# junliu111/CV-MonoSLAM

Hardware: AMD Instinct MI355X
Metric: srukf_updates_per_sec (higher is better)
Workload: dtype f64; 1 GPU; BASELINE configs[2]: 200 inverse-depth landmarks (n=1204, Na=1209, L=2419), M=N matched, fp64, one batched refactor per frame, synthetic 640x480 figure-8 sequence; landmarks=200, state_dim=1204, sequences_per_gpu=1, update_mode=batched

## Files before the change

### cv-monoslam_amd/csrc/srukf_api.hip

```cpp

#include "srukf_ctx.h"
using namespace srukf_impl;


namespace srukf_impl {

void srukf_pool_init()
{
    static std::mutex mu;
    static unsigned long long done_mask = 0;
    int dev = 0; hipMemPool_t pool = nullptr;
    if (hipGetDevice(&dev) != hipSuccess || dev < 0 || dev >= 64) return;
    const unsigned long long bit = 1ull << dev;
    std::lock_guard<std::mutex> lk(mu);
    if (done_mask & bit) return;
    if (hipDeviceGetDefaultMemPool(&pool, dev) == hipSuccess && pool) {
        unsigned long long keep = ~0ull;
        hipMemPoolSetAttribute(pool, hipMemPoolAttrReleaseThreshold, &keep);
    }
    done_mask |= bit;
}

hipError_t srukf_dmalloc_raw(void** p, size_t bytes)
{
    srukf_pool_init();
    hipError_t e = hipMallocAsync(p, bytes ? bytes : 8, nullptr);
    if (e == hipSuccess) e = hipStreamSynchronize(nullptr);
    return e;
}

hipError_t srukf_dfree(void* p) { return p ? hipFreeAsync(p, nullptr) : hipSuccess; }
hipError_t srukf_dfree_on(void* p, hipStream_t st) { return p ? hipFreeAsync(p, st) : hipSuccess; }

thread_local std::string g_create_error;

}

static thread_local double* g_spare_stage = nullptr;

static thread_local size_t g_spare_stage_bytes = 0;

namespace srukf_impl {

const char* const kclass_name[KC_COUNT] = { "k_motion", "k_project", "k_meas_stats", "k_pxy", "k_gain", "k_syrk",
                                             "k_gmw_step64", "k_gmw_persist", "k_gmw_check", "k_gmw_col", "k_rank_expand", "k_project_motion", "k_project_table", "k_pxy2",
                                             "misc", "k_det_response", "k_det_cand", "k_det_rank", "k_det_select", "k_capture_patch", "k_lm_ellipsoid", "k_bgr2gray", "k_overlay",
                                             "k_archive_predict", "k_archive_warp", "k_archive_search", "k_associate_checked" };

void gmw_plan_destroy(GmwPlan& g, hipStream_t st)
{
    if (g.pans) srukf_dfree_on(g.pans, st);
    if (g.sync) srukf_dfree_on(g.sync, st);
    if (g.tiles) srukf_dfree_on(g.tiles, st);
    g = GmwPlan();
}

}

static void gmw_tiles_xcd_order(std::vector<short>& tk, int ntiles_all, int workers, int T, int Tp)
{
    const int ntiles = ntiles_all - ((Tp > 0 && Tp < T) ? T - Tp : 0);
    if (ntiles > workers || ntiles < 16) return;
    struct Tl { short v[4]; };
    std::vector<Tl> comp, rest;
    const int h0 = srukf_gmw_head_rows() / 64, hx = h0 + srukf_gmw_head_extra_diag();
    for (int q = 0; q < ntiles; q++) {
        Tl t; for (int e = 0; e < 4; e++) t.v[e] = tk[4 * q + e];
        const int I = t.v[0], J = t.v[1];
        const bool computes = I >= h0 && !(I < hx && J < hx) && !(Tp < T && I == Tp);
        (computes ? comp : rest).push_back(t);
    }
    if (comp.size() < 16) return;
    std::sort(comp.begin(), comp.end(), [](const Tl& a, const Tl& b) { return a.v[0] != b.v[0] ? a.v[0] < b.v[0] : a.v[1] < b.v[1]; });
    size_t cut = comp.size() / 2;
    while (cut < comp.size() && cut > 0 && comp[cut].v[0] == comp[cut - 1].v[0]) cut++;
    std::vector<std::vector<Tl>> grp(8);
    for (int band = 0; band < 2; band++) {
        std::vector<Tl> b(comp.begin() + (band ? cut : 0), band ? comp.end() : comp.begin() + cut);
        std::sort(b.begin(), b.end(), [](const Tl& x, const Tl& y) { return x.v[1] != y.v[1] ? x.v[1] < y.v[1] : x.v[0] < y.v[0]; });
        for (size_t q = 0; q < b.size(); q++) grp[4 * band + std::min<size_t>(3, q * 4 / b.size())].push_back(b[q]);
    }
    int cap[8] = { 0 };
    for (int w = 0; w < ntiles; w++) cap[(w + 1) % 8]++;
    std::vector<Tl> spill(rest);
    for (int x = 0; x < 8; x++) while ((int)grp[x].size() > cap[x]) { spill.push_back(grp[x].back()); grp[x].pop_back(); }
    for (int x = 0; x < 8; x++) while ((int)grp[x].size() < cap[x] && !spill.empty()) { grp[x].push_back(spill.back()); spill.pop_back(); }
    size_t pos[8] = { 0 };
    for (int w = 0; w < ntiles; w++) {
        const int x = (w + 1) % 8;
        const Tl t = grp[x][pos[x]++];
        for (int e = 0; e < 4; e++) tk[4 * w + e] = t.v[e];
    }
}

namespace srukf_impl {

int gmw_plan_create(GmwPlan& g, int np, hipStream_t st, int Tp, int tenants)
{
    g.T = np / 64;
    g.Tp = (Tp > 0 && Tp < g.T) ? Tp : g.T;
    g.tenants = tenants > 1 ? tenants : 1;
    int cus = 0, dev = 0;
    if (hipGetDevice(&dev) != hipSuccess || hipDeviceGetAttribute(&cus, hipDeviceAttributeMultiprocessorCount, dev) != hipSuccess || cus < 2) cus = 2;
    g.cus = cus;
    const int cap = cus / (tenants > 1 ? tenants : 1) - 1;
    g.workers = cap >= 1 ? srukf_gmw_persist_workers(g.T, g.Tp, cap) : -1;
    g.ntiles = srukf_gmw_build_tiles(g.T, g.Tp, nullptr);
    g.nreal = g.ntiles - (g.Tp < g.T ? g.T - g.Tp : 0);
    std::vector<short> tk((size_t)4 * (g.ntiles > 0 ? g.ntiles : 1), 0);
    srukf_gmw_build_tiles(g.T, g.Tp, tk.data());
    gmw_tiles_xcd_order(tk, g.ntiles, g.workers, g.T, g.Tp);
    const size_t sync_bytes = (size_t)srukf_gmw_sync_bytes(g.T);
    if (srukf_dmalloc_on(&g.pans, (size_t)srukf_gmw_panel_bytes() * g.T, st) != hipSuccess ||
        srukf_dmalloc_on(&g.sync, sync_bytes, st) != hipSuccess ||
        srukf_dmalloc_on(&g.tiles, sizeof(short) * tk.size(), st) != hipSuccess) { gmw_plan_destroy(g, st); return SRUKF_ERR_NOMEM; }
    const unsigned long long epoch1 = 1;
    if (hipMemsetAsync(g.pans, 0, (size_t)srukf_gmw_panel_bytes() * g.T, st) != hipSuccess ||
        hipMemsetAsync(g.sync, 0, sync_bytes, st) != hipSuccess ||
        hipMemcpyAsync((char*)g.sync + offsetof(GmwSync, epoch), &epoch1, sizeof epoch1, hipMemcpyHostToDevice, st) != hipSuccess ||
        hipMemcpyAsync(g.tiles, tk.data(), sizeof(short) * tk.size(), hipMemcpyHostToDevice, st) != hipSuccess ||
        hipStreamSynchronize(st) != hipSuccess) { gmw_plan_destroy(g, st); return SRUKF_ERR_HIP; }
    return SRUKF_OK;
}

void host_weights(int Na, const srukf_params& p, KWeights& w)
{
    const double alpha = p.ut_alpha, beta = p.ut_beta;
    const double Lammda = alpha * alpha * Na - Na;
    switch (p.weight_type) {
    case 0:
        w.wm0 = 1.0 - Na / 3.0; w.wc0 = 1.0 - Na / 3.0; w.wi = (1.0 - w.wc0) / (2 * Na); w.wi_sr = sqrt(w.wi);
        w.gamma = sqrt(Na / (1.0 - w.wm0));
        break;
    case 1:
        w.gamma = sqrt(Na + Lammda); w.wm0 = Lammda / (Na + Lammda); w.wc0 = w.wm0 + (1 - alpha * alpha + beta);
        w.wi = 1.0 / (2 * (Na + Lammda)); w.wi_sr = sqrt(fabs(w.wi));
        break;
    default:
        w.gamma = sqrt(3.0 * Na / 2.0); w.wm0 = 1.0 / 3.0; w.wc0 = 1.0 / 3.0; w.wi = 1.0 / (3.0 * Na); w.wi_sr = sqrt(w.wi);
        break;
    }
}

void prof_collect(srukf_ctx* c)
{
    for (auto& e : c->pev) {
        float ms = 0.f;
        hipEventSynchronize(e.b);
        hipEventElapsedTime(&ms, e.a, e.b);
        c->prof_ms[e.kc] += ms; c->prof_n[e.kc] += 1;
        hipEventDestroy(e.a); hipEventDestroy(e.b);
    }
    c->pev.clear();
}

}


namespace srukf_impl {

std::vector<int> build_tile_table(int n_own, int n_other, bool upper, bool own_is_row, int k_index )
{
    std::vector<std::vector<int>> lst(8);
    for (int x = 0; x < 8; x++)
        for (int o = 0; o < n_other; o++)
            for (int w = x; w < n_own; w += 8) {
                const int r = own_is_row ? w : o, c = own_is_row ? o : w;
                if (upper && c < r) continue;
                lst[x].push_back(r); lst[x].push_back(c);
            }
    {
        for (auto& l : lst) {
            std::vector<std::pair<int, int>> t;
            for (size_t q = 0; q < l.size() / 2; q++) t.push_back({ l[2 * q], l[2 * q + 1] });
            std::stable_sort(t.begin(), t.end(), [k_index](const std::pair<int, int>& a, const std::pair<int, int>& b) {
                return k_index ? a.second > b.second : a.first > b.first; });
            for (size_t q = 0; q < t.size(); q++) { l[2 * q] = t[q].first; l[2 * q + 1] = t[q].second; }
        }
    }
    size_t mx = 0;
    for (auto& l : lst) mx = l.size() / 2 > mx ? l.size() / 2 : mx;
    std::vector<int> tab(mx * 8 * 2, -1);
    for (int x = 0; x < 8; x++)
        for (size_t q = 0; q < lst[x].size() / 2; q++) { tab[(q * 8 + x) * 2] = lst[x][2 * q]; tab[(q * 8 + x) * 2 + 1] = lst[x][2 * q + 1]; }
    return tab;
}

}

static int alloc_zero(srukf_ctx* c, void** p, size_t bytes)
{
    HIPCHK(c, srukf_dmalloc_on(p, bytes, c->stream));
    HIPCHK(c, hipMemsetAsync(*p, 0, bytes, c->stream));
    return SRUKF_OK;
}

#define ALLOC(ptr, count) do { int rc_ = alloc_zero(c, (void**)&(ptr), sizeof(*(ptr)) * (size_t)(count)); if (rc_) { g_create_error = c->err; srukf_destroy(c); return rc_; } } while (0)

static int block_cov(srukf_ctx* c, int off, int bs, double* out)
{
    srukf_launch_block_cov(c->stream, c->d, c->S, off, bs, c->small, nullptr);
    HIPCHK(c, hipMemcpyAsync(c->hstage, c->small, sizeof(double) * bs * bs, hipMemcpyDeviceToHost, c->stream));
    HIPCHK(c, hipStreamSynchronize(c->stream));
    memcpy(out, c->hstage, sizeof(double) * bs * bs);
    return SRUKF_OK;
}

extern "C" {

int srukf_abi_version(void) { return SRUKF_ABI_VERSION; }

int srukf_default_params(srukf_params* p)
{
    if (!p) return SRUKF_ERR_BAD_ARG;
    memset(p, 0, sizeof *p);
    p->cam_dx = 0.0028; p->cam_dy = 0.0028; p->cam_cx = 310.1129; p->cam_cy = 236.7526;
    p->cam_k1 = 0.0001; p->cam_k2 = 0.0; p->cam_f = 2.1735; p->image_w = 640; p->image_h = 480;
    p->a1 = p->a2 = p->a3 = p->a4 = 8.0; p->sigma_measure = 3.0; p->rho0 = 1.0 / 3.0; p->sigma_rho = p->rho0 / 2.0;
    p->sigma_x = 0.02; p->sigma_y = 0.02; p->sigma_z = 0.005; p->sigma_theta = 0.02;
    p->epsilon = 1e-13; p->ut_alpha = 1e-3; p->ut_beta = 2.0;
    p->weight_type = 0; p->noise_type = 0; p->newton_iters = 100;
    return SRUKF_OK;
}

const char* srukf_last_error(const srukf_ctx* ctx) { return ctx ? ctx->err.c_str() : g_create_error.c_str(); }

int srukf_create(srukf_ctx** out, int N, const srukf_params* p, int device, void* stream)
{
    if (!out || !p || N < 0) { g_create_error = "bad argument"; return SRUKF_ERR_BAD_ARG; }
    if (N > 32 * SRUKF_STAT_GROUPS) { g_create_error = "more than 2048 landmarks: the per-group statistics counters (FrameScalars::stat_cnt) serve 64 groups of 32"; return SRUKF_ERR_UNSUPPORTED; }
    if (p->noise_type != 0) { g_create_error = "noise_type != 0 draws random numbers (SLAM.cpp:1505-1516) and is not built"; return SRUKF_ERR_UNSUPPORTED; }
    int ndev = 0;
    if (hipGetDeviceCount(&ndev) != hipSuccess || ndev <= 0 || device < 0 || device >= ndev) {
        g_create_error = "no HIP device (this library has no CPU fallback)";
        return SRUKF_ERR_NO_DEVICE;
    }
    if (hipSetDevice(device) != hipSuccess) { g_create_error = "hipSetDevice failed"; return SRUKF_ERR_NO_DEVICE; }
    hipDeviceProp_t prop;
    if (hipGetDeviceProperties(&prop, device) != hipSuccess) { g_create_error = "hipGetDeviceProperties failed"; return SRUKF_ERR_NO_DEVICE; }
    if (strncmp(prop.gcnArchName, "gfx950", 6) != 0) {
        g_create_error = std::string("device is ") + prop.gcnArchName + ", kernels are built for gfx950 only";
        return SRUKF_ERR_NO_DEVICE;
    }
    srukf_ctx* c = new srukf_ctx();
    c->device = device; c->p = *p;
    if (!g_dbg_graphs) c->use_graph = false;
    if (stream) { c->stream = (hipStream_t)stream; c->own_stream = false; }
    else {
        if (hipStreamCreateWithFlags(&c->stream, hipStreamNonBlocking) != hipSuccess) { g_create_error = "hipStreamCreate failed"; delete c; return SRUKF_ERR_HIP; }
        c->own_stream = true;
    }
    KDims& d = c->d;
    d.N = N; d.n = 6 * N + 4; d.Na = d.n + 5; d.L = 2 * d.Na + 1;
    d.np = round_up(d.n, SRUKF_PAD); d.mp = round_up(2 * N > 0 ? 2 * N : 1, SRUKF_PAD);
    host_weights(d.Na, c->p, c->w);
    const size_t np = d.np, mp = d.mp;
    ALLOC(c->X, np); ALLOC(c->S, np * np); ALLOC(c->G, np * np); ALLOC(c->Gbak, np * np); ALLOC(c->Wf, np * np);
    ALLOC(c->sigR, (size_t)d.L * 8 + 8); ALLOC(c->mpart, srukf_meas_part_doubles(d.mp)); ALLOC(c->dxp, srukf_gain_part_doubles(d.np)); ALLOC(c->Cmat, (np + 64) * 4); ALLOC(c->Z, (size_t)d.L * mp); ALLOC(c->DZ, np * mp);
    ALLOC(c->Ut, mp * np); ALLOC(c->PxyR, 5 * mp);
    { const size_t Nn = (size_t)(N > 0 ? N : 1); ALLOC(c->h, mp + 4 * Nn + (Nn + 1) / 2); c->Si = c->h + mp; c->vis = (int*)(c->h + mp + 4 * Nn);
      ALLOC(c->zcur, mp + (Nn + 1) / 2); c->mcur = (int*)(c->zcur + mp); }
    ALLOC(c->D, np); ALLOC(c->odocur, 8); ALLOC(c->small, 64);
    ALLOC(c->theta, np); ALLOC(c->fs, 1);
    { char* pb0 = nullptr; char* pb1 = nullptr; ALLOC(pb0, srukf_gmw_panel_bytes()); ALLOC(pb1, srukf_gmw_panel_bytes()); c->pan[0] = pb0; c->pan[1] = pb1; }
// ... 530 lines not shown
```

### cv-monoslam_amd/csrc/srukf_ctx.h

```cpp
#pragma once
#include <hip/hip_runtime.h>
#include <math.h>
#include <stdio.h>
#include <stdlib.h>
#include <string.h>
#include <string>
#include <cstddef>
#include <vector>
#include <algorithm>
#include <utility>
#include <atomic>
#include <mutex>
#include <map>
#include "srukf_device.h"
#include "srukf_rank.h"

extern "C" {
void srukf_launch_motion(hipStream_t, KDims, KWeights, srukf_params, double*, double*, double*, double*, FrameScalars*, const double*, const double*, RankArgs);
void srukf_launch_project(hipStream_t, KDims, KWeights, srukf_params, const double*, const double*, const double*, double*, double*, const FrameScalars*);
void srukf_launch_meas_stats(hipStream_t, KDims, KWeights, const double*, const double*, const double*, double*, double*, double*, int*, double*);
int srukf_meas_part_doubles(int);
void srukf_launch_gain(hipStream_t, KDims, KWeights, double*, const double*, const double*, const int*, const double*, const double*,
                       const double*, const int*, const int*, FrameScalars*, double*, double*, const double*, RankArgs, const double*, double*,
                       const double*, int, const double*, double, const double*, int, const double*, double*);
void srukf_launch_project_motion(hipStream_t, KDims, KWeights, srukf_params, double*, double*, double*, double*, double*, double*, FrameScalars*, RankArgs);
int srukf_gain_part_doubles(int);
void srukf_launch_traj(hipStream_t, KDims, const double*, const double*, FrameScalars*, double*, int);
void srukf_launch_block_cov(hipStream_t, KDims, const double*, int, int, double*, const double*);
void srukf_launch_project_points(hipStream_t, srukf_params, int, const double*, const double*, const double*, const double*, double*);
void srukf_launch_pxy(hipStream_t, KDims, const double*, const double*, double*, const void*, int, KWeights, MeasArgs);
void srukf_launch_pxy2(hipStream_t, KDims, const double*, const double*, double*, double*, const void*, int, int, KWeights, MeasArgs, GainFold);
int srukf_pxy2_build_tiles(int mp, int np, int kr, int* out);
int srukf_pxy2_split_groups(void);
void srukf_launch_syrk(hipStream_t, KDims, const double*, const double*, int, int, double*, FrameScalars*, const void*, int, const double*, double*, RankArgs, const double*);
void srukf_launch_gmw_step64(hipStream_t, int, int, int, double, double*, const void*, void*, double*, double*, const FrameScalars*);
int srukf_gmw_panel_bytes(void);
int srukf_gmw_sync_bytes(int T);
int srukf_gmw_build_tiles(int T, int Tp, short* out);
int srukf_gmw_persist_workers(int T, int Tp, int max_workers);
void srukf_launch_gmw_persist(hipStream_t, int, int, double, double*, void*, double*, double*, void*, const void*, int, int, void*, const double*, const double*, int, int, int, int, int);
void srukf_launch_gmw_persist_head(hipStream_t, int, int, double, double*, void*, double*, double*, void*, const void*, int, int, void*, const double*, const double*, int, int, int, int, int, const HeadArgs*);
void srukf_launch_gmw_split(hipStream_t, hipStream_t, int, int, double, double*, void*, double*, double*, void*, const void*, int, void*, int, int, double*, double*, int);
void srukf_launch_gmw_split_fold(hipStream_t, hipStream_t, int, int, double, double*, void*, double*, double*, void*, const void*, int, void*, int, int, double*, double*, const double*, const double*, int);
int srukf_gmw_build_fold_list(int T, int Tp, short* out);
int srukf_gmw_fold_head_tile(int tr, int tc, int head_rows);
int srukf_gmw_fold_head_rows(int Tp);
void srukf_gmw_fold_head_override(int v);
void srukf_launch_gmw_split_alone(hipStream_t, int, int, int, double, double*, void*, double*, double*, void*, const void*, int, void*, int, int, double*, double*);
void srukf_launch_row_energy(hipStream_t, int, int, const double*, double*);
void srukf_launch_rank_diag(hipStream_t, int, int, const double*, const int*, double*);
void srukf_launch_rank_expand(hipStream_t, int, int, int, double, const double*, const double*, const int*, const int*, const double*, void*, const double*, int, double*, double*, double*, double, int, KDims, KWeights, srukf_params, double*, double*, int, const StepExport*, double, unsigned int*, int);
void srukf_launch_project_table(hipStream_t, KDims, KWeights, srukf_params, double*, double*, double*, double*, double*, double*, FrameScalars*, RankArgs, NullSkip);
void srukf_launch_sigr_rows(hipStream_t, KDims, KWeights, const double*, const double*, double*, const FrameScalars*, const int*, int);
void srukf_launch_rank_shadow(hipStream_t, int, int, int, const double*, const int*, double*);
void srukf_launch_rank_canon(hipStream_t, int, int, int, double, const int*, double*);
void srukf_launch_rank_round(hipStream_t, int, int, double*);
void srukf_launch_syrk_own(hipStream_t, int, int, const double*, const double*, int, int, int, double*, void*, const void*, int, int);
int srukf_gmw_register_form(int, int, int, int);
int srukf_pxy2_b_per(int, int);
void srukf_launch_pxy2_b(hipStream_t, KDims, const void*, int, const void*, int, int, KWeights, int);
void srukf_launch_gain_b(hipStream_t, KDims, KWeights, const void*, int, int, double);
void srukf_launch_syrk_b(hipStream_t, KDims, const void*, int, const void*, int, int, int, int);
void srukf_launch_syrk_own_b(hipStream_t, int, int, const void*, int, int, int, int, const void*, int, int);
void srukf_launch_gmw_step64_b(hipStream_t, int, int, int, double, const void*, int, int, int);
void srukf_launch_gmw_pivslab_b(hipStream_t, int, int, int, double, const void*, int, int, int);
void srukf_launch_gmw_trail_b(hipStream_t, int, int, const void*, int, int, int, int);
void srukf_launch_rank_expand_b(hipStream_t, int, int, int, double, const void*, int, double, KDims, KWeights, srukf_params);
int srukf_gmw_head_rows(void);
int srukf_gmw_head_extra_diag(void);
void srukf_launch_gmw_check(hipStream_t, int, int, const double*, const double*, FrameScalars*, const double*, int, double*);
void srukf_launch_gmw_col(hipStream_t, int, int, int, double, const double*, double*, double*, unsigned long long*, FrameScalars*, double*);
void srukf_set_exact_right_looking(int on);
void srukf_warm_exact_path(hipStream_t st, FrameScalars* fs);
int srukf_get_exact_right_looking(void);
void srukf_launch_gmw_stats(hipStream_t, int, int, const double*, FrameScalars*);
void srukf_launch_landmarks_cartesian(hipStream_t, KDims, const double*, const double*, double*, double*);
void srukf_launch_aug_map(hipStream_t, srukf_params, int, int, int, int, double, const double*, const double*, const double*, double*);
void srukf_launch_aug_x(hipStream_t, int, int, int, double, double, const double*, const double*, const int*, double*, double*, int, int);
void srukf_launch_aug_build(hipStream_t, int, int, int, int, double, double, const double*, const double*, const double*, double*, int, int, int);
void srukf_launch_gram(hipStream_t, int, int, const double*, double*);
void srukf_launch_warp_patch(hipStream_t, KDims, srukf_params, const double*, const double*, const double*, const double*, const double*, const double*,
                             const unsigned char*, const int*, unsigned char*);
void srukf_launch_associate(hipStream_t, KDims, srukf_params, const unsigned char*, const double*, const double*, const int*, const int*,
                            const unsigned char*, double*, int*, double*);
int srukf_mixed_build_tasks(int np, int ue, short* out_tasks, int* out_tiles, int* ntiles);
int srukf_mixed_build_tasks_red(int np, int ue, int krows, int rows_lim, short* out_tasks, int* out_tiles, int* ntiles);
int srukf_mixed_krows(int r);
void srukf_launch_split_bf3(hipStream_t, int, int, int, int, const double*, void*, size_t);
void srukf_launch_syrk_bf3(hipStream_t, int, int, int, int, int, const void*, size_t, const void*, int, const void*, int, double*, double*, void*);
size_t srukf_mixed_part_bytes(int ntasks);
void srukf_launch_cvt_f32(hipStream_t, size_t, const double*, float*);
void srukf_launch_cvt_robot_cols(hipStream_t, int, int, const double*, float*);
void srukf_launch_gain_dx(hipStream_t, int, int, const double*, double*, const double*);
void srukf_launch_syrk32(hipStream_t, int, int, int, const float*, const float*, const void*, int, const void*, int, double*, double*, void*, int);
int srukf_app_patch_stride(void);
int srukf_app_tmpl_stride(void);
void srukf_launch_associate_checked(hipStream_t, KDims, srukf_params, double, double, int, int, const unsigned char*, const double*, const double*, const int*, const int*,
                                    const unsigned char*, double*, int*, double*, double*, double*);
int srukf_match_score_stride(void);
int srukf_match_tmpl_stride(void);
}

#define SRUKF_GRAPH_FRAMES 8
#define SRUKF_MAX_TENANTS 4
#define SRUKF_NULL_ENERGY 1e-12
#ifndef SRUKF_BATCH_GROUPS_MAX
#define SRUKF_BATCH_GROUPS_MAX 4
#endif

enum KClass { KC_MOTION = 0, KC_PROJECT, KC_STATS, KC_PXY, KC_GAIN, KC_SYRK, KC_GMW_TRAIL, KC_GMW_PERSIST, KC_GMW_CHECK,
              KC_GMW_COL, KC_RANK_EXPAND, KC_PROJECT_MOTION, KC_PROJECT_TABLE, KC_PXY2, KC_MISC,
              KC_DET_RESPONSE, KC_DET_CAND, KC_DET_RANK, KC_DET_SELECT, KC_CAPTURE, KC_LM_ELLIPSOID, KC_BGR2GRAY, KC_OVERLAY,
              KC_ARCHIVE_PREDICT, KC_ARCHIVE_WARP, KC_ARCHIVE_SEARCH, KC_ASSOC_CHECKED, KC_COUNT };
struct ProfEvent { hipEvent_t a, b; int kc; };

struct GmwPlan { void* pans = nullptr; void* sync = nullptr; void* tiles = nullptr; int ntiles = 0, nreal = 0, T = 0, Tp = 0, workers = -1, tenants = 1, cus = 0; };

struct DetScratch {
    double *resp = nullptr, *cand_r = nullptr; int *cand_pix = nullptr, *sorted = nullptr, *rank = nullptr, *gxy = nullptr, *blk = nullptr; void* hdr = nullptr;
    void *in = nullptr, *out = nullptr; size_t in_bytes = 0, out_bytes = 0;
};

struct RansacScratch {
    double *Ut = nullptr, *D = nullptr, *zin = nullptr, *res = nullptr, *X = nullptr, *S = nullptr, *odo = nullptr;
    double *sigR = nullptr, *Cm = nullptr, *Z = nullptr, *DZ = nullptr, *h = nullptr, *PxyR = nullptr, *mpart = nullptr;
    unsigned char* F = nullptr; int* votes = nullptr; FrameScalars* fs = nullptr;
};

struct ArchiveState {
    int L = 0;
    double *X6 = nullptr, *S66 = nullptr, *R = nullptr, *t = nullptr, *px = nullptr, *rob = nullptr, *out = nullptr, *hst = nullptr;
    unsigned char *patch = nullptr, *tmpl = nullptr;
};


struct srukf_switches {
    int rank_aware = 1;
    int debug_allow_mixed = 0;
    int debug_starve = 0;
    bool split_off = false;
    bool use_graph = true;
    struct DbgSwitches {
        int fused_motion = 2;
        int f32_fuse = 1;
        int table_perm = 1;
        int tail_fuse = 1;
        int head_fold = 1;
        int nullskip = 1;
        int pxy2 = 1;
        int step_fuse_export = 1;
        int view_auto = 1;
        int step_early = 2;
        int step_spin = 1;
        int step_fast = 1;
        int split_record = 0;
        int null_canon = 1;
        int split_fold = 1;
        int gain_fold = 0;
        int mixed_rank = 1;
        int mixed_null_ppm = 1;
        int mixed_bf16 = 0;
        int mixed_f64_robot = 1;
    } dbg;
};

struct srukf_handle_scope : srukf_switches {
    int device = 0;
    hipStream_t stream = nullptr;
    bool own_stream = false;
    srukf_params p;
    std::vector<srukf_ctx*> retired;
    double* spare_stage = nullptr; size_t spare_stage_bytes = 0;
    bool profiling = false;
    std::vector<ProfEvent> pev;
    double prof_ms[KC_COUNT] = {}; long long prof_n[KC_COUNT] = {}; double prof_flops[KC_COUNT] = {}; double prof_bytes[KC_COUNT] = {};
    unsigned char *d_image = nullptr, *d_bgr = nullptr, *d_ovl = nullptr; bool frame_valid = false, bgr_valid = false;
    DetScratch det;
    ArchiveState archive;
    std::string err;
    template <class F> void each_device_buffer(F f) const { void* b[] = { d_image, d_bgr, d_ovl }; for (void* q : b) f(q); }
};

struct srukf_life {
    int storage = SRUKF_STORAGE_F64;
    bool dx_pending = false;
    bool dx_lm = false;
    bool xr1_pending = false;
    int K_new = 0;
    bool null_canonical = false;
    bool tail_ok = false;
    int clamp_frame_host = -1, clamp_row_host = -1;
    int seqF = 0;
    int phase = 0;
    bool frame_updated = false;
    bool next_odo_valid = false;
    bool async_pending = false;
    bool step_fast = false;
    bool step_uncommitted = false;
    bool step_chain = false;
    bool proj_valid = false;
    bool fs_seq_step = false;
    bool last_update_sequential = false;
    bool ck_valid = false;
    bool ck3_inflight = false;
    bool ck_pending = false;
    bool pre_issued = false;
    bool next_pose_pending = false;
    bool setstep_done = false;
    unsigned long long meas_seq = 0;
    bool step_export_attached = false;
    StepExport step_export = {};
    bool mirror_next = false;
    bool view_auto = false; int view_unused = 0;
    int view_hits = 0;
    bool view_cached = false;
    bool robot_cached = false;
    bool f32_stale = false;
    int step_fast_frames = 0, step_slow_frames = 0;
    int exact_frames = 0;
};

struct srukf_map_scope : srukf_life {
    KDims d;
    KWeights w;
    double *X = nullptr, *S = nullptr, *G = nullptr, *Gbak = nullptr, *Wf = nullptr;
    double *sigR = nullptr, *Cmat = nullptr, *Z = nullptr, *DZ = nullptr, *Ut = nullptr;
    double *h = nullptr, *Si = nullptr, *PxyR = nullptr, *D = nullptr;
    double *zcur = nullptr, *odocur = nullptr, *small = nullptr, *mpart = nullptr, *dxp = nullptr;
    int *vis = nullptr, *mcur = nullptr;
    unsigned long long* theta = nullptr;
    unsigned int* fold_sync = nullptr; double* dxk = nullptr; int fold_robot_tiles = 0;
    unsigned char *app_patch = nullptr, *app_tmpl = nullptr;
    double *appR = nullptr, *appT = nullptr, *appPx = nullptr, *corr = nullptr;
    int* has_app = nullptr;
    double* ov_in = nullptr; void* ov_rec = nullptr;
    double *match_res = nullptr, *match_scores = nullptr; bool match_valid = false;
    RansacScratch ransac;
    double* disp = nullptr;
    float *S32 = nullptr, *X32 = nullptr;
    float *U32 = nullptr; double* mx_part = nullptr; void *mx_tasks = nullptr, *mx_tiles = nullptr; int mx_ntasks = 0, mx_ntiles = 0;
    float* A32 = nullptr; double* mxr_part = nullptr; void *mxr_tasks = nullptr, *mxr_tiles = nullptr; int mxr_ntasks = 0, mxr_ntiles = 0, mxr_krows = 0, mxr_for_r = 0;
    int* mxr_f64_tiles = nullptr; int mxr_n_f64_tiles = 0;
    unsigned short* mxr_xt = nullptr; size_t mxr_xt_stride = 0; int mxr_ktot = 0;
    int *perm = nullptr, *iperm = nullptr;
    double* Sdis = nullptr;
    void* pan[2] = { nullptr, nullptr };
    GmwPlan gplan;
    int red_r = 0, red_Tp = 0;
    int *red_perm = nullptr, *red_iperm = nullptr;
    double* gdiag = nullptr;
    double *shadowA = nullptr, *Utp = nullptr;
    double *slabW = nullptr, *slabL = nullptr;
    double *gsW = nullptr, *gsL = nullptr; int gs_panels = 0;
    hipStream_t side = nullptr; hipEvent_t ev_fork = nullptr, ev_join = nullptr;
    double* P1 = nullptr; int* pxy2_tiles = nullptr; int n_pxy2_tiles = 0, pxy2_split_b0 = 0;
    int* nskip = nullptr; int ns_full = 0, ns_null = 0, ns_rows = 0;
    int* red_head0_tiles = nullptr; int n_red_head0_tiles = 0;
    void* split_fold_list = nullptr; int n_split_fold = 0;
    double red_head0_flop = 0.0;
    int* red_syrk_tiles = nullptr; int n_red_syrk_tiles = 0;
    double red_fac_flop = 0, red_own_flop = 0;
    GmwPlan gplan_red;
    int shared_tenants = 2;
    int gmw_shared = 0;
    double *ckS = nullptr, *ckX = nullptr;
    int *syrk_tiles = nullptr, *pxy_tiles = nullptr;
    int *syrk_head_tiles = nullptr;
    int n_syrk_tiles = 0, n_pxy_tiles = 0, n_syrk_head_tiles = 0, n_syrk_head_crit = 0;
    int* syrk_head_tiles_b = nullptr; int n_syrk_head_tiles_b = 0;
// ... 184 lines not shown
```

### cv-monoslam_amd/csrc/srukf_debug.hip

```cpp

#include "srukf_ctx.h"
using namespace srukf_impl;


namespace srukf_impl {
std::atomic<int> g_dbg_gmw_persist{1}, g_dbg_gmw_fused{1}, g_dbg_rank_fused{1}, g_dbg_rank_fold{1}, g_dbg_rank_aware{1}, g_dbg_graphs{1};
std::atomic<int> g_dbg_mem_split{1};
std::atomic<int> g_dbg_shared_tenants{2};
std::atomic<int> g_dbg_batch_wide{1}, g_dbg_batch_groups{0}, g_dbg_batch_split{1};
std::atomic<int> g_dbg_timing{0}, g_dbg_fold_head{0}, g_dbg_fold_force{0}, g_dbg_ctx_keep{24}, g_dbg_batch_xcd{1}, g_dbg_batch_k128{1};
std::atomic<int> g_dbg_head_fold_free{0};
}

static bool debug_buffer(srukf_ctx* c, const char* key, double** ptr, long long* cap)
{
    const KDims& d = c->d;
    const GmwPlan& gp = c->red_r > 0 ? c->gplan_red : c->gplan;
    double* src = nullptr; long long n = 0;
    if (!strcmp(key, "Z")) { src = c->Z; n = (long long)d.L * d.mp; }
    else if (!strcmp(key, "DZ")) { src = c->DZ; n = (long long)d.np * d.mp; }
    else if (!strcmp(key, "sigR")) { src = c->sigR; n = (long long)(d.L + 1) * 8; }
    else if (!strcmp(key, "Cmat")) { src = c->Cmat; n = (long long)d.n * 4; }
    else if (!strcmp(key, "Xr1")) { src = (double*)((char*)c->fs + offsetof(FrameScalars, Xr1)); n = 4; }
    else if (!strcmp(key, "Utp")) { src = c->Utp; n = c->Utp ? (long long)d.mp * d.np : 0; }
    else if (!strcmp(key, "P1")) { src = c->P1; n = c->P1 ? (long long)d.mp * d.np : 0; }
    else if (!strcmp(key, "h")) { src = c->h; n = 2LL * d.N; }
    else if (!strcmp(key, "Si")) { src = c->Si; n = 4LL * d.N; }
    else if (!strcmp(key, "det_resp")) { src = c->det.resp; n = c->det.resp ? (long long)c->p.image_w * (long long)c->p.image_h : 0; }
    else if (!strcmp(key, "Wf")) { src = c->Wf; n = (long long)d.np * d.np; }
    else if (!strcmp(key, "Gbak")) { src = c->Gbak; n = (long long)d.np * d.np; }
    else if (!strcmp(key, "G")) { src = c->G; n = (long long)d.np * d.np; }
    else if (!strcmp(key, "D")) { src = c->D; n = d.np; }
    else if (!strcmp(key, "fold_dbg")) { src = c->fold_sync ? (double*)(c->fold_sync + ((srukf_fold_words(d.mp / 64, d.np / 64) + 1) & ~1)) : nullptr; n = c->fold_sync ? FOLD_DBG_STAMPS : 0; }
    else if (!strcmp(key, "gsW")) { src = c->gsW; n = c->gsW ? (long long)c->gs_panels * 64 * d.np : 0; }
    else if (!strcmp(key, "gsL")) { src = c->gsL; n = c->gsL ? (long long)c->gs_panels * 64 * d.np : 0; }
    else if (!strcmp(key, "pans")) { src = (double*)gp.pans; n = gp.pans ? (long long)srukf_gmw_panel_bytes() * gp.T / 8 : 0; }
    else if (!strcmp(key, "sync")) { src = (double*)gp.sync; n = gp.sync ? (long long)srukf_gmw_sync_bytes(gp.T) / 8 : 0; }
    else return false;
    *ptr = src; *cap = n;
    return true;
}

extern "C" {

int srukf_debug_allow_mixed(srukf_ctx* c, int on)
{
    if (!c) return SRUKF_ERR_BAD_ARG;
    c->debug_allow_mixed = on ? 1 : 0;
    return SRUKF_OK;
}

int srukf_debug_poke_state(srukf_ctx* c, int row, int col, double value)
{
    if (!c || row < 0 || col < row || col >= c->d.n) return SRUKF_ERR_BAD_ARG;
    HIPCHK(c, hipSetDevice(c->device));
    step_commit_motion(c); step_invalidate(c);
    HIPCHK(c, hipStreamSynchronize(c->stream));
    HIPCHK(c, hipMemcpy(c->S + (size_t)row * c->d.np + col, &value, sizeof(double), hipMemcpyHostToDevice));
    return SRUKF_OK;
}

int srukf_debug_set(srukf_ctx* c, const char* key, int value)
{
    if (!key) return SRUKF_ERR_BAD_ARG;
    struct { const char* k; std::atomic<int>* v; } globals[] = { { "gmw_persist", &g_dbg_gmw_persist }, { "gmw_fused", &g_dbg_gmw_fused }, { "rank_fused", &g_dbg_rank_fused },
                                                    { "rank_fold", &g_dbg_rank_fold }, { "rank_aware", &g_dbg_rank_aware }, { "graphs", &g_dbg_graphs }, { "mem_split", &g_dbg_mem_split }
                                                  };
    if (!strcmp(key, "batch_split")) { g_dbg_batch_split = value ? 1 : 0; batch_drop_all_graphs(); return SRUKF_OK; }
    if (!strcmp(key, "head_fold_free")) { if (value < 1) return SRUKF_ERR_BAD_ARG; g_dbg_head_fold_free = value; if (c) { hipSetDevice(c->device); step_commit_motion(c); step_invalidate(c); hipStreamSynchronize(c->stream); drop_graphs(c); } return SRUKF_OK; }
    if (!strcmp(key, "batch_groups")) { if (value < 0 || value > SRUKF_BATCH_GROUPS_MAX) return SRUKF_ERR_BAD_ARG; g_dbg_batch_groups = value; return SRUKF_OK; }
    if (!strcmp(key, "batch_wide")) { g_dbg_batch_wide = value ? 1 : 0; return SRUKF_OK; }
    if (!strcmp(key, "timing")) { g_dbg_timing = value ? 1 : 0; return SRUKF_OK; }
    if (!strcmp(key, "fold_head")) { g_dbg_fold_head = value < 0 ? 0 : value; srukf_gmw_fold_head_override(g_dbg_fold_head); return SRUKF_OK; }
    if (!strcmp(key, "batch_k128")) { g_dbg_batch_k128 = value ? 1 : 0; batch_drop_all_graphs(); return SRUKF_OK; }
    if (!strcmp(key, "batch_xcd")) { g_dbg_batch_xcd = value ? 1 : 0; batch_drop_all_graphs(); return SRUKF_OK; }
    if (!strcmp(key, "ctx_keep")) { g_dbg_ctx_keep = value < 0 ? 0 : value; return SRUKF_OK; }
    if (!strcmp(key, "fold_force")) { g_dbg_fold_force = value ? 1 : 0; return SRUKF_OK; }
    if (!strcmp(key, "exact_rl")) { srukf_set_exact_right_looking(value); return SRUKF_OK; }
    if (!strcmp(key, "shared_tenants")) {
        if (value < 2 || value > 8) return SRUKF_ERR_BAD_ARG;
        g_dbg_shared_tenants = value;
        return SRUKF_OK;
    }
    for (auto& g : globals)
        if (!strcmp(key, g.k)) {
            g.v->store(!strcmp(key, "mem_split") ? value : (value ? 1 : 0));
            if (c) { hipSetDevice(c->device); step_commit_motion(c); step_invalidate(c); hipStreamSynchronize(c->stream); drop_graphs(c); if (!strcmp(key, "rank_aware")) return update_null_set(c); }
            return SRUKF_OK;
        }
    if (!c) return SRUKF_ERR_BAD_ARG;
    HIPCHK(c, hipSetDevice(c->device));
    step_commit_motion(c); step_invalidate(c);
    HIPCHK(c, hipStreamSynchronize(c->stream));
    if (!strcmp(key, "use_graph")) c->use_graph = value != 0;
    else if (!strcmp(key, "pxy2")) c->dbg.pxy2 = value ? 1 : 0;
    else if (!strcmp(key, "nullskip")) c->dbg.nullskip = value ? 1 : 0;
    else if (!strcmp(key, "head_fold")) c->dbg.head_fold = value ? 1 : 0;
    else if (!strcmp(key, "tail_fuse")) c->dbg.tail_fuse = value ? 1 : 0;
    else if (!strcmp(key, "table_perm")) c->dbg.table_perm = value ? 1 : 0;
    else if (!strcmp(key, "f32_fuse")) c->dbg.f32_fuse = value ? 1 : 0;
    else if (!strcmp(key, "split_record")) c->dbg.split_record = value ? 1 : 0;
    else if (!strcmp(key, "gain_fold")) c->dbg.gain_fold = value ? 1 : 0;
    else if (!strcmp(key, "null_canon")) c->dbg.null_canon = value ? 1 : 0;
    else if (!strcmp(key, "split_fold")) c->dbg.split_fold = value < 0 ? 0 : value > 2 ? 2 : value;
    else if (!strcmp(key, "mixed_rank")) c->dbg.mixed_rank = value ? 1 : 0;
    else if (!strcmp(key, "mixed_f64_robot")) c->dbg.mixed_f64_robot = value ? 1 : 0;
    else if (!strcmp(key, "mixed_bf16")) c->dbg.mixed_bf16 = value ? 1 : 0;
    else if (!strcmp(key, "mixed_null_ppm")) c->dbg.mixed_null_ppm = value < 0 ? 0 : value;
    else if (!strcmp(key, "step_fast")) c->dbg.step_fast = value ? 1 : 0;
    else if (!strcmp(key, "step_spin")) c->dbg.step_spin = value ? 1 : 0;
    else if (!strcmp(key, "step_early")) c->dbg.step_early = value < 0 ? 0 : value > 2 ? 2 : value;
    else if (!strcmp(key, "view_auto")) { c->dbg.view_auto = value ? 1 : 0; if (!value) { c->view_auto = false; c->view_cached = false; } }
    else if (!strcmp(key, "step_fuse_export")) c->dbg.step_fuse_export = value ? 1 : 0;
    else if (!strcmp(key, "fused_motion")) c->dbg.fused_motion = value < 0 ? 0 : value > 2 ? 2 : value;
    else { c->err = std::string("srukf_debug_set: unknown key ") + key; return SRUKF_ERR_BAD_ARG; }
    drop_graphs(c);
    return SRUKF_OK;
}

int srukf_debug_gmw_stamps(srukf_ctx* c, unsigned long long* buf)
{
    if (!c) return SRUKF_ERR_BAD_ARG;
    static unsigned long long* dbuf = nullptr;
    HIPCHK(c, hipSetDevice(c->device));
    HIPCHK(c, hipStreamSynchronize(c->stream));
    GmwPlan& g = c->red_r > 0 ? c->gplan_red : c->gplan;
    if (!g.sync) return SRUKF_ERR_SEQUENCE;
    if (!dbuf) { HIPCHK(c, hipMalloc((void**)&dbuf, 8 * 4096)); HIPCHK(c, hipMemset(dbuf, 0, 8 * 4096)); }
    if (buf) HIPCHK(c, hipMemcpy(buf, dbuf, 8 * 4096, hipMemcpyDeviceToHost));
    HIPCHK(c, hipMemcpy((char*)g.sync + offsetof(GmwSync, dbg), &dbuf, 8, hipMemcpyHostToDevice));
    return SRUKF_OK;
}

int srukf_debug_get(srukf_ctx* c, const char* key, long long* value)
{
    if (!c || !key || !value) return SRUKF_ERR_BAD_ARG;
    HIPCHK(c, hipSetDevice(c->device));
    HIPCHK(c, hipMemcpyAsync(c->hfs, c->fs, sizeof(FrameScalars), hipMemcpyDeviceToHost, c->stream));
    HIPCHK(c, hipStreamSynchronize(c->stream));
    if (!strcmp(key, "gmw_aborts")) *value = c->hfs->gmw_aborts;
    else if (!strcmp(key, "clamp_rows")) *value = c->hfs->clamp_rows;
    else if (!strcmp(key, "frame")) *value = c->hfs->frame;
    else if (!strcmp(key, "frozen")) *value = c->hfs->frozen;
    else if (!strcmp(key, "gate_timeouts")) *value = c->hfs->gate_timeouts;
    else if (!strcmp(key, "gmw_shared")) *value = c->gmw_shared;
    else if (!strcmp(key, "split_off")) *value = c->split_off ? 1 : 0;
    else if (!strcmp(key, "use_graph")) *value = c->use_graph ? 1 : 0;
    else if (!strncmp(key, "pad", 3) && key[3] >= '1' && key[3] <= '7' && !key[4]) {
        const GmwPlan& gp = c->red_r > 0 ? c->gplan_red : c->gplan;
        unsigned long long v = 0, zero = 0;
        const size_t off = offsetof(GmwSync, pad) + 8 * (size_t)(key[3] - '0');
        if (gp.sync) { HIPCHK(c, hipMemcpy(&v, (char*)gp.sync + off, sizeof v, hipMemcpyDeviceToHost)); HIPCHK(c, hipMemcpy((char*)gp.sync + off, &zero, sizeof zero, hipMemcpyHostToDevice)); }
        *value = (long long)v;
    }
    else if (!strcmp(key, "abort_code")) {
        const GmwPlan& gp = c->red_r > 0 ? c->gplan_red : c->gplan;
        unsigned long long code = 0, zero = 0;
        if (gp.sync) {
            HIPCHK(c, hipMemcpy(&code, (char*)gp.sync + offsetof(GmwSync, pad), sizeof code, hipMemcpyDeviceToHost));
            HIPCHK(c, hipMemcpy((char*)gp.sync + offsetof(GmwSync, pad), &zero, sizeof zero, hipMemcpyHostToDevice));
        }
        *value = (long long)code;
    }
    else if (!strcmp(key, "step_fast")) *value = c->step_fast_frames;
    else if (!strcmp(key, "step_slow")) *value = c->step_slow_frames;
    else if (!strcmp(key, "exact_frames")) *value = c->exact_frames;
    else if (!strcmp(key, "fold_seqs")) *value = c->fold_seqs;
    else if (!strcmp(key, "split_fold_seqs")) *value = c->split_fold_seqs;
    else if (!strncmp(key, "pxy2_stamp", 10) && key[10] >= '1' && key[10] <= '7') { const unsigned long long* t = (const unsigned long long*)(c->hmeas + c->d.mp + 5 * (size_t)c->d.N); *value = (long long)(t[key[10] - '0'] - t[0]); }
    else if (!strcmp(key, "meas_flag_ticks")) { const unsigned long long* t = (const unsigned long long*)(c->hmeas + c->d.mp + 5 * (size_t)c->d.N); *value = (long long)(t[1] - t[0]); }
    else if (!strcmp(key, "view_hits")) *value = c->view_hits;
    else if (!strcmp(key, "view_auto")) *value = c->view_auto ? 1 : 0;
    else if (!strcmp(key, "split_form")) *value = split_form(c, c->red_r > 0 ? c->gplan_red : c->gplan) ? 1 : 0;
    else if (!strncmp(key, "plan_", 5)) {
        const GmwPlan& gp = c->red_r > 0 ? c->gplan_red : c->gplan;
        const RefactorPlan rp = refactor_form(c, refactor_frame_tail(c));
        const bool persist = plan_persists(c, gp);
        const char* k = key + 5;
        if (!strcmp(k, "T")) *value = gp.T;
        else if (!strcmp(k, "Tp")) *value = gp.Tp;
        else if (!strcmp(k, "tiles")) *value = gp.nreal;
        else if (!strcmp(k, "workers")) *value = gp.workers;
        else if (!strcmp(k, "persist")) *value = persist ? 1 : 0;
        else if (!strcmp(k, "register_form")) *value = (persist && !split_form(c, gp) && srukf_gmw_register_form(gp.T, gp.Tp, gp.ntiles, gp.workers)) ? 1 : 0;
        else if (!strcmp(k, "tiles_per_worker")) *value = gp.workers > 0 ? (gp.nreal + gp.workers - 1) / gp.workers : -1;
        else if (!strcmp(k, "fold")) *value = rp.form == RF_OWNERS_FOLD ? 1 : 0;
        else if (!strcmp(k, "head_fold")) *value = rp.head_fold ? 1 : 0;
        else if (!strcmp(k, "red_perm")) *value = replay_red_perm(c) ? 1 : 0;
        else if (!strcmp(k, "motion")) *value = replay_motion_mode(c);
        else if (!strcmp(k, "fuse")) *value = frame_form(c).fused_tail() ? 1 : 0;
        else if (!strcmp(k, "kept")) *value = c->red_r;
        else if (!strcmp(k, "sync_doubles")) *value = gp.sync ? srukf_gmw_sync_bytes(gp.T) / 8 : 0;
        else if (!strcmp(k, "pans_doubles")) *value = gp.pans ? (long long)srukf_gmw_panel_bytes() * gp.T / 8 : 0;
        else if (!strcmp(k, "slab_panels")) *value = c->gs_panels;
        else return SRUKF_ERR_BAD_ARG;
    }
    else return SRUKF_ERR_BAD_ARG;
    return SRUKF_OK;
}

int srukf_debug_copy(srukf_ctx* c, const char* key, double* out, long long count)
{
    if (!c || !key || !out || count < 0) return SRUKF_ERR_BAD_ARG;
    HIPCHK(c, hipSetDevice(c->device));
    HIPCHK(c, hipStreamSynchronize(c->stream));
    double* src = nullptr; long long cap = 0;
    if (!debug_buffer(c, key, &src, &cap)) return SRUKF_ERR_BAD_ARG;
    if (!src || count > cap) return SRUKF_ERR_DIM_MISMATCH;
    HIPCHK(c, hipMemcpy(out, src, sizeof(double) * (size_t)count, hipMemcpyDeviceToHost));
    return SRUKF_OK;
}

int srukf_debug_upload(srukf_ctx* c, const char* key, const double* in, long long count)
{
    if (!c || !key || !in || count < 0) return SRUKF_ERR_BAD_ARG;
    HIPCHK(c, hipSetDevice(c->device));
    HIPCHK(c, hipStreamSynchronize(c->stream));
    double* dst = nullptr; long long cap = 0;
    if (!debug_buffer(c, key, &dst, &cap)) return SRUKF_ERR_BAD_ARG;
    if (!dst || count > cap) return SRUKF_ERR_DIM_MISMATCH;
    HIPCHK(c, hipMemcpy(dst, in, sizeof(double) * (size_t)count, hipMemcpyHostToDevice));
    return SRUKF_OK;
}

int srukf_debug_starve_workers(srukf_ctx* c, int on)
{
    if (!c) return SRUKF_ERR_BAD_ARG;
    c->debug_starve = on == 2 ? 2 : on ? 1 : 0;
    step_invalidate(c);
    drop_graphs(c);
    return SRUKF_OK;
}

int srukf_gmw_host(int device, int n, const double* G, double* S_out, double* D_out, double epsilon, int force_slow, int* clamp_hit)
{
    if (n < 1 || !G || !S_out) return SRUKF_ERR_BAD_ARG;
    int ndev = 0;
    if (hipGetDeviceCount(&ndev) != hipSuccess || device < 0 || device >= ndev) return SRUKF_ERR_NO_DEVICE;
    if (hipSetDevice(device) != hipSuccess) return SRUKF_ERR_NO_DEVICE;
    const int np = round_up(n, SRUKF_PAD);
    const size_t bytes = sizeof(double) * (size_t)np * np;
    std::vector<double> hG((size_t)np * np, 0.0), hS((size_t)np * np, 0.0), hD(np, 0.0);
    for (int r = 0; r < n; r++) for (int c = r; c < n; c++) hG[(size_t)r * np + c] = G[(size_t)r * n + c];
    struct Res {
        double *dG = nullptr, *dS = nullptr, *dD = nullptr, *dWf = nullptr; unsigned long long* dTh = nullptr; FrameScalars* dFs = nullptr;
        void* pan[2] = { nullptr, nullptr }; GmwPlan gp;
        ~Res() { for (void* b : { (void*)dG, (void*)dS, (void*)dD, (void*)dWf, (void*)dTh, (void*)dFs, pan[0], pan[1] }) if (b) srukf_dfree(b); gmw_plan_destroy(gp); }
    } r;
#define GH(call) do { if ((call) != hipSuccess) return SRUKF_ERR_HIP; } while (0)
    GH(srukf_dmalloc((void**)&r.dG, bytes)); GH(srukf_dmalloc((void**)&r.dS, bytes)); GH(srukf_dmalloc((void**)&r.dWf, bytes));
    GH(srukf_dmalloc((void**)&r.dD, sizeof(double) * np)); GH(srukf_dmalloc((void**)&r.dTh, sizeof(unsigned long long) * np)); GH(srukf_dmalloc((void**)&r.dFs, sizeof(FrameScalars)));
    GH(hipMemcpy(r.dG, hG.data(), bytes, hipMemcpyHostToDevice));
    GH(hipMemset(r.dS, 0, bytes)); GH(hipMemset(r.dWf, 0, bytes)); GH(hipMemset(r.dTh, 0, sizeof(unsigned long long) * np));
    GH(hipMemset(r.dFs, 0, sizeof(FrameScalars))); GH(hipMemset(r.dD, 0, sizeof(double) * np));
    hipStream_t st = nullptr;
    srukf_launch_gmw_stats(st, n, np, r.dG, r.dFs);
    FrameScalars fs;
    if (!force_slow) {
        if (gmw_persist_mode()) { const int rc = gmw_plan_create(r.gp, np, st); if (rc) return rc; }
        if (gmw_persist_mode() && r.gp.workers >= 0) {
            srukf_launch_gmw_persist(st, n, np, epsilon, r.dG, r.gp.pans, r.dD, r.dS, r.gp.sync, r.gp.tiles, r.gp.ntiles, r.gp.workers, r.dFs, nullptr, nullptr, 0, 0, 0, 0, 0);
        } else {
            GH(srukf_dmalloc(&r.pan[0], srukf_gmw_panel_bytes())); GH(srukf_dmalloc(&r.pan[1], srukf_gmw_panel_bytes()));
            GH(hipMemset(r.pan[0], 0, srukf_gmw_panel_bytes())); GH(hipMemset(r.pan[1], 0, srukf_gmw_panel_bytes()));
            int pb = 0;
            for (int j0 = -64; j0 + 64 < np; j0 += 64, pb ^= 1)
                srukf_launch_gmw_step64(st, n, np, j0, epsilon, r.dG, r.pan[pb ^ 1], r.pan[pb], r.dD, r.dS, nullptr);
        }
        GH(hipDeviceSynchronize());
        srukf_launch_gmw_check(st, n, np, r.dD, r.dS, r.dFs, nullptr, 0, nullptr);
        GH(hipMemcpy(&fs, r.dFs, sizeof fs, hipMemcpyDeviceToHost));
        if (clamp_hit) *clamp_hit = fs.clamp_rows;
        if (fs.clamp_rows > 0) force_slow = 2;
    }
    if (force_slow) {
        GH(hipMemcpy(r.dG, hG.data(), bytes, hipMemcpyHostToDevice));
        GH(hipMemset(r.dTh, 0, sizeof(unsigned long long) * np));
        GH(hipMemset(r.dS, 0, bytes));
        for (int j = 0; j < n; j++) srukf_launch_gmw_col(st, n, np, j, epsilon, r.dG, r.dWf, r.dD, r.dTh, r.dFs, r.dS);
        GH(hipMemcpy(&fs, r.dFs, sizeof fs, hipMemcpyDeviceToHost));
        if (clamp_hit && force_slow == 1) *clamp_hit = fs.clamp_rows;
    }
    GH(hipDeviceSynchronize());
    GH(hipMemcpy(hS.data(), r.dS, bytes, hipMemcpyDeviceToHost));
    GH(hipMemcpy(hD.data(), r.dD, sizeof(double) * np, hipMemcpyDeviceToHost));
#undef GH
    for (int rr = 0; rr < n; rr++) memcpy(S_out + (size_t)rr * n, hS.data() + (size_t)rr * np, sizeof(double) * n);
    if (D_out) memcpy(D_out, hD.data(), sizeof(double) * n);
    return SRUKF_OK;
}

int srukf_project_host(int device, const srukf_params* p, int count, const double* feat6, const double* pos3, const double* psi,
                       const double* err2, double* uv_out)
{
    if (!p || count < 1 || !feat6 || !pos3 || !psi || !err2 || !uv_out) return SRUKF_ERR_BAD_ARG;
    int ndev = 0;
    if (hipGetDeviceCount(&ndev) != hipSuccess || device < 0 || device >= ndev) return SRUKF_ERR_NO_DEVICE;
    if (hipSetDevice(device) != hipSuccess) return SRUKF_ERR_NO_DEVICE;
    double *df, *dp, *ds, *de, *dout;
    srukf_dmalloc((void**)&df, sizeof(double) * 6 * count); srukf_dmalloc((void**)&dp, sizeof(double) * 3 * count);
    srukf_dmalloc((void**)&ds, sizeof(double) * count); srukf_dmalloc((void**)&de, sizeof(double) * 2 * count); srukf_dmalloc((void**)&dout, sizeof(double) * 2 * count);
    hipMemcpy(df, feat6, sizeof(double) * 6 * count, hipMemcpyHostToDevice); hipMemcpy(dp, pos3, sizeof(double) * 3 * count, hipMemcpyHostToDevice);
    hipMemcpy(ds, psi, sizeof(double) * count, hipMemcpyHostToDevice); hipMemcpy(de, err2, sizeof(double) * 2 * count, hipMemcpyHostToDevice);
    srukf_launch_project_points(nullptr, *p, count, df, dp, ds, de, dout);
    hipError_t e = hipDeviceSynchronize();
    hipMemcpy(uv_out, dout, sizeof(double) * 2 * count, hipMemcpyDeviceToHost);
    srukf_dfree(df); srukf_dfree(dp); srukf_dfree(ds); srukf_dfree(de); srukf_dfree(dout);
    return e == hipSuccess ? SRUKF_OK : SRUKF_ERR_HIP;
}

}
```

### cv-monoslam_amd/csrc/srukf_gmw_persist.hip

```cpp
#include <hip/hip_runtime.h>
#include <algorithm>
#include <cmath>
#include <cstdio>
#include <cstdlib>
#include <utility>
#include <vector>
#include "srukf_device.h"
#include "srukf_tiles.h"
#include "srukf_gmw_cols.h"
#include "srukf_gmw_panel.h"
#include "srukf_rank.h"

#ifndef GMW_XWG_LIMIT
#define GMW_XWG_LIMIT (1 << 16)
#endif
__device__ __forceinline__ unsigned long long gmw_uniform64(unsigned long long v)
{
    return ((unsigned long long)(unsigned)__builtin_amdgcn_readfirstlane((int)(v >> 32)) << 32) | (unsigned)__builtin_amdgcn_readfirstlane((int)v);
}
__device__ __forceinline__ bool gmw_wait_ge(const unsigned long long* f, unsigned long long want, const int* abort_flag)
{
    for (int spins = 0; spins < GMW_XWG_LIMIT; spins++) {
        if (gmw_uniform64(__hip_atomic_load(f, __ATOMIC_RELAXED, __HIP_MEMORY_SCOPE_AGENT)) >= want) return true;
        if ((spins & 31) == 31 && __builtin_amdgcn_readfirstlane(__hip_atomic_load(abort_flag, __ATOMIC_RELAXED, __HIP_MEMORY_SCOPE_AGENT))) return false;
// ... 123 lines not shown
                    Wc[32 + jj][cc] = W2[a][t];  Lr[32 + jj][cc] = W2[a][t] * dr[2 + a][t];
                }
        }
        if (wv0) GMW_TS(sy, p, 1);
        __syncthreads();
        if (!first) {
#pragma unroll
            for (int k = 0; k < 64; k += 4)
                g = __builtin_amdgcn_mfma_f64_16x16x4f64(-Lr[k + lk][16 * qa + lr], Wc[k + lk][16 * qb + lr], g, 0, 0, 0);
        }
#pragma unroll
        for (int t = 0; t < 4; t++) ws.Xm[16 * qa + lk + 4 * t][16 * qb + lr] = g[t];
        __syncthreads();
        if (wv0) GMW_TS(sy, p, 2);
        if (wv0) { gmw_cols_pivot_wave(ws, eps, lane); GMW_TS(sy, p + 64, 4); }
        else if (wvu == 2) { gmw_cols_t_wave<0>(ws, lane, nullptr, kp.T1); GMW_TS(sy, p + 64, 5); }
        else {
            if (!first) {
#pragma unroll
                for (int k = 0; k < 64; k += 4) {
                    const double a0 = -Lr[k + lk][ro + lr], a1 = -Lr[k + lk][ro + 16 + lr];
                    const double b0 = Wc[k + lk][32 + lr], b1 = Wc[k + lk][48 + lr];
                    acc[0][0] = __builtin_amdgcn_mfma_f64_16x16x4f64(a0, b0, acc[0][0], 0, 0, 0);
                    acc[0][1] = __builtin_amdgcn_mfma_f64_16x16x4f64(a0, b1, acc[0][1], 0, 0, 0);
                    acc[1][0] = __builtin_amdgcn_mfma_f64_16x16x4f64(a1, b0, acc[1][0], 0, 0, 0);
                    acc[1][1] = __builtin_amdgcn_mfma_f64_16x16x4f64(a1, b1, acc[1][1], 0, 0, 0);
                }
            }
            double (*X)[32] = (wv == 1) ? X01 : X11;
#pragma unroll
            for (int a = 0; a < 2; a++)
#pragma unroll
                for (int b = 0; b < 2; b++)
#pragma unroll
                    for (int t = 0; t < 4; t++) X[16 * a + lk + 4 * t][16 * b + lr] = acc[a][b][t];
            if (!first) {
                const int c4 = lr * 4;
#pragma unroll 4
                for (int i = 0; i < 8; i++) {
                    const int row = ro + 4 * i + lk;
                    const double sq = kp.sq[row];
                    d4 w = *(const d4*)&Wc[row][c4];
                    w[0] *= sq; w[1] *= sq; w[2] *= sq; w[3] *= sq;
                    *(d4*)&Sout[(size_t)(j0 + row) * ld + base + c4] = w;
                }
            }
            if (wv1) GMW_TS(sy, p + 64, 6); else GMW_TS(sy, p + 64, 7);
        }
        __syncthreads();
        if (wv0) GMW_TS(sy, p, 3);
        {
            d4 wq = (d4){0, 0, 0, 0};
#pragma unroll
            for (int u = 0; u < 8; u++)
                wq = __builtin_amdgcn_mfma_f64_16x16x4f64(kp.T1[(4 * u + lk) * 33 + 16 * qa + lr], X01[4 * u + lk][16 * qb + lr], wq, 0, 0, 0);
#pragma unroll
            for (int t = 0; t < 4; t++) {
                const int k = 16 * qa + lk + 4 * t, cc = 16 * qb + lr;
                const double e = wq[t] * gmw_pivot_rcp(ws.Dv[k]);
                Wc[k][cc] = wq[t];
                Lr[k][cc] = e;
                kp.Ep[k * 32 + (cc ^ (16 * (k & 1)))] = e;
            }
        }
        __syncthreads();
        if (!half_only) {
            d4 x;
#pragma unroll
            for (int t = 0; t < 4; t++) x[t] = X11[16 * qa + lk + 4 * t][16 * qb + lr];
#pragma unroll
            for (int k = 0; k < 32; k += 4)
                x = __builtin_amdgcn_mfma_f64_16x16x4f64(-Lr[k + lk][16 * qa + lr], Wc[k + lk][16 * qb + lr], x, 0, 0, 0);
#pragma unroll
            for (int t = 0; t < 4; t++) ws2.Xm[16 * qa + lk + 4 * t][16 * qb + lr] = x[t];
        }
        __syncthreads();
        if (wv0) GMW_TS(sy, p, 4);
        unsigned long long early = 0;
        if (wv0) { if (!half_only) gmw_cols_pivot_wave(ws2, eps, lane); GMW_TS(sy, p + 64, 0); }
        else if (wvu == 2) {
            if (!half_only) {
            unsigned long long fa = 0, fb = 0;
            if (p >= 1 && p + 1 < Tp) {
                fa = __hip_atomic_load(&ver[GMW_VIDX(p, p + 1, T)], __ATOMIC_RELAXED, __HIP_MEMORY_SCOPE_AGENT);
                fb = __hip_atomic_load(&ver[GMW_VIDX((p + 1), p + 1, T)], __ATOMIC_RELAXED, __HIP_MEMORY_SCOPE_AGENT);
            }
            gmw_cols_t_wave<2>(ws2, lane, nxt->Tt2, kp.T2, [&] {
                if (p == 0 || gmw_uniform64(fa) >= ebase + p) stageok[0] = 1;
                if (p == 0 || gmw_uniform64(fb) >= ebase + p) stageok[1] = 1;
            });
            GMW_TS(sy, p + 192, 0);
            }
        } else {
            const int c4 = (lane & 7) * 4;
            if (wv1) {
#pragma unroll
                for (int i = 0; i < 4; i++) {
                    const int row = 8 * i + (lane >> 3);
                    st_d4<true>(&nxt->E[row * 32 + c4], *(const d4*)&Lr[row][c4]);
                }
                if (lane < 32) {
                    const double D = ws.Dv[lane], rc = gmw_pivot_rcp(D), sq = sqrt(D) * rc;
                    st_dev(&nxt->D[lane], D); st_dev(&nxt->sq[lane], sq); st_dev(&nxt->rD[lane], rc);
                }
            } else gmw_copy_t<true>(kp.T1, nxt->Tt1, lane);
            asm volatile("s_waitcnt vmcnt(0)" ::: "memory");
            {
                int prev = 0;
                if (lane == 0) prev = __hip_atomic_fetch_add(halfcnt, 1, __ATOMIC_RELAXED, __HIP_MEMORY_SCOPE_WORKGROUP);
                if (__builtin_amdgcn_readfirstlane(prev) == 1) gmw_set_panel_flag(sy->half_ready, ebase + p + 1, lane);
            }
            if (!wv1) {
#pragma unroll
                for (int i = 0; i < 4; i++) {
                    const int row = 8 * i + (lane >> 3);
                    const double Dr = ws.Dv[row];
                    const double sq = (base + row < n) ? sqrt(Dr) * gmw_pivot_rcp(Dr) : 0.0;
                    d4 w = *(const d4*)&Wc[row][c4];
                    w[0] *= sq; w[1] *= sq; w[2] *= sq; w[3] *= sq;
                    *(d4*)&Sout[(size_t)(base + row) * ld + base + 32 + c4] = w;
                }
            }
            gmw_cols_out_wave<true>(ws, wv1 ? 0 : 1, lane, n, ld, base, nxt->D, nxt->sq, nxt->rD, Dall, Sout, kp.sq, kp.rD);
            if (!half_only) gmw_cols_out_wave<true>(ws2, wv1 ? 0 : 1, lane, n, ld, base + 32, nxt->D + 32, nxt->sq + 32, nxt->rD + 32, Dall, Sout, kp.sq + 32, kp.rD + 32,
                                                    [&] { if (p >= 1 && p + 1 < Tp) early = __hip_atomic_load(&ver[GMW_VIDX((wv1 ? p : p + 1), p + 1, T)], __ATOMIC_RELAXED, __HIP_MEMORY_SCOPE_AGENT); });
            if (wv1) GMW_TS(sy, p + 64, 1); else GMW_TS(sy, p + 64, 2);
        }
        if (p + 1 < Tp) {
            const bool tileA = wvu < 2;
            const int tr = tileA ? p : p + 1, r0 = (wvu & 1) ? 0 : 32;
            if (wv1) GMW_TS(sy, p, 5);
            const bool ready = p == 0 || gmw_uniform64(early) >= ebase + p || __builtin_amdgcn_readfirstlane(stageok[tileA ? 0 : 1]) != 0 ||
                               gmw_wait_ge(&ver[GMW_VIDX(tr, p + 1, T)], ebase + p, &sy->abort);
            if (wv1) GMW_TS(sy, p, 6);
            if (!ready) *okp = 0;
            else {
                double (*dst)[G64_LS] = tileA ? Lr : Wc;
                const double* src = G + (size_t)(64 * tr + r0) * ld + 64 * (p + 1) + lane;
                double v[32];
#pragma unroll
                for (int r = 0; r < 32; r++) v[r] = ld_dev(src + (size_t)r * ld);
#pragma unroll
                for (int r = 0; r < 32; r++) dst[r0 + r][lane] = v[r];
            }
        }
        else asm volatile("s_waitcnt vmcnt(0)" ::: "memory");
        __syncthreads();
        if (wv3 && p + 1 < T) { gmw_set_panel_flag(sy->panel_ready, ebase + p + 1, lane); GMW_TS(sy, p + 64, 3); }
        if (wv0) GMW_TS(sy, p, 7);
        if (!*okp) { if (wv0) gmw_abandon(sy, 1); return; }
    }
}

#ifndef GMW_MEM_EARLY2
#define GMW_MEM_EARLY2 0
#endif
struct GmwOwned { int I, J, nsteps; bool computed; int kfirst; bool passon; };
struct KDimsLite { int n, ld; };
__device__ __forceinline__ bool gmw_owner_step(int n, int ld, int T, int k, const GmwOwned& tl, d4 (&acc)[2][2], double* __restrict__ G,
                                               GmwPanel64* pans, double* __restrict__ Sout, GmwSync* sy, unsigned long long ebase,
                                               double (*Lr)[G64_LS], double (*Wc)[G64_LS], int* okp, bool wv0, int tid, bool memtile = false, bool rows32 = false)
{
    unsigned long long* ver = gmw_sync_ver(sy);
    if (wv0) {
        const unsigned long long want = ebase + k;
        unsigned long long a = want, b = want, pr = 0;
        for (int spins = 0; spins < GMW_XWG_LIMIT; spins++) {
            if (k > 0) {
                a = __hip_atomic_load(&ver[GMW_VIDX(k, tl.I, T)], __ATOMIC_RELAXED, __HIP_MEMORY_SCOPE_AGENT);
                b = __hip_atomic_load(&ver[GMW_VIDX(k, tl.J, T)], __ATOMIC_RELAXED, __HIP_MEMORY_SCOPE_AGENT);
            }
            pr = __hip_atomic_load(&sy->panel_ready[(blockIdx.x % GMW_FLAG_COPIES) * GMW_FLAG_STRIDE], __ATOMIC_RELAXED, __HIP_MEMORY_SCOPE_AGENT);
            a = gmw_uniform64(a); b = gmw_uniform64(b); pr = gmw_uniform64(pr);
            if (a >= want && b >= want) break;
            if ((spins & 31) == 31 && __builtin_amdgcn_readfirstlane(__hip_atomic_load(&sy->abort, __ATOMIC_RELAXED, __HIP_MEMORY_SCOPE_AGENT))) break;
            __builtin_amdgcn_s_sleep(1);
        }
        *okp = (a >= want && b >= want) ? ((pr >= ebase + k + 1) ? 2 : 1) : 0;
    }
    __syncthreads();
    if (!*okp) return false;
    const bool behind = *okp == 2;
    const bool last = k == tl.nsteps - 1;
    __syncthreads();
    return gmw_tile_update<true>(n, ld, 64 * k, tl.I - k - 1, tl.J - k - 1, G, pans + k, Sout, Lr, Wc, tid, acc, !tl.passon && (memtile || (k == 0 && !tl.computed)),
                                 !tl.passon && (memtile || last),
        [&] {
            if (!behind) { if (wv0) *okp = gmw_wait_ge(&sy->half_ready[(blockIdx.x % GMW_FLAG_COPIES) * GMW_FLAG_STRIDE], ebase + k + 1, &sy->abort); }
            __syncthreads();
            return *okp != 0;
        },
        [&] {
            if (!behind) { if (wv0) *okp = gmw_wait_ge(&sy->panel_ready[(blockIdx.x % GMW_FLAG_COPIES) * GMW_FLAG_STRIDE], ebase + k + 1, &sy->abort); }
            __syncthreads();
            return *okp != 0;
        },
        [&] { if (last && !tl.passon) gmw_publish(&ver[GMW_VIDX(tl.I, tl.J, T)], ebase + tl.nsteps, wv0); },
        behind && (!memtile || GMW_MEM_EARLY2 > 0), rows32 && tl.passon, memtile && GMW_MEM_EARLY2 == 1);
}

#define GMW_OWNED_MAX 2
#define GMW_OWNED_MEM 6
struct GmwTile { short I, J, nsteps, pad; };
#define GMW_HEAD_ROWS 2
#define GMW_HEAD_EXTRA_DIAG 2
__device__ __forceinline__ bool gmw_owner_computes(int I, int J) { return I >= GMW_HEAD_ROWS && !(I < GMW_HEAD_ROWS + GMW_HEAD_EXTRA_DIAG && J < GMW_HEAD_ROWS + GMW_HEAD_EXTRA_DIAG); }
template <bool DEEP = true>
__device__ __forceinline__ void gmw_owner_syrk(const KDimsLite d, const double* __restrict__ S0, const double* __restrict__ Ut0, int u0, int u1,
                                               int I, int J, d4 (&acc)[2][2], FrameScalars* __restrict__ fs, int tid, int krows)
{
    const int lane = tid & 63, wv = tid >> 6, lr = lane & 15, lk = lane >> 4;
    const int m0 = 64 * I + 32 * (wv >> 1), c0 = 64 * J + 32 * (wv & 1);
    zero_acc(acc);
    if (m0 >= d.ld || c0 >= d.ld || c0 + 32 <= m0) return;
    if constexpr (DEEP) {
        tile32_tn_deep<false>(acc, S0, d.ld, S0, d.ld, m0, c0, 0, min(m0 + 32, krows), lane);
        tile32_tn_deep<true>(acc, Ut0, d.ld, Ut0, d.ld, m0, c0, u0, u1, lane);
    } else {
        tile32_tn<false>(acc, S0, d.ld, S0, d.ld, m0, c0, 0, min(m0 + 32, krows), lane);
        tile32_tn<true>(acc, Ut0, d.ld, Ut0, d.ld, m0, c0, u0, u1, lane);
    }
    double gmax = 0.0, xmax = 0.0;
#pragma unroll
    for (int a = 0; a < 2; a++)
#pragma unroll
        for (int b = 0; b < 2; b++)
#pragma unroll
            for (int t = 0; t < 4; t++) {
                const int r = m0 + 16 * a + lk + 4 * t, c = c0 + 16 * b + lr;
                if (r < d.n && c < d.n && c >= r) { if (r == c) gmax = fmax(gmax, acc[a][b][t]); else xmax = fmax(xmax, acc[a][b][t]); }
            }
    gmax = wave_max(gmax); xmax = wave_max(xmax);
    if (lane == 0) {
        if (gmax > 0.0) atomicMax(&fs->gmax_bits, (unsigned long long)__double_as_longlong(gmax));
        if (xmax > 0.0) atomicMax(&fs->ximax_bits, (unsigned long long)__double_as_longlong(xmax));
    }
}

template <bool DEEP>
__device__ __forceinline__ void syrk_own_body(int n, int ld, const double* __restrict__ S0, const double* __restrict__ Ut0, int u0, int u1, int krows,
                                              double* __restrict__ G, FrameScalars* __restrict__ fs, const GmwTile* __restrict__ tiles, int nreal, const int bid)
{
    const GmwTile t = tiles[nreal - 1 - bid];
    if (!gmw_owner_computes(t.I, t.J)) return;
    const int tid = threadIdx.x, lane = tid & 63, wv = tid >> 6, lr = lane & 15, lk = lane >> 4;
    d4 acc[2][2];
    const KDimsLite dl = { n, ld };
    gmw_owner_syrk<DEEP>(dl, S0, Ut0, u0, u1, t.I, t.J, acc, fs, tid, krows);
    const int m0 = 64 * t.I + 32 * (wv >> 1), c0 = 64 * t.J + 32 * (wv & 1);
    if (m0 >= ld || c0 >= ld || c0 + 32 <= m0) return;
#pragma unroll
    for (int a = 0; a < 2; a++)
#pragma unroll
        for (int b = 0; b < 2; b++)
#pragma unroll
            for (int tt = 0; tt < 4; tt++) G[(size_t)(m0 + 16 * a + lk + 4 * tt) * ld + c0 + 16 * b + lr] = acc[a][b][tt];
}
__global__ __launch_bounds__(256) void k_syrk_own(int n, int ld, const double* __restrict__ S0, const double* __restrict__ Ut0, int u0, int u1, int krows,
                                                  double* __restrict__ G, FrameScalars* __restrict__ fs, const GmwTile* __restrict__ tiles, int nreal)
{
    syrk_own_body<true>(n, ld, S0, Ut0, u0, u1, krows, G, fs, tiles, nreal, (int)blockIdx.x);
}
__global__ __launch_bounds__(256) __attribute__((amdgpu_waves_per_eu(4, 8))) void k_syrk_own_b(int n, int ld, const SyrkOwnArgs* __restrict__ tab, int B, int u0, int u1, int krows, const GmwTile* __restrict__ tiles, int nreal)
{
    const int f = (int)blockIdx.x % B, bid = (int)blockIdx.x / B;
    const SyrkOwnArgs a = tab[f];
    syrk_own_body<false>(n, ld, a.S0, a.Ut0, u0, u1, krows, a.G, a.fs, tiles, nreal, bid);
}

__device__ int g_gmw_admitted = 0;
__global__ void k_gmw_gate(FrameScalars* __restrict__ fs, int limit)
{
    if (fs->frozen) return;
    if (threadIdx.x != 0) return;
    for (int spins = 0; spins < (1 << 22); spins++) {
        const int cur = __hip_atomic_load(&g_gmw_admitted, __ATOMIC_RELAXED, __HIP_MEMORY_SCOPE_AGENT);
        if (cur < limit && atomicCAS(&g_gmw_admitted, cur, cur + 1) == cur) return;
        __builtin_amdgcn_s_sleep(8);
    }
    atomicAdd(&g_gmw_admitted, 1);
    atomicAdd(&fs->gate_timeouts, 1);
}

__device__ __forceinline__ void gmw_head_tile_job(int n, int ld, int krows, const double* __restrict__ S0, const double* __restrict__ Ut0, int u0, int u1,
                                                  int2 tl, double* __restrict__ G, FrameScalars* __restrict__ fs, double* smem, int tid, GmwSync* sy = nullptr, bool stamp = false)
{
    if (tl.x < 0) return;
    double (*red)[64][17] = (double (*)[64][17])smem;
    const int lane = tid & 63, wv = tid >> 6, lr = lane & 15, lk = lane >> 4;
    const int m0 = tl.x * 32, n0 = tl.y * 32;
    d4 acc[2][2];
    zero_acc(acc);
    const int ke = min(m0 + 32, krows);
    const int ngs = ke >> 4, ngu = (u1 - u0) >> 4, ng = ngs + ngu;
    const int g0 = (ng * wv) >> 2, g1 = (ng * (wv + 1)) >> 2;
    if (g0 < ngs) tile32_tn_deep<false>(acc, S0, ld, S0, ld, m0, n0, g0 << 4, min(g1, ngs) << 4, lane);
    if (stamp && wv == 0) GMW_TS(sy, 132, 1);
    if (g1 > ngs) tile32_tn_deep<true>(acc, Ut0, ld, Ut0, ld, m0, n0, u0 + ((max(g0, ngs) - ngs) << 4), u0 + ((g1 - ngs) << 4), lane);
    if (stamp && wv == 0) GMW_TS(sy, 132, 2);
    if (stamp && wv == 3) GMW_TS(sy, 132, 6);
    splitk_reduce(acc, red, wv, lane);
    if (stamp && wv == 0) GMW_TS(sy, 132, 3);
    if (wv != 0) return;
    double gmax = 0.0, xmax = 0.0;
#pragma unroll
    for (int a = 0; a < 2; a++)
#pragma unroll
        for (int b = 0; b < 2; b++)
#pragma unroll
            for (int t = 0; t < 4; t++) {
                const int r = m0 + 16 * a + lk + 4 * t, c = n0 + 16 * b + lr;
                const double v = acc[a][b][t];
                st_dev(&G[(size_t)r * ld + c], v);
                if (r < n && c < n) { if (r == c) gmax = fmax(gmax, v); else xmax = fmax(xmax, v); }
            }
    gmax = wave_max(gmax); xmax = wave_max(xmax);
    if (lane == 0) {
        if (gmax > 0.0) atomicMax(&fs->gmax_bits, (unsigned long long)__double_as_longlong(gmax));
        if (xmax > 0.0) atomicMax(&fs->ximax_bits, (unsigned long long)__double_as_longlong(xmax));
    }
}
__device__ __forceinline__ bool gmw_wait_head(const unsigned int* cnt, unsigned int want, const int* abort_flag)
{
    for (int spins = 0; spins < GMW_XWG_LIMIT; spins++) {
        if ((unsigned)__builtin_amdgcn_readfirstlane((int)__hip_atomic_load(cnt, __ATOMIC_RELAXED, __HIP_MEMORY_SCOPE_AGENT)) >= want) return true;
        if ((spins & 31) == 31 && __builtin_amdgcn_readfirstlane(__hip_atomic_load(abort_flag, __ATOMIC_RELAXED, __HIP_MEMORY_SCOPE_AGENT))) return false;
        __builtin_amdgcn_s_sleep(1);
    }
    return false;
}

template <bool MEM>
__global__ __launch_bounds__(256) void k_gmw_persist(int n, int ld, int T, int Tp, double* __restrict__ G, GmwPanel64* __restrict__ pans,
                                                     double* __restrict__ Sout, double* __restrict__ Dall, double eps,
                                                     GmwSync* __restrict__ sy, const GmwTile* __restrict__ tiles, int ntiles,
                                                     FrameScalars* __restrict__ fs,
                                                     const double* __restrict__ S0, const double* __restrict__ Ut0, int u0, int u1, int krows, int gated,
                                                     const HeadArgs ha)
{
    __shared__ double Lr[64][G64_LS];
    __shared__ double Wc[64][G64_LS];
    __shared__ double facreg[2 * GMW_FAC_DOUBLES];
    __shared__ double xreg[1024 + 1024 + 32 * 33];
    __shared__ double keepreg[1024 + 64 + 64];
    __shared__ int ok, halfcnt, stageok[2];
    const int tid = threadIdx.x;
    const int nhelp = ha.nhelp;
    const int nmain = (int)gridDim.x - nhelp;
    const int role = (int)blockIdx.x < nmain ? (int)blockIdx.x : -1;
    int2 mytile = make_int2(-1, -1);
    unsigned long long t01 = 0, t23 = 0, t45 = 0;
    const int npass = (!MEM && Tp < T) ? T - Tp : 0, nreal = ntiles - npass;
    if (!MEM) {
        if (role < 0) { const int hb = (int)blockIdx.x - nmain; if (hb < ha.ntiles) mytile = ha.tiles[hb]; }
        else if (role > 0) {
            const unsigned long long* tq = (const unsigned long long*)tiles;
            if (role - 1 < nreal) t01 = tq[role - 1];
            if (role - 1 + nmain - 1 < nreal) t23 = tq[role - 1 + nmain - 1];
            if (role - 1 < npass) t45 = tq[nreal + role - 1];
        }
    }
    int frozen_now = fs->frozen;
    unsigned long long epoch_now = sy->epoch;
    if constexpr (MEM) asm volatile("" : "+s"(frozen_now), "+s"(epoch_now));
    else asm volatile("" : "+v"(mytile.x), "+v"(mytile.y), "+v"(t01), "+v"(t23), "+v"(t45), "+v"(frozen_now), "+v"(epoch_now));
    if (frozen_now) return;
    const unsigned long long ebase = epoch_now << GMW_EPOCH_SHIFT;
    if (role < 0) {
        if constexpr (!MEM) {
        const int nhead = ha.ntiles + ha.ndx + ha.ngd;
        const int wvu = __builtin_amdgcn_readfirstlane(tid >> 6), lane = tid & 63;
        const int job = (int)blockIdx.x - nmain;
#ifdef SRUKF_GMW_DBG
        if (tid == 0) atomicAdd(&sy->pad[1], 1ull);
#endif
        if ((int)blockIdx.x == nmain) GMW_TS(sy, 131, 0);
        if (job < ha.ntiles) {
            if (job == 0) GMW_TS(sy, 132, 0);
            gmw_head_tile_job(n, ld, krows, S0, Ut0, u0, u1, mytile, G, fs, &Lr[0][0], tid, sy, job == 0);
            if (job == 0) GMW_TS(sy, 132, 4);
            asm volatile("s_waitcnt vmcnt(0)" ::: "memory");
            __syncthreads();
            if (job == 0) GMW_TS(sy, 132, 5);
            if (job < ha.ncrit && job < 32) GMW_TS(sy, 140 + job, 0);
            if (wvu == 0) { if (lane == 0) __hip_atomic_fetch_add(job < ha.ncrit ? gmw_head_crit(sy) : gmw_head_done(sy), 1u, __ATOMIC_RELAXED, __HIP_MEMORY_SCOPE_AGENT); }
        } else if (job < ha.ntiles + ha.ndx) {
            const int dj = job - ha.ntiles;
            if (ha.ra.prep_next && dj == 0 && tid == 255) fs->ctl_next_valid = srukf_prepare_control(fs, fs->frame + 1) ? 1 : 0;
            srukf_gain_dx_job(n, ld, ha.dxp, ha.X, dj, ha.xr1, ha.ra.f32round, ha.ra.dxN);
        } else if (job < nhead) srukf_rank_gdiag_job(n, ld, u1, ha.ra, &fs->gmax_bits, job - ha.ntiles - ha.ndx);
        if ((int)blockIdx.x == nmain) GMW_TS(sy, 131, 1);
        if ((int)blockIdx.x == (int)gridDim.x - 1) GMW_TS(sy, 131, 2);
#ifdef SRUKF_GMW_DBG
        __syncthreads();
        if (tid == 0) atomicAdd(&sy->pad[2], 1ull);
#endif
        }
    } else if (role == 0) {
        bool head_ok = true;
        GMW_TS(sy, 128, 0);
        if (ha.ntiles > 0) {
            if (__builtin_amdgcn_readfirstlane(tid >> 6) == 0) ok = gmw_wait_head(gmw_head_crit(sy), (unsigned)ha.ncrit, &sy->abort) ? 1 : 0;
            __syncthreads();
            head_ok = ok != 0;
            __syncthreads();
        }
        GMW_TS(sy, 128, 1);
        if (head_ok) gmw_pivot_persist(n, ld, T, Tp, eps, G, pans, Dall, Sout, sy, ebase, Lr, Wc, facreg, xreg, keepreg, &ok, &halfcnt, stageok, tid, krows);
        else if (__builtin_amdgcn_readfirstlane(tid >> 6) == 0) gmw_abandon(sy, 2);
        GMW_TS(sy, 128, 2);
    } else {
        const bool wv0 = __builtin_amdgcn_readfirstlane(tid >> 6) == 0;
        const int workers = nmain - 1, w = role - 1;
        bool good = true;
        const bool half_last = (Tp < T) && (krows <= 64 * (Tp - 1) + 32);
        if constexpr (MEM) {
            int kmax = 0;
            for (int m = 0; m < GMW_OWNED_MEM; m++) if (w + m * workers < ntiles) kmax = max(kmax, (int)tiles[w + m * workers].nsteps);
            for (int k = 0; k < kmax && good; k++)
                for (int m = 0; m < GMW_OWNED_MEM && good; m++) {
                    const int ti = w + m * workers;
                    if (ti >= ntiles) break;
                    const GmwTile t = tiles[ti];
                    if (k >= t.nsteps) continue;
                    if (k < t.pad) continue;
                    const GmwOwned tm = { t.I, t.J, t.nsteps, false, t.pad, Tp < T && t.I == Tp };
                    d4 accm[2][2];
                    zero_acc(accm);
                    good = gmw_owner_step(n, ld, T, k, tm, accm, G, pans, Sout, sy, ebase, Lr, Wc, &ok, wv0, tid, true, half_last && k == Tp - 1);
                }
        } else {
        GmwOwned ta = { 0, 0, 0, false, 0, false }, tb = { 0, 0, 0, false, 0, false }, tc = { 0, 0, 0, false, 0, false };
        auto entry = [](unsigned long long q) { GmwTile t; t.I = (short)(q & 0xffff); t.J = (short)((q >> 16) & 0xffff); t.nsteps = (short)((q >> 32) & 0xffff); t.pad = (short)((q >> 48) & 0xffff); return t; };
        if (w < nreal) { const GmwTile t = entry(t01); ta.I = t.I; ta.J = t.J; ta.nsteps = t.nsteps; ta.kfirst = t.pad; ta.passon = Tp < T && t.I == Tp; }
        if (w + workers < nreal) { const GmwTile t = entry(t23); tb.I = t.I; tb.J = t.J; tb.nsteps = t.nsteps; tb.kfirst = t.pad; tb.passon = Tp < T && t.I == Tp; }
        if (w < npass) { const GmwTile t = entry(t45); tc.I = t.I; tc.J = t.J; tc.nsteps = t.nsteps; tc.kfirst = t.pad; tc.passon = true; tc.computed = true; }
        d4 acca[2][2], accb[2][2];
        zero_acc(acca); zero_acc(accb);
        if (role == 1) GMW_TS(sy, 129, 0);
        if (role == nmain - 1) GMW_TS(sy, 130, 0);
        if (S0) {
            const KDimsLite dl = { n, ld };
            if (ta.nsteps > 0 && gmw_owner_computes(ta.I, ta.J)) { if (!ta.passon) gmw_owner_syrk(dl, S0, Ut0, u0, u1, ta.I, ta.J, acca, fs, tid, krows); ta.computed = true; }
            if (tb.nsteps > 0 && gmw_owner_computes(tb.I, tb.J)) { if (!tb.passon) gmw_owner_syrk(dl, S0, Ut0, u0, u1, tb.I, tb.J, accb, fs, tid, krows); tb.computed = true; }
        }
        if (role == 1) GMW_TS(sy, 129, 1);
        if (role == nmain - 1) GMW_TS(sy, 130, 1);
        if (ha.ntiles > 0) {
            if (wv0) ok = (gmw_wait_head(gmw_head_crit(sy), (unsigned)ha.ncrit, &sy->abort) && gmw_wait_head(gmw_head_done(sy), (unsigned)(ha.ntiles - ha.ncrit), &sy->abort)) ? 1 : 0;
            __syncthreads();
            good = ok != 0;
            if (!good && wv0) gmw_abandon(sy, 3);
            __syncthreads();
        }
        if (role == 1) GMW_TS(sy, 129, 2);
        if (role == nmain - 1) GMW_TS(sy, 130, 2);
        const int kmax = max(ta.nsteps, tb.nsteps);
        for (int k = 0; k < kmax && good; k++) {
            if (k < ta.nsteps && k >= ta.kfirst) good = gmw_owner_step(n, ld, T, k, ta, acca, G, pans, Sout, sy, ebase, Lr, Wc, &ok, wv0, tid, false, half_last && k == Tp - 1);
            if (good && k < tb.nsteps && k >= tb.kfirst) good = gmw_owner_step(n, ld, T, k, tb, accb, G, pans, Sout, sy, ebase, Lr, Wc, &ok, wv0, tid, false, half_last && k == Tp - 1);
        }
        if (good && tc.nsteps > 0) good = gmw_owner_step(n, ld, T, tc.kfirst, tc, acca, G, pans, Sout, sy, ebase, Lr, Wc, &ok, wv0, tid, false, half_last);
        }
        if (!good && wv0) gmw_abandon(sy, 4);
        if (role == 1) GMW_TS(sy, 129, 3);
        if (role == nmain - 1) GMW_TS(sy, 130, 3);
    }
    GMW_DBG(sy, 6, 7777);
    __syncthreads();
    if (tid == 0) {
        const unsigned int done = __hip_atomic_fetch_add(&sy->exited, 1u, __ATOMIC_RELAXED, __HIP_MEMORY_SCOPE_AGENT);
        if (done == gridDim.x - 1) {
            if (__hip_atomic_load(&sy->abort, __ATOMIC_RELAXED, __HIP_MEMORY_SCOPE_AGENT)) { atomicAdd(&fs->clamp_rows, 1); atomicMin(&fs->clamp_first, 0); atomicAdd(&fs->gmw_aborts, 1); }
#ifdef SRUKF_GMW_DBG
            sy->pad[3] = __hip_atomic_load(gmw_head_done(sy), __ATOMIC_RELAXED, __HIP_MEMORY_SCOPE_AGENT); sy->pad[4] = __hip_atomic_load(gmw_head_crit(sy), __ATOMIC_RELAXED, __HIP_MEMORY_SCOPE_AGENT);
            sy->pad[5] = gridDim.x; sy->pad[6] = (unsigned long long)nhelp;
#endif
            __hip_atomic_store(&sy->abort, 0, __ATOMIC_RELAXED, __HIP_MEMORY_SCOPE_AGENT);
            __hip_atomic_store(&sy->exited, 0u, __ATOMIC_RELAXED, __HIP_MEMORY_SCOPE_AGENT);
            __hip_atomic_store(gmw_head_done(sy), 0u, __ATOMIC_RELAXED, __HIP_MEMORY_SCOPE_AGENT);
            __hip_atomic_store(gmw_head_crit(sy), 0u, __ATOMIC_RELAXED, __HIP_MEMORY_SCOPE_AGENT);
            __hip_atomic_store(&sy->resident, 0u, __ATOMIC_RELAXED, __HIP_MEMORY_SCOPE_AGENT);
            __hip_atomic_store(&sy->epoch, (ebase >> GMW_EPOCH_SHIFT) + 1, __ATOMIC_RELAXED, __HIP_MEMORY_SCOPE_AGENT);
            if (gated) atomicSub(&g_gmw_admitted, 1);
        }
    }
}

__global__ __launch_bounds__(256) void k_gmw_pivslab_persist(int n, int ld, int T, int Tp, double* __restrict__ G, GmwPanel64* __restrict__ pans,
                                                             double* __restrict__ Sout, double* __restrict__ Dall, double eps, GmwSync* __restrict__ sy,
                                                             FrameScalars* __restrict__ fs, int krows, double* __restrict__ Wslab, double* __restrict__ Lslab,
                                                             unsigned int total_exits)
{
    __shared__ double Lr[64][G64_LS];
    __shared__ double Wc[64][G64_LS];
    __shared__ double facreg[2 * GMW_FAC_DOUBLES];
    __shared__ double xreg[1024 + 1024 + 32 * 33];
    __shared__ double keepreg[1024 + 64 + 64];
    __shared__ int ok, halfcnt, stageok[2];
    const int tid = threadIdx.x, lane = tid & 63;
    int frozen_now = fs->frozen;
    unsigned long long epoch_now = sy->epoch;
    asm volatile("" : "+s"(frozen_now), "+s"(epoch_now));
    if (frozen_now) return;
    const unsigned long long ebase = epoch_now << GMW_EPOCH_SHIFT;
    if (tid == 0) __hip_atomic_fetch_add(&sy->resident, 1u, __ATOMIC_RELAXED, __HIP_MEMORY_SCOPE_AGENT);
    const bool wv0 = __builtin_amdgcn_readfirstlane(tid >> 6) == 0;
    if (blockIdx.x == 0) {
        gmw_pivot_persist(n, ld, T, Tp, eps, G, pans, Dall, Sout, sy, ebase, Lr, Wc, facreg, xreg, keepreg, &ok, &halfcnt, stageok, tid, krows);
    } else {
        const int J = (int)blockIdx.x, wv = tid >> 6;
        unsigned long long* ver = gmw_sync_ver(sy);
        unsigned long long* slabver = gmw_sync_slabver(sy, T);
        const bool half_last = (Tp < T) && (krows <= 64 * (Tp - 1) + 32);
        const int kend = min(J, Tp);
        bool good = true;
        for (int k = 0; k < kend && good; k++) {
            if (wv0) {
                bool g2 = gmw_wait_ge(&sy->panel_ready[(blockIdx.x % GMW_FLAG_COPIES) * GMW_FLAG_STRIDE], ebase + k + 1, &sy->abort);
                if (g2 && k >= 1) g2 = gmw_wait_ge(&ver[GMW_VIDX(k, J, T)], ebase + k, &sy->abort);
                ok = g2 ? 1 : 0;
            }
            __syncthreads();
            good = ok != 0;
            if (good) {
                const bool r32 = half_last && k == Tp - 1;
                gmw_slab16_to_global<true>(n, ld, 64 * k, 64 * J + 16 * wv, G, pans + k, Sout, Wslab + (size_t)k * 64 * ld, Lslab + (size_t)k * 64 * ld, J >= k + 2 || (Tp < T && k == Tp - 1), r32, lane);
                gmw_publish(&slabver[GMW_VIDX(k, J, T)], ebase + 1, wv0);
            }
            __syncthreads();
        }
        if (!good && wv0) gmw_abandon(sy, 5);
    }
    __syncthreads();
    if (tid == 0) {
        const unsigned int done = __hip_atomic_fetch_add(&sy->exited, 1u, __ATOMIC_RELAXED, __HIP_MEMORY_SCOPE_AGENT);
        if (done == total_exits - 1) {
            if (__hip_atomic_load(&sy->abort, __ATOMIC_RELAXED, __HIP_MEMORY_SCOPE_AGENT)) { atomicAdd(&fs->clamp_rows, 1); atomicMin(&fs->clamp_first, 0); atomicAdd(&fs->gmw_aborts, 1); }
            __hip_atomic_store(&sy->abort, 0, __ATOMIC_RELAXED, __HIP_MEMORY_SCOPE_AGENT);
            __hip_atomic_store(&sy->exited, 0u, __ATOMIC_RELAXED, __HIP_MEMORY_SCOPE_AGENT);
            __hip_atomic_store(&sy->resident, 0u, __ATOMIC_RELAXED, __HIP_MEMORY_SCOPE_AGENT);
            __hip_atomic_store(&sy->epoch, (ebase >> GMW_EPOCH_SHIFT) + 1, __ATOMIC_RELAXED, __HIP_MEMORY_SCOPE_AGENT);
        }
    }
}
__global__ __launch_bounds__(256) __attribute__((amdgpu_waves_per_eu(4, 8)))
void k_gmw_tiles_persist(int ld, int T, double* __restrict__ G, GmwSync* __restrict__ sy, const GmwTile* __restrict__ tiles, FrameScalars* __restrict__ fs,
                         const double* __restrict__ Wslab, const double* __restrict__ Lslab, unsigned int total_exits)
{
    __shared__ int ok;
    const int tid = threadIdx.x, lane = tid & 63, wv = tid >> 6, lr = lane & 15, lk = lane >> 4;
    const unsigned long long tq = ((const unsigned long long*)tiles)[blockIdx.x];
    int frozen_now = fs->frozen;
    unsigned long long epoch_now = sy->epoch;
    if (frozen_now) return;
    const unsigned long long ebase = epoch_now << GMW_EPOCH_SHIFT;
    const int I = (int)(short)(tq & 0xffff), J = (int)(short)((tq >> 16) & 0xffff), ns = (int)(short)((tq >> 32) & 0xffff);
    const bool wv0 = __builtin_amdgcn_readfirstlane(wv) == 0;
    unsigned long long* ver = gmw_sync_ver(sy);
    const unsigned long long* slabver = gmw_sync_slabver(sy, T);
    const int m0 = 64 * I + 32 * (wv >> 1), c0 = 64 * J + 32 * (wv & 1);
    const bool live = (m0 < ld) && (c0 < ld) && (c0 + 32 > m0);
    d4 acc[2][2];
    zero_acc(acc);
    if (live) {
#pragma unroll
        for (int a = 0; a < 2; a++)
#pragma unroll
            for (int b = 0; b < 2; b++)
#pragma unroll
                for (int t = 0; t < 4; t++) acc[a][b][t] = G[(size_t)(m0 + 16 * a + lk + 4 * t) * ld + c0 + 16 * b + lr];
    }
    bool good = true;
    for (int k = 0; k < ns && good; k++) {
        if (wv0) {
            const unsigned long long want = ebase + 1;
            unsigned long long a = 0, b = 0;
            for (int spins = 0; spins < GMW_XWG_LIMIT; spins++) {
                a = gmw_uniform64(__hip_atomic_load(&slabver[GMW_VIDX(k, I, T)], __ATOMIC_RELAXED, __HIP_MEMORY_SCOPE_AGENT));
                b = gmw_uniform64(__hip_atomic_load(&slabver[GMW_VIDX(k, J, T)], __ATOMIC_RELAXED, __HIP_MEMORY_SCOPE_AGENT));
                if (a >= want && b >= want) break;
                if ((spins & 31) == 31 && __builtin_amdgcn_readfirstlane(__hip_atomic_load(&sy->abort, __ATOMIC_RELAXED, __HIP_MEMORY_SCOPE_AGENT))) break;
                if (I - k <= 2) __builtin_amdgcn_s_sleep(2); else __builtin_amdgcn_s_sleep(32);
            }
            ok = (a >= want && b >= want) ? 1 : 0;
        }
        __syncthreads();
        good = ok != 0;
        if (good && live) {
            const double* __restrict__ Lb = Lslab + (size_t)k * 64 * ld + m0 + lr;
            const double* __restrict__ Wb = Wslab + (size_t)k * 64 * ld + c0 + lr;
#pragma unroll
            for (int kk = 0; kk < 64; kk += 16) {
                double a0[4], a1[4], b0[4], b1[4];
#pragma unroll
                for (int u = 0; u < 4; u++) {
                    const size_t ro = (size_t)(kk + 4 * u + lk) * ld;
                    a0[u] = Lb[ro]; a1[u] = Lb[ro + 16]; b0[u] = Wb[ro]; b1[u] = Wb[ro + 16];
                }
#pragma unroll
                for (int u = 0; u < 4; u++) {
                    acc[0][0] = __builtin_amdgcn_mfma_f64_16x16x4f64(-a0[u], b0[u], acc[0][0], 0, 0, 0);
                    acc[0][1] = __builtin_amdgcn_mfma_f64_16x16x4f64(-a0[u], b1[u], acc[0][1], 0, 0, 0);
                    acc[1][0] = __builtin_amdgcn_mfma_f64_16x16x4f64(-a1[u], b0[u], acc[1][0], 0, 0, 0);
                    acc[1][1] = __builtin_amdgcn_mfma_f64_16x16x4f64(-a1[u], b1[u], acc[1][1], 0, 0, 0);
                }
            }
        }
        __syncthreads();
    }
    if (good) {
        if (live) {
#pragma unroll
            for (int a = 0; a < 2; a++)
#pragma unroll
                for (int b = 0; b < 2; b++)
#pragma unroll
                    for (int t = 0; t < 4; t++) st_dev(&G[(size_t)(m0 + 16 * a + lk + 4 * t) * ld + c0 + 16 * b + lr], acc[a][b][t]);
// ... 34 lines not shown
        for (int b = 0; b < 2; b++)
#pragma unroll
            for (int t = 0; t < 4; t++) {
                const int r = m0 + 16 * a + lk + 4 * t, c = n0 + 16 * b + lr;
                const double v = acc[a][b][t];
                st_dev(&G[(size_t)r * ld + c], v);
                if (r < n && c < n) { if (r == c) gmax = fmax(gmax, v); else xmax = fmax(xmax, v); }
            }
    gmax = wave_max(gmax); xmax = wave_max(xmax);
    if (lane == 0) {
        if (gmax > 0.0) atomicMax(&fs->gmax_bits, (unsigned long long)__double_as_longlong(gmax));
        if (xmax > 0.0) atomicMax(&fs->ximax_bits, (unsigned long long)__double_as_longlong(xmax));
    }
}
__device__ __forceinline__ void gmw_fold_tile_wg(int ld, int T, int I, int J, int ns, double* __restrict__ G, GmwSync* __restrict__ sy, unsigned long long ebase,
                                                 const double* __restrict__ Wslab, const double* __restrict__ Lslab, int* okp, int head_rows)
{
    const int tid = threadIdx.x, lane = tid & 63, wv = tid >> 6, lr = lane & 15, lk = lane >> 4;
    const bool wv0 = __builtin_amdgcn_readfirstlane(wv) == 0;
    unsigned long long* ver = gmw_sync_ver(sy);
    const unsigned long long* slabver = gmw_sync_slabver(sy, T);
    unsigned long long* formver = gmw_sync_formver(sy, T);
    int& ok = *okp;
    {
        __builtin_amdgcn_s_setprio(3);
        const int m0 = 64 * I + 32 * (wv >> 1), c0 = 64 * J + 32 * (wv & 1);
        const bool live = (m0 < ld) && (c0 < ld) && (c0 + 32 > m0);
        if (wv0) {
            const int nq = (I < head_rows || (I == 1 && J == 1)) ? 0 : (I == J ? 3 : 4);
            const unsigned long long want = ebase + nq;
            const unsigned long long* w = &formver[GMW_VIDX(I, J, T)];
            int got = nq == 0 ? 1 : 0;
            for (int spins = 0; spins < GMW_XWG_LIMIT && !got; spins++) {
                if (gmw_uniform64(__hip_atomic_load(w, __ATOMIC_RELAXED, __HIP_MEMORY_SCOPE_AGENT)) >= want) got = 1;
                else {
                    if ((spins & 31) == 31 && __builtin_amdgcn_readfirstlane(__hip_atomic_load(&sy->abort, __ATOMIC_RELAXED, __HIP_MEMORY_SCOPE_AGENT))) break;
                    if (I <= 2) __builtin_amdgcn_s_sleep(2); else __builtin_amdgcn_s_sleep(32);
                }
            }
            ok = got;
        }
        __syncthreads();
        bool good = ok != 0;
        __syncthreads();
        d4 acc[2][2];
        zero_acc(acc);
        if (good && live) {
#pragma unroll
            for (int a = 0; a < 2; a++)
#pragma unroll
                for (int b = 0; b < 2; b++)
#pragma unroll
                    for (int t = 0; t < 4; t++) acc[a][b][t] = ld_dev(&G[(size_t)(m0 + 16 * a + lk + 4 * t) * ld + c0 + 16 * b + lr]);
        }
        for (int k = 0; k < ns && good; k++) {
            if (wv0) {
                const unsigned long long want = ebase + 1;
                unsigned long long a = 0, b = 0;
                for (int spins = 0; spins < GMW_XWG_LIMIT; spins++) {
                    a = gmw_uniform64(__hip_atomic_load(&slabver[GMW_VIDX(k, I, T)], __ATOMIC_RELAXED, __HIP_MEMORY_SCOPE_AGENT));
                    b = gmw_uniform64(__hip_atomic_load(&slabver[GMW_VIDX(k, J, T)], __ATOMIC_RELAXED, __HIP_MEMORY_SCOPE_AGENT));
                    if (a >= want && b >= want) break;
                    if ((spins & 31) == 31 && __builtin_amdgcn_readfirstlane(__hip_atomic_load(&sy->abort, __ATOMIC_RELAXED, __HIP_MEMORY_SCOPE_AGENT))) break;
                    if (I - k <= 2) __builtin_amdgcn_s_sleep(2); else __builtin_amdgcn_s_sleep(32);
                }
                ok = (a >= want && b >= want) ? 1 : 0;
            }
            __syncthreads();
            good = ok != 0;
            if (good && live) {
                const double* __restrict__ Lb = Lslab + (size_t)k * 64 * ld + m0 + lr;
                const double* __restrict__ Wb = Wslab + (size_t)k * 64 * ld + c0 + lr;
                double a0[16], a1[16], b0[16], b1[16];
#pragma unroll
                for (int u = 0; u < 16; u++) {
                    const size_t ro = (size_t)(4 * u + lk) * ld;
                    a0[u] = Lb[ro]; a1[u] = Lb[ro + 16]; b0[u] = Wb[ro]; b1[u] = Wb[ro + 16];
                }
#pragma unroll
                for (int u = 0; u < 16; u++) {
                    acc[0][0] = __builtin_amdgcn_mfma_f64_16x16x4f64(-a0[u], b0[u], acc[0][0], 0, 0, 0);
                    acc[0][1] = __builtin_amdgcn_mfma_f64_16x16x4f64(-a0[u], b1[u], acc[0][1], 0, 0, 0);
                    acc[1][0] = __builtin_amdgcn_mfma_f64_16x16x4f64(-a1[u], b0[u], acc[1][0], 0, 0, 0);
                    acc[1][1] = __builtin_amdgcn_mfma_f64_16x16x4f64(-a1[u], b1[u], acc[1][1], 0, 0, 0);
                }
            }
            __syncthreads();
        }
        if (good) {
            if (live) {
#pragma unroll
                for (int a = 0; a < 2; a++)
#pragma unroll
                    for (int b = 0; b < 2; b++)
#pragma unroll
                        for (int t = 0; t < 4; t++) st_dev(&G[(size_t)(m0 + 16 * a + lk + 4 * t) * ld + c0 + 16 * b + lr], acc[a][b][t]);
            }
            gmw_publish(&ver[GMW_VIDX(I, J, T)], ebase + ns, wv0);
        } else if (wv0) gmw_abandon(sy, 6);
        }
}
__global__ __launch_bounds__(256) __attribute__((amdgpu_waves_per_eu(4, 8)))
void k_gmw_tiles_fold(int n, int ld, int T, double* __restrict__ G, GmwSync* __restrict__ sy, const GmwTile* __restrict__ list, FrameScalars* __restrict__ fs,
                      const double* __restrict__ Wslab, const double* __restrict__ Lslab, unsigned int total_exits,
                      const double* __restrict__ A, const double* __restrict__ Ut, int mp, int krows, int head_rows)
{
    __shared__ int ok;
    __shared__ double red[3][64][17];
    const int tid = threadIdx.x;
    const unsigned long long tq = ((const unsigned long long*)list)[blockIdx.x];
    int frozen_now = fs->frozen;
    unsigned long long epoch_now = sy->epoch;
    if (frozen_now) return;
    const unsigned long long ebase = epoch_now << GMW_EPOCH_SHIFT;
    const int I = (int)(short)(tq & 0xffff), J = (int)(short)((tq >> 16) & 0xffff), ns = (int)(short)((tq >> 32) & 0xffff);
    unsigned long long* formver = gmw_sync_formver(sy, T);
    if (ns == -1) {
        gmw_form_job(n, ld, krows, A, Ut, mp, I, J, G, fs, red, tid);
        asm volatile("s_waitcnt vmcnt(0)" ::: "memory");
        if (tid == 0) {
            unsigned long long* w = &formver[GMW_VIDX(I >> 1, J >> 1, T)];
            unsigned long long cur = __hip_atomic_load(w, __ATOMIC_RELAXED, __HIP_MEMORY_SCOPE_AGENT);
            for (;;) {
                const unsigned long long nxt = (cur >= ebase ? cur : ebase) + 1;
                if (__hip_atomic_compare_exchange_strong(w, &cur, nxt, __ATOMIC_RELAXED, __ATOMIC_RELAXED, __HIP_MEMORY_SCOPE_AGENT)) break;
            }
        }
    } else if (ns >= 0) {
        gmw_fold_tile_wg(ld, T, I, J, ns, G, sy, ebase, Wslab, Lslab, &ok, head_rows);
    }
    __syncthreads();
    if (tid == 0) {
        const unsigned int done = __hip_atomic_fetch_add(&sy->exited, 1u, __ATOMIC_RELAXED, __HIP_MEMORY_SCOPE_AGENT);
        if (done == total_exits - 1) {
            if (__hip_atomic_load(&sy->abort, __ATOMIC_RELAXED, __HIP_MEMORY_SCOPE_AGENT)) { atomicAdd(&fs->clamp_rows, 1); atomicMin(&fs->clamp_first, 0); atomicAdd(&fs->gmw_aborts, 1); }
            __hip_atomic_store(&sy->abort, 0, __ATOMIC_RELAXED, __HIP_MEMORY_SCOPE_AGENT);
            __hip_atomic_store(&sy->exited, 0u, __ATOMIC_RELAXED, __HIP_MEMORY_SCOPE_AGENT);
            __hip_atomic_store(&sy->resident, 0u, __ATOMIC_RELAXED, __HIP_MEMORY_SCOPE_AGENT);
            __hip_atomic_store(&sy->epoch, (ebase >> GMW_EPOCH_SHIFT) + 1, __ATOMIC_RELAXED, __HIP_MEMORY_SCOPE_AGENT);
        }
    }
}
__global__ void k_gmw_split_gate(GmwSync* __restrict__ sy, const FrameScalars* __restrict__ fs, unsigned int want)
{
    if (fs->frozen) return;
    for (int spins = 0; spins < GMW_XWG_LIMIT; spins++) {
        if ((unsigned)__builtin_amdgcn_readfirstlane((int)__hip_atomic_load(&sy->resident, __ATOMIC_RELAXED, __HIP_MEMORY_SCOPE_AGENT)) >= want) return;
        __builtin_amdgcn_s_sleep(4);
    }
    if (threadIdx.x == 0) gmw_abandon(sy, 7);
}

extern "C" {
int srukf_gmw_sync_bytes(int T) { return (int)(sizeof(GmwSync) + 3 * sizeof(unsigned long long) * (size_t)T * T * GMW_VER_STRIDE); }
int srukf_gmw_build_tiles(int T, int Tp, short* out)
{
    int cnt = 0;
    const int Imax = (Tp < T) ? Tp : T - 1;
    for (int I = 1; I <= Imax; I++)
        for (int J = I; J < T; J++) {
            const int ns = (I == J && I < Tp) ? I - 1 : I;
            if (ns < 1) continue;
            if (out) { out[4 * cnt] = (short)I; out[4 * cnt + 1] = (short)J; out[4 * cnt + 2] = (short)ns; out[4 * cnt + 3] = (short)((Tp < T && I == Tp) ? Tp - 1 : 0); }
            cnt++;
        }
    return cnt;
}
int srukf_gmw_persist_workers(int T, int Tp, int max_workers)
{
    const int nt = srukf_gmw_build_tiles(T, Tp, nullptr);
    if (nt == 0) return 0;
    const int npass = (Tp > 0 && Tp < T) ? T - Tp : 0, nreal = nt - npass;
    if (nreal >= 1 && nreal <= GMW_OWNED_MAX * max_workers) {
        const int w = nreal <= max_workers ? nreal : max_workers;
        if (npass <= w) return w;
    }
    if (nt <= GMW_OWNED_MEM * max_workers) return max_workers;
    return -1;
}
static bool gmw_register_form(int T, int Tp, int ntiles, int workers)
{
    const int npass = (Tp > 0 && Tp < T) ? T - Tp : 0, nreal = ntiles - npass;
    return workers > 0 && nreal <= GMW_OWNED_MAX * workers && npass <= workers;
}
void srukf_launch_gmw_persist_head(hipStream_t st, int n, int ld, double eps, double* G, void* pans, double* D, double* Sout,
                                   void* sync, const void* tiles, int ntiles, int workers, void* fs,
                                   const double* S0, const double* Ut0, int u0, int u1, int Tp, int krows, int gate_limit, const HeadArgs* hap)
{
    if (gate_limit > 0) hipLaunchKernelGGL(k_gmw_gate, dim3(1), dim3(64), 0, st, (FrameScalars*)fs, gate_limit);
    const int T = ld / 64;
    if (Tp <= 0 || Tp > T) Tp = T;
    if (krows <= 0 || krows > ld) krows = ld;
    HeadArgs ha = {};
    if (hap) ha = *hap;
    if (workers > 0 && !gmw_register_form(T, Tp, ntiles, workers))
        hipLaunchKernelGGL((k_gmw_persist<true>), dim3(1 + workers), dim3(256), 0, st, n, ld, T, Tp, G, (GmwPanel64*)pans, Sout, D, eps,
                           (GmwSync*)sync, (const GmwTile*)tiles, ntiles, (FrameScalars*)fs, S0, Ut0, u0, u1, krows, gate_limit > 0 ? 1 : 0, HeadArgs{});
    else
        hipLaunchKernelGGL((k_gmw_persist<false>), dim3(ha.nhelp + 1 + workers), dim3(256), 0, st, n, ld, T, Tp, G, (GmwPanel64*)pans, Sout, D, eps,
                           (GmwSync*)sync, (const GmwTile*)tiles, ntiles, (FrameScalars*)fs, S0, Ut0, u0, u1, krows, gate_limit > 0 ? 1 : 0, ha);
}
void srukf_launch_gmw_persist(hipStream_t st, int n, int ld, double eps, double* G, void* pans, double* D, double* Sout,
                              void* sync, const void* tiles, int ntiles, int workers, void* fs,
                              const double* S0, const double* Ut0, int u0, int u1, int Tp, int krows, int gate_limit)
{
    srukf_launch_gmw_persist_head(st, n, ld, eps, G, pans, D, Sout, sync, tiles, ntiles, workers, fs, S0, Ut0, u0, u1, Tp, krows, gate_limit, nullptr);
}
void srukf_launch_syrk_own(hipStream_t st, int n, int ld, const double* S0, const double* Ut0, int u0, int u1, int krows, double* G, void* fs, const void* tiles, int ntiles, int Tp)
{
    const int T = ld / 64;
    const int nreal = ntiles - ((Tp > 0 && Tp < T) ? T - Tp : 0);
    if (krows <= 0 || krows > ld) krows = ld;
    if (nreal > 0) hipLaunchKernelGGL(k_syrk_own, dim3(nreal), dim3(256), 0, st, n, ld, S0, Ut0, u0, u1, krows, G, (FrameScalars*)fs, (const GmwTile*)tiles, nreal);
}
void srukf_launch_syrk_own_b(hipStream_t st, int n, int ld, const void* tab, int B, int u0, int u1, int krows, const void* tiles, int ntiles, int Tp)
{
    const int T = ld / 64;
    const int nreal = ntiles - ((Tp > 0 && Tp < T) ? T - Tp : 0);
    if (krows <= 0 || krows > ld) krows = ld;
    if (nreal > 0) hipLaunchKernelGGL(k_syrk_own_b, dim3(nreal * B), dim3(256), 0, st, n, ld, (const SyrkOwnArgs*)tab, B, u0, u1, krows, (const GmwTile*)tiles, nreal);
}
int srukf_gmw_register_form(int T, int Tp, int ntiles, int workers) { return gmw_register_form(T, Tp, ntiles, workers) ? 1 : 0; }
void srukf_launch_gmw_split(hipStream_t stA, hipStream_t stB, int n, int ld, double eps, double* G, void* pans, double* D, double* Sout, void* sync,
                            const void* tiles, int ntiles, void* fs, int Tp, int krows, double* Wslab, double* Lslab, int starve)
{
    const int T = ld / 64;
    if (Tp <= 0 || Tp > T) Tp = T;
    if (krows <= 0 || krows > ld) krows = ld;
    const int nreal = ntiles - ((Tp < T) ? T - Tp : 0);
    const unsigned int total = (unsigned)(T + (starve ? 0 : nreal));
    hipLaunchKernelGGL(k_gmw_pivslab_persist, dim3(T), dim3(256), 0, stA, n, ld, T, Tp, G, (GmwPanel64*)pans, Sout, D, eps, (GmwSync*)sync, (FrameScalars*)fs, krows, Wslab, Lslab, total);
    hipLaunchKernelGGL(k_gmw_split_gate, dim3(1), dim3(64), 0, stB, (GmwSync*)sync, (const FrameScalars*)fs, (unsigned)T);
    if (nreal > 0 && !starve) hipLaunchKernelGGL(k_gmw_tiles_persist, dim3(nreal), dim3(256), 0, stB, ld, T, G, (GmwSync*)sync, (const GmwTile*)tiles, (FrameScalars*)fs, Wslab, Lslab, total);
}
void srukf_launch_gmw_split_alone(hipStream_t st, int which, int n, int ld, double eps, double* G, void* pans, double* D, double* Sout, void* sync,
                                  const void* tiles, int ntiles, void* fs, int Tp, int krows, double* Wslab, double* Lslab)
{
    const int T = ld / 64;
    if (Tp <= 0 || Tp > T) Tp = T;
    if (krows <= 0 || krows > ld) krows = ld;
    const int nreal = ntiles - ((Tp < T) ? T - Tp : 0);
    if (which == 0) hipLaunchKernelGGL(k_gmw_pivslab_persist, dim3(T), dim3(256), 0, st, n, ld, T, Tp, G, (GmwPanel64*)pans, Sout, D, eps, (GmwSync*)sync, (FrameScalars*)fs, krows, Wslab, Lslab, (unsigned)T);
    else if (nreal > 0) hipLaunchKernelGGL(k_gmw_tiles_persist, dim3(nreal), dim3(256), 0, st, ld, T, G, (GmwSync*)sync, (const GmwTile*)tiles, (FrameScalars*)fs, Wslab, Lslab, (unsigned)nreal);
}
static int g_fold_head_override = 0;
void srukf_gmw_fold_head_override(int v) { g_fold_head_override = v; }
int srukf_gmw_fold_head_rows(int Tp)
{
    int v = 2 * (Tp - 17);
    if (g_fold_head_override > 0) v = g_fold_head_override;
    return std::max(1, std::min(v, Tp - 4));
}
int srukf_gmw_fold_head_tile(int tr, int tc, int head_rows) { return (tr < 2 * head_rows || (tr < 4 && tc < 4)) ? 1 : 0; }
int srukf_gmw_build_fold_list(int T, int Tp, short* out)
{
    if (Tp <= 0 || Tp > T) Tp = T;
    const int nt = srukf_gmw_build_tiles(T, Tp, nullptr);
    std::vector<short> tk((size_t)4 * (nt > 0 ? nt : 1));
    srukf_gmw_build_tiles(T, Tp, tk.data());
    const int nreal = nt - ((Tp < T) ? T - Tp : 0);
    const int Ilast = (Tp < T) ? Tp - 1 : T - 1;
    const int head_rows = srukf_gmw_fold_head_rows(Tp);
    int cnt = 0;
    auto emit = [&](int a, int b, int c) { if (out) { out[4 * cnt] = (short)a; out[4 * cnt + 1] = (short)b; out[4 * cnt + 2] = (short)c; out[4 * cnt + 3] = 0; } cnt++; };
    auto pad8 = [&]() { while (cnt % 8) emit(0, 0, -2); };
    const double lead_a = 1.38, lead_b = 4.6;
    auto place = [&](int I) { const int f = (int)floor(lead_a * I - lead_b); return std::min(Ilast, std::max(I, f)); };
    const int rows = 2, single = 2;
    for (int F0 = 1; F0 <= Ilast;) {
        const int F1 = std::min(Ilast, F0 <= single ? F0 : F0 + rows - 1);
        std::vector<std::pair<short, short>> q[8];
        for (int Jc = F0; Jc < T; Jc++)
            for (int F = F0; F <= F1 && F <= Jc; F++)
                for (int tc = 2 * Jc; tc <= 2 * Jc + 1; tc++)
                    for (int tr = 2 * F; tr <= 2 * F + 1 && tr <= tc; tr++)
                        if (!srukf_gmw_fold_head_tile(tr, tc, head_rows)) q[Jc % 8].push_back({ (short)tr, (short)tc });
        size_t longest = 0;
        for (int x = 0; x < 8; x++) longest = std::max(longest, q[x].size());
        for (size_t r = 0; r < longest; r++)
            for (int x = 0; x < 8; x++) { if (r < q[x].size()) emit(q[x][r].first, q[x][r].second, -1); else emit(0, 0, -2); }
        for (int I = 1; I <= Ilast; I++) {
            const int pl = place(I);
            if (pl < F0 || pl > F1) continue;
            for (int t = 0; t < nreal; t++) if (tk[4 * t] == I) emit(tk[4 * t], tk[4 * t + 1], tk[4 * t + 2]);
        }
        pad8();
        F0 = F1 + 1;
    }
    return cnt;
}
void srukf_launch_gmw_split_fold(hipStream_t stA, hipStream_t stB, int n, int ld, double eps, double* G, void* pans, double* D, double* Sout, void* sync,
                                 const void* list, int nlist, void* fs, int Tp, int krows, double* Wslab, double* Lslab, const double* A, const double* Ut, int mp)
{
    const int T = ld / 64;
    if (Tp <= 0 || Tp > T) Tp = T;
    if (krows <= 0 || krows > ld) krows = ld;
    const unsigned int total = (unsigned)(T + nlist);
    hipLaunchKernelGGL(k_gmw_pivslab_persist, dim3(T), dim3(256), 0, stA, n, ld, T, Tp, G, (GmwPanel64*)pans, Sout, D, eps, (GmwSync*)sync, (FrameScalars*)fs, krows, Wslab, Lslab, total);
    hipLaunchKernelGGL(k_gmw_split_gate, dim3(1), dim3(64), 0, stB, (GmwSync*)sync, (const FrameScalars*)fs, (unsigned)T);
    if (nlist > 0) hipLaunchKernelGGL(k_gmw_tiles_fold, dim3(nlist), dim3(256), 0, stB, n, ld, T, G, (GmwSync*)sync, (const GmwTile*)list, (FrameScalars*)fs, Wslab, Lslab, total, A, Ut, mp, krows, srukf_gmw_fold_head_rows(Tp));
}
int srukf_gmw_head_rows(void) { return 64 * GMW_HEAD_ROWS; }
int srukf_gmw_head_extra_diag(void) { return GMW_HEAD_EXTRA_DIAG; }
}
```

### cv-monoslam_amd/csrc/srukf_replay.hip

```cpp

#include "srukf_ctx.h"
using namespace srukf_impl;

__global__ void k_refactor_reset(int np, unsigned long long* theta_bits, FrameScalars* fs, int reset_stats)
{
    const int i = blockIdx.x * blockDim.x + threadIdx.x;
    if (i < np) theta_bits[i] = 0ull;
    if (i == 0 && reset_stats) { fs->gmax_bits = 0ull; fs->ximax_bits = 0ull; }
}

__global__ void k_set_seq(FrameScalars* fs, const double* odo_seq, int seqF, double a1, double a2, double a3, double a4)
{
    fs->odo_seq = odo_seq; fs->seqF = seqF;
    fs->a[0] = a1; fs->a[1] = a2; fs->a[2] = a3; fs->a[3] = a4;
}

__global__ void k_set_frame(FrameScalars* fs, int frame, int clear_clamp)
{
    fs->frame = frame;
    srukf_prepare_control(fs);
    fs->stat_count = 0;
    fs->const_rows_ok = 0; fs->const_rows_pending = 0;
    for (int q = 0; q < SRUKF_STAT_GROUPS; q++) fs->stat_cnt[q] = 0;
    fs->traj_base = nullptr;
// ... 98 lines not shown
{
    StepPoses po; for (int e = 0; e < 9; e++) po.v[e] = poses[e];
    hipLaunchKernelGGL(k_set_step, dim3(1), dim3(1), 0, st, fs, odo, seqF, a1, a2, a3, a4, fresh, po);
}
void launch_export(hipStream_t st, const void* a, size_t bytes_a, const void* b, size_t bytes_b, void* host_pinned, unsigned long long* flag, unsigned long long seq)
{
    const int na = (int)((bytes_a + 7) / 8), nb = (int)((bytes_b + 7) / 8);
    const int blocks = flag ? 1 : ((na + nb + 255) / 256 > 8 ? 8 : (na + nb + 255) / 256);
    hipLaunchKernelGGL(k_export, dim3(blocks), dim3(256), 0, st, (const unsigned long long*)a, na, (const unsigned long long*)b, nb, (unsigned long long*)host_pinned, flag, seq);
}
void launch_set_frame_control(hipStream_t st, FrameScalars* fs) { hipLaunchKernelGGL(k_set_frame_control, dim3(1), dim3(1), 0, st, fs); }
void launch_commit_motion(hipStream_t st, int n, int ld, double* X, double* S, const double* Cm, const FrameScalars* fs, double* A, const int* iperm, int rk) { hipLaunchKernelGGL(k_commit_motion, dim3((n + 255) / 256), dim3(256), 0, st, n, ld, X, S, Cm, fs, A, iperm, rk); }
void launch_sym_permute(hipStream_t st, int n, int ld, const double* src, int lds, double* dst, const int* map) { hipLaunchKernelGGL(k_sym_permute, dim3(ld), dim3(256), 0, st, n, ld, src, lds, dst, map); }
void launch_gather(hipStream_t st, int n, int ld, const double* src, double* dst, const int* map) { hipLaunchKernelGGL(k_gather, dim3((ld + 255) / 256), dim3(256), 0, st, n, ld, src, dst, map); }

int gmw_persist_mode() { return g_dbg_gmw_persist; }

void quantize_state(srukf_ctx* c)
{
    if (c->storage != SRUKF_STORAGE_F64) hipLaunchKernelGGL(k_quantize, dim3(c->d.n + 1), dim3(256), 0, c->stream, c->d.n, c->d.np, c->S, c->X, c->S32, c->X32);
}

static const double* dx_src(const srukf_ctx* c) { return c->dx_pending ? (c->dx_lm ? c->dxk : c->dxp) : nullptr; }

RankArgs rank_args(const srukf_ctx* c)
{
    RankArgs ra = {};
    ra.dxN = (c->dx_pending && c->dx_lm) ? c->d.N : 0;
    if (c->red_r > 0 && c->shadowA) { ra.A = c->shadowA; ra.Utp = c->Utp; ra.gdiag = c->gdiag; ra.iperm = c->red_iperm; ra.perm = c->red_perm; ra.r = c->red_r; }
    return ra;
}

RankArgs tail_rank_args(const srukf_ctx* c, FrameForm ff) { RankArgs ra = rank_args(c); ra.prep_next = ff.robot_table ? 1 : 0; ra.f32round = (ff.fused_tail() && storage_f32_like(c)) ? 1 : 0; return ra; }

NullSkip null_skip(const srukf_ctx* c)
{
    NullSkip ns = {};
    if (c->dbg.nullskip && c->dbg.pxy2 && c->nskip && c->red_r > 0) {
        ns.dirs = c->nskip; ns.nulls = c->nskip + c->ns_full; ns.rows = c->nskip + c->ns_full + c->ns_null;
        ns.nfull = c->ns_full; ns.nnull = c->ns_null; ns.nrows = c->ns_rows; ns.iperm = c->red_iperm; ns.r = c->red_r;
    }
    return ns;
}

static const double* take_xr1(srukf_ctx* c)
{
    if (!c->xr1_pending) return nullptr;
    c->xr1_pending = false;
    return (const double*)((const char*)c->fs + offsetof(FrameScalars, Xr1));
}

void seq_predict_fused(srukf_ctx* c, FrameForm ff)
{
    const KDims& d = c->d;
    ProfScope ps(c, ff.robot_table ? KC_PROJECT_TABLE : KC_PROJECT_MOTION, 2.0 * 60.0 * d.Na * d.N + 60.0 * d.L, 8.0 * ((double)d.n * d.n / 2 + 2.0 * d.L * 2 * d.N + (double)d.n * 2 * d.N + 8.0 * d.L + 8.0 * d.n));
    RankArgs ra = rank_args(c);
    ra.dzperm = (ff.robot_table && ff.pxy2()) ? 1 : 0;
    if (ff.robot_table) srukf_launch_project_table(c->stream, d, c->w, c->p, c->X, c->S, c->sigR, c->Cmat, c->Z, c->DZ, c->fs, ra, null_skip(c));
    else srukf_launch_project_motion(c->stream, d, c->w, c->p, c->X, c->S, c->sigR, c->Cmat, c->Z, c->DZ, c->fs, ra);
    c->xr1_pending = true;
}

void seq_predict_motion(srukf_ctx* c, const double* odo_pair_dev)
{
    const KDims& d = c->d;
    ProfScope ps(c, KC_MOTION, 60.0 * d.L, 8.0 * (4.0 * d.n + 8.0 * d.L + 4.0 * d.n));
    srukf_launch_motion(c->stream, d, c->w, c->p, c->X, c->S, c->sigR, c->Cmat, c->fs, c->odo_seq, odo_pair_dev, rank_args(c));
}

void seq_predict_measurement(srukf_ctx* c, FrameForm ff)
{
    const KDims& d = c->d;
    {
        ProfScope ps(c, KC_PROJECT, 2.0 * 60.0 * d.Na * d.N, 8.0 * ((double)d.n * d.n / 2 + 2.0 * d.L * 2 * d.N + (double)d.n * 2 * d.N));
        srukf_launch_project(c->stream, d, c->w, c->p, c->X, c->S, c->sigR, c->Z, c->DZ, c->fs);
    }
    if (!ff.fused_stats()) {
        ProfScope ps(c, KC_STATS, 30.0 * d.L * d.N, 8.0 * 3.0 * d.L * 2 * d.N);
        srukf_launch_meas_stats(c->stream, d, c->w, c->X, c->sigR, c->Z, c->mpart, c->h, c->Si, c->vis, c->PxyR);
    }
}

int rank_fused_mode() { return g_dbg_rank_fused; }

void shadow_rebuild(srukf_ctx* c)
{
    if (c->red_r > 0 && c->shadowA) srukf_launch_rank_shadow(c->stream, c->d.n, c->d.np, c->red_r, c->S, c->red_perm, c->shadowA);
}

static bool gmw_plan_persists(const srukf_ctx* c, const GmwPlan& gp) { return gp.workers >= 0 || split_form(c, gp, true); }
static bool gmw_use_persist(const srukf_ctx* c) { return gmw_persist_mode() && c->gmw_shared != 2 && gmw_plan_persists(c, c->gplan); }
bool plan_persists(const srukf_ctx* c, const GmwPlan& gp) { return gmw_use_persist(c) && gmw_plan_persists(c, gp); }

static int plan_tenants(const srukf_ctx* c) { return c->gmw_shared == 1 ? c->shared_tenants : 1; }
int gate_limit(const srukf_ctx* c) { return c->gmw_shared == 1 ? c->shared_tenants : 0; }

static void rank_expand(srukf_ctx* c, const RefactorRequest& rq, FrameForm ff)
{
    const int n = c->d.n, np = c->d.np;
    const bool frame_tail = rq.kind == RefactorRequest::FRAME_TAIL, table = ff.robot_table, fuse = ff.fused_tail();
    const bool f32s = c->storage != SRUKF_STORAGE_F64;
    const bool f32fuse = storage_f32_like(c) && fuse && table && frame_tail;
    const bool f32 = f32s && !f32fuse;
    const bool tt = table && frame_tail && !f32;
    const bool exports = c->step_export.dst && tt && fuse;
    srukf_launch_rank_expand(c->stream, n, np, c->red_r, c->p.epsilon, c->G, c->D, c->red_perm, c->red_iperm, c->gdiag, c->fs, c->X, (frame_tail && !f32) ? 1 : 0, c->S, c->shadowA,
                             tt ? c->sigR : nullptr, c->w.gamma, (tt && fuse) ? 1 : 0, c->d, c->w, c->p, c->Z, c->DZ, f32fuse ? 1 : 0, exports ? &c->step_export : nullptr,
                             c->storage == SRUKF_STORAGE_F32_MIXED ? 1e-6 * c->dbg.mixed_null_ppm : 0.0,
                             (tt && fuse) ? c->fold_sync : nullptr, c->fold_sync ? 4 * (c->d.mp / 64) * (c->d.np / 64) : 0);
    c->step_export_attached = exports;
    if (f32) {
        quantize_state(c);
        srukf_launch_rank_round(c->stream, np, c->red_r, c->shadowA);
        if (frame_tail) srukf_launch_traj(c->stream, c->d, c->X, c->S, c->fs, nullptr, 1);
    }
}

static int fold_tiles_pct(const srukf_ctx* c) { return c->gmw_shared == 1 ? 200 : 106; }

static bool replay_red_fused(const srukf_ctx* c)
{
    return c->red_r > 0 && c->storage != SRUKF_STORAGE_F32_MIXED && c->shadowA && c->w.wc0 == c->w.wm0 && gmw_use_persist(c) &&
           c->gplan_red.workers >= 0 && c->gplan_red.nreal <= c->gplan_red.workers * fold_tiles_pct(c) / 100 && c->gplan_red.T >= 16 &&
           !c->debug_starve && g_dbg_gmw_fused && rank_fused_mode() && g_dbg_rank_fold;
}

bool replay_red_perm(const srukf_ctx* c) { return c->dbg.table_perm && refactor_form(c, refactor_frame_tail(c)).form == RF_PERMUTED_SYRK; }

int replay_motion_mode(const srukf_ctx* c)
{
    const bool st_ok = c->storage == SRUKF_STORAGE_F64 ||
                       (storage_f32_like(c) && c->dbg.f32_fuse && c->dbg.tail_fuse && c->dbg.pxy2 && c->dbg.nullskip && c->nskip && c->tail_ok &&
                        (size_t)c->d.np * sizeof(double) <= 48 * 1024);
    if (c->dbg.fused_motion == 2 && !((replay_red_fused(c) || replay_red_perm(c)) && st_ok && c->null_canonical)) return 1;
    return c->dbg.fused_motion;
}

FrameForm frame_form(const srukf_ctx* c)
{
    const int mode = replay_motion_mode(c);
    const bool fuse = mode == 2 && c->dbg.pxy2 && c->dbg.nullskip && c->nskip && c->tail_ok && c->dbg.tail_fuse &&
                      (size_t)c->d.np * sizeof(double) <= 48 * 1024;
    return FrameForm{ fuse ? MEAS_FUSED_TAIL : (mode == 2 && c->dbg.pxy2) ? MEAS_TABLE : mode ? MEAS_FUSED_MOTION : MEAS_PLAIN, mode == 2 };
}

#define SRUKF_HEAD_FOLD_MIN_FREE_CUS 32

struct HeadJobs { int tiles, dx, gd; int total() const { return tiles + dx + gd; } };
static HeadJobs head_fold_jobs(const srukf_ctx* c) { return HeadJobs{ c->n_syrk_head_tiles, (c->d.n + 255) / 256, (c->d.n - c->red_r + SRUKF_RANK_COLS - 1) / SRUKF_RANK_COLS }; }

static bool head_fold_ok(const srukf_ctx* c)
{
    const int need = g_dbg_head_fold_free.load() > 0 ? g_dbg_head_fold_free.load() : SRUKF_HEAD_FOLD_MIN_FREE_CUS;
    const int free_cus = c->gplan_red.cus - 1 - c->gplan_red.workers;
    const int nhelp = head_fold_jobs(c).total();
    const bool pays = g_dbg_head_fold_free.load() > 0 || 4 * nhelp <= 9 * free_cus;
    return c->dbg.head_fold && c->gmw_shared == 0 && free_cus >= need && pays;
}

static bool split_fold_ok(const srukf_ctx* c)
{
    const GmwPlan& gp = c->gplan_red;
    const bool fits = gp.nreal <= 4 * (gp.cus - gp.T) || g_dbg_fold_force.load() != 0;
    return c->dbg.split_fold && (fits || c->dbg.split_fold == 2) && c->red_r > 0 && c->storage != SRUKF_STORAGE_F32_MIXED && c->split_fold_list && c->n_split_fold > 0 && c->red_head0_tiles &&
           !c->debug_starve && !c->dbg.split_record && plan_persists(c, gp) && split_form(c, gp, true);
}

RefactorPlan refactor_form(const srukf_ctx* c, const RefactorRequest& rq)
{
    RefactorPlan p = {};
    const GmwPlan& gr = c->gplan_red;
    const bool tail = rq.kind == RefactorRequest::FRAME_TAIL;
    const bool reduced = c->red_r > 0 && (c->storage != SRUKF_STORAGE_F32_MIXED || (c->dbg.mixed_rank && c->A32));
    if (tail && replay_red_fused(c)) {
        p.form = RF_OWNERS_FOLD; p.persist = true; p.head_fold = head_fold_ok(c);
    } else if (reduced && tail && c->shadowA && c->w.wc0 == c->w.wm0 && rank_fused_mode()) {
        p.form = RF_PERMUTED_SYRK; p.persist = plan_persists(c, gr);
        p.own_order = c->gmw_shared == 1 && gmw_use_persist(c) && gr.workers > 0 && gr.T >= 16 && !c->debug_starve && g_dbg_gmw_fused && g_dbg_rank_fold &&
                      srukf_gmw_register_form(gr.T, gr.Tp, gr.ntiles, gr.workers);
        p.split_fold = !p.own_order && split_fold_ok(c);
    } else if (reduced) {
        p.form = RF_RANK_VIA_PERMUTATION; p.persist = plan_persists(c, gr);
    } else {
        p.form = RF_FULL_RANK; p.persist = gmw_use_persist(c);
        p.fused = tail && p.persist && c->storage == SRUKF_STORAGE_F64 && c->gplan.ntiles <= c->gplan.workers && c->gplan.T >= 16 && !c->debug_starve && g_dbg_gmw_fused;
    }
    return p;
}

static void syrk_permuted(srukf_ctx* c, FrameForm ff, const int* tiles, int ntiles)
{
    srukf_launch_syrk(c->stream, c->d, c->shadowA, c->Utp, 0, c->d.mp, c->Wf, c->fs, tiles, ntiles, dx_src(c), c->X, tail_rank_args(c, ff), take_xr1(c));
    c->dx_pending = false;
}

static void refactor_owners_fold(srukf_ctx* c, const RefactorRequest& rq, const RefactorPlan& plan, FrameForm ff)
{
    const KDims& d = c->d; const int np = d.np, n = d.n;
    const double rr = c->red_r, hr = srukf_gmw_head_rows();
    const double head_flop = 2.0 * hr * n * (hr / 2.0 + d.mp) + 2.0 * (n - rr) * (rr + d.mp), head_byte = 8.0 * ((hr + d.mp) * n + (n - rr) * (rr + d.mp));
    if (!plan.head_fold) {
        ProfScope ps(c, KC_SYRK, head_flop, head_byte);
        syrk_permuted(c, ff, c->syrk_head_tiles, c->n_syrk_head_tiles);
    }
    {
        ProfScope ps(c, KC_GMW_PERSIST, c->red_fac_flop + c->red_own_flop + (plan.head_fold ? head_flop : 0.0), 8.0 * (2.0 * rr * n + (double)d.mp * n));
        HeadArgs ha = {};
        if (plan.head_fold) {
            HeadJobs hj = head_fold_jobs(c);
            if (!c->dx_pending) hj.dx = 0;
            ha.tiles = (const int2*)c->syrk_head_tiles; ha.ntiles = hj.tiles; ha.ncrit = c->n_syrk_head_crit;
            ha.dxp = dx_src(c); ha.X = c->X; ha.xr1 = take_xr1(c); ha.ndx = hj.dx;
            ha.ra = tail_rank_args(c, ff); ha.ngd = hj.gd;
            ha.nhelp = hj.total();
            c->dx_pending = false;
        }
        srukf_launch_gmw_persist_head(c->stream, n, np, c->p.epsilon, c->Wf, c->gplan_red.pans, c->D, c->G, c->gplan_red.sync, c->gplan_red.tiles, c->gplan_red.ntiles,
                                      c->gplan_red.workers, c->fs, c->shadowA, c->Utp, 0, d.mp, c->red_Tp, kept_rows16(c), gate_limit(c), plan.head_fold ? &ha : nullptr);
    }
    ProfScope ps(c, KC_RANK_EXPAND, 0, 8.0 * 2.5 * (double)n * n);
    rank_expand(c, rq, ff);
}

static void refactor_permuted_syrk(srukf_ctx* c, const RefactorRequest& rq, const RefactorPlan& plan, FrameForm ff)
{
    const KDims& d = c->d; const int np = d.np, n = d.n;
    const double rr = c->red_r, rp = 64.0 * c->red_Tp;
    const bool sfold = plan.split_fold;
    const double syrk_flop_all = rr * rr * rr / 3.0 + rr * rr * (n - rr) + 2.0 * d.mp * (rr * n - rr * rr / 2.0) + 2.0 * (n - rr) * (rr + d.mp);
    {
        ProfScope ps(c, KC_SYRK, sfold ? c->red_head0_flop + 2.0 * (n - rr) * (rr + d.mp) : syrk_flop_all, 8.0 * (rr * n + (double)d.mp * n + rp * n));
        if (c->storage == SRUKF_STORAGE_F32_MIXED) {
            if (c->dbg.mixed_bf16 && c->mxr_xt) {
                srukf_launch_split_bf3(c->stream, c->mxr_krows, np, c->mxr_ktot, 0, c->shadowA, c->mxr_xt, c->mxr_xt_stride);
                srukf_launch_split_bf3(c->stream, d.mp, np, c->mxr_ktot, c->mxr_krows, c->Utp, c->mxr_xt, c->mxr_xt_stride);
                srukf_launch_syrk_bf3(c->stream, n, np, d.mp, c->mxr_krows, c->mxr_ktot, c->mxr_xt, c->mxr_xt_stride, c->mxr_tasks, c->mxr_ntasks, c->mxr_tiles, c->mxr_ntiles,
                                      c->mxr_part, c->Wf, c->fs);
            } else {
                srukf_launch_cvt_f32(c->stream, (size_t)c->mxr_krows * np, c->shadowA, c->A32);
                srukf_launch_cvt_f32(c->stream, (size_t)d.mp * np, c->Utp, c->U32);
                srukf_launch_syrk32(c->stream, n, np, d.mp, c->A32, c->U32, c->mxr_tasks, c->mxr_ntasks, c->mxr_tiles, c->mxr_ntiles, c->mxr_part, c->Wf, c->fs, c->mxr_krows);
            }
            syrk_permuted(c, ff, c->mxr_f64_tiles, c->dbg.mixed_f64_robot ? c->mxr_n_f64_tiles : 0);
        } else if (plan.own_order) {
            syrk_permuted(c, ff, c->syrk_head_tiles, c->n_syrk_head_tiles);
            srukf_launch_syrk_own(c->stream, n, np, c->shadowA, c->Utp, 0, d.mp, kept_rows16(c), c->Wf, c->fs, c->gplan_red.tiles, c->gplan_red.ntiles, c->red_Tp);
        } else if (sfold && c->dbg.split_fold != 2)
            syrk_permuted(c, ff, c->red_head0_tiles, c->n_red_head0_tiles);
        else
            syrk_permuted(c, ff, c->red_syrk_tiles, c->n_red_syrk_tiles);
    }
    {
        ProfScope ps(c, plan.persist ? KC_GMW_PERSIST : KC_GMW_TRAIL, c->red_fac_flop + (sfold ? syrk_flop_all - c->red_head0_flop : 0.0), 8.0 * 2.0 * rp * n);
        launch_gmw_fast(c, c->Wf, c->G, sfold ? GMW_KEPT_PANELS_SPLIT_FOLD : GMW_KEPT_PANELS);
    }
    ProfScope ps(c, KC_RANK_EXPAND, 0, 8.0 * 2.5 * (double)n * n);
    rank_expand(c, rq, ff);
}

static double product_state_order(srukf_ctx* c, const RefactorRequest& rq, const RefactorPlan& plan)
{
    const KDims& d = c->d; const int np = d.np, n = d.n, ub = rq.ub, ue = rq.ue;
    const bool fused = plan.fused;
    const double nn = n;
    const double syrk_flop = nn * nn * nn / 3.0 + nn * nn * (ue - ub), syrk_byte = 8.0 * (nn * nn + (double)(ue - ub) * nn);
    const double head_frac = fused ? fmin(1.0, 2.0 * srukf_gmw_head_rows() / nn) : 1.0;
    if (c->storage == SRUKF_STORAGE_F32_MIXED && ub == 0 && ue == d.mp && !(c->dbg.mixed_rank && c->A32)) {
        ProfScope ps(c, KC_SYRK, syrk_flop, 4.0 * (nn * nn + (double)(ue - ub) * nn) + 8.0 * nn * nn / 2);
        if (c->dx_pending) srukf_launch_gain_dx(c->stream, n, np, c->dxp, c->X, take_xr1(c));
        c->dx_pending = false;
        srukf_launch_cvt_f32(c->stream, (size_t)d.mp * np, c->Ut, c->U32);
        srukf_launch_cvt_robot_cols(c->stream, n, np, c->S, c->S32);
        srukf_launch_syrk32(c->stream, n, np, d.mp, c->S32, c->U32, c->mx_tasks, c->mx_ntasks, c->mx_tiles, c->mx_ntiles, c->mx_part, c->G, c->fs, np);
    } else {
        ProfScope ps(c, KC_SYRK, syrk_flop * head_frac, syrk_byte * head_frac);
        srukf_launch_syrk(c->stream, d, c->S, c->Ut, ub, ue, c->G, c->fs, fused ? c->syrk_head_tiles : c->syrk_tiles,
                          fused ? c->n_syrk_head_tiles : c->n_syrk_tiles, dx_src(c), c->X, RankArgs{}, take_xr1(c));
        c->dx_pending = false;
    }
    if (rq.kind != RefactorRequest::FRAME_TAIL) hipMemcpyAsync(c->Gbak, c->G, sizeof(double) * (size_t)np * np, hipMemcpyDeviceToDevice, c->stream);
    return head_frac;
}

static void refactor_via_permutation(srukf_ctx* c, const RefactorRequest& rq, const RefactorPlan& plan)
{
    const int np = c->d.np, n = c->d.n;
    const double nn = n;
    product_state_order(c, rq, plan);
    {
        ProfScope ps(c, KC_MISC, 0, 16.0 * nn * nn);
        launch_sym_permute(c->stream, n, np, c->G, np, c->Wf, c->red_perm);
        srukf_launch_rank_diag(c->stream, n, np, c->G, c->red_perm, c->gdiag);
    }
    {
        const double rr = 64.0 * c->red_Tp;
        ProfScope ps(c, plan.persist ? KC_GMW_PERSIST : KC_GMW_TRAIL, rr * rr * rr / 3.0 + rr * rr * (nn - rr) + rr * (nn - rr) * (nn - rr) / 2.0, 8.0 * (rr * nn));
        launch_gmw_fast(c, c->Wf, c->G, GMW_KEPT_PANELS);
    }
    ProfScope ps(c, KC_GMW_CHECK, 0, 8.0 * nn * nn);
    rank_expand(c, rq, FORM_PLAIN);
}

static void refactor_full_rank(srukf_ctx* c, const RefactorRequest& rq, const RefactorPlan& plan)
{
    const int np = c->d.np, n = c->d.n;
    const double nn = n;
    const bool fused = plan.fused;
    const double head_frac = product_state_order(c, rq, plan);
    const double syrk_flop = nn * nn * nn / 3.0 + nn * nn * (rq.ue - rq.ub), syrk_byte = 8.0 * (nn * nn + (double)(rq.ue - rq.ub) * nn);
    auto panel_flop = [&](int j0) { const double r2 = np - j0 - 64; return j0 < 0 ? 64.0 * 64.0 * 64.0 / 3.0 : 64.0 * r2 * r2 + 3.0 * 2.0 * 32.0 * 32.0 * r2 + 64.0 * 64.0 * 64.0 / 3.0; };
    auto panel_byte = [&](int j0) { const double r2 = np - j0 - 64; return 8.0 * (r2 * r2 + 2.0 * 64.0 * r2); };
    if (plan.persist) {
        double fl = 0.0, by = 0.0;
        for (int j0 = -64; j0 + 64 < np; j0 += 64) { fl += panel_flop(j0); by += panel_byte(j0); }
        ProfScope ps(c, KC_GMW_PERSIST, fl + syrk_flop * (1.0 - head_frac), by + syrk_byte * (1.0 - head_frac));
        if (fused) srukf_launch_gmw_persist(c->stream, n, np, c->p.epsilon, c->G, c->gplan.pans, c->D, c->Wf, c->gplan.sync, c->gplan.tiles, c->gplan.ntiles,
                                            c->gplan.workers, c->fs, c->S, c->Ut, rq.ub, rq.ue, 0, 0, gate_limit(c));
        else launch_gmw_fast(c, c->G, c->S, GMW_ALL_PANELS);
    } else {
        int pb = 0;
        for (int j0 = -64; j0 + 64 < np; j0 += 64, pb ^= 1) {
            ProfScope ps(c, KC_GMW_TRAIL, panel_flop(j0), panel_byte(j0));
            srukf_launch_gmw_step64(c->stream, n, np, j0, c->p.epsilon, c->G, c->pan[pb ^ 1], c->pan[pb], c->D, c->S, c->fs);
        }
    }
    quantize_state(c);
    {
        ProfScope ps(c, KC_GMW_CHECK, 0, 8.0 * (double)n * n / 2);
        srukf_launch_gmw_check(c->stream, n, np, c->D, fused ? c->Wf : c->S, c->fs, c->X, rq.kind == RefactorRequest::FRAME_TAIL ? 1 : 0, fused ? c->S : nullptr);
    }
    shadow_rebuild(c);
}

void seq_refactor(srukf_ctx* c, const RefactorRequest& rq, FrameForm ff)
{
    if (rq.kind == RefactorRequest::SEQ_COLUMN) {
        ProfScope ps(c, KC_MISC, 0, 8.0 * c->d.np);
        launch_refactor_reset(c->stream, c->d.np, c->theta, c->fs, 1);
    }
    const RefactorPlan plan = refactor_form(c, rq);
    switch (plan.form) {
    case RF_OWNERS_FOLD: refactor_owners_fold(c, rq, plan, ff); break;
    case RF_PERMUTED_SYRK: refactor_permuted_syrk(c, rq, plan, ff); break;
    case RF_RANK_VIA_PERMUTATION: refactor_via_permutation(c, rq, plan); break;
    case RF_FULL_RANK: refactor_full_rank(c, rq, plan); break;
    }
}

int exact_repeat_begin(srukf_ctx* c, int frame, double* traj_base)
{
    const size_t np = c->d.np;
    launch_set_frame(c->stream, c->fs, frame, 1);
    if (traj_base) hipLaunchKernelGGL(k_set_traj, dim3(1), dim3(1), 0, c->stream, c->fs, traj_base);
    launch_refactor_reset(c->stream, (int)np, c->theta, c->fs, 0);
    HIPCHK(c, hipMemcpyAsync(c->G, c->Gbak, sizeof(double) * np * np, hipMemcpyDeviceToDevice, c->stream));
    return SRUKF_OK;
}

void launch_gmw_fast(srukf_ctx* c, double* Gbuf, double* Sout, GmwPanels which)
{
    const int np = c->d.np, n = c->d.n;
    const bool reduced = which != GMW_ALL_PANELS, fold = which == GMW_KEPT_PANELS_SPLIT_FOLD;
    const GmwPlan& gp = reduced ? c->gplan_red : c->gplan;
    const int Tp = reduced ? c->red_Tp : np / 64;
    const int krows = reduced ? kept_rows16(c) : 0;
    if (plan_persists(c, gp)) {
        const int workers = c->debug_starve == 1 ? 0 : gp.workers;
        if (split_form(c, gp, true)) {
            if (c->dbg.split_record) hipMemcpyAsync(c->Gbak, Gbuf, sizeof(double) * (size_t)np * np, hipMemcpyDeviceToDevice, c->stream);
            hipEventRecord(c->ev_fork, c->stream);
            hipStreamWaitEvent(c->side, c->ev_fork, 0);
            if (fold) {
                c->split_fold_seqs++;
                srukf_launch_gmw_split_fold(c->stream, c->side, n, np, c->p.epsilon, Gbuf, gp.pans, c->D, Sout, gp.sync, c->split_fold_list, c->n_split_fold, c->fs, Tp, krows,
                                            c->gsW, c->gsL, c->shadowA, c->Utp, c->d.mp);
            } else
                srukf_launch_gmw_split(c->stream, c->side, n, np, c->p.epsilon, Gbuf, gp.pans, c->D, Sout, gp.sync, gp.tiles, gp.ntiles, c->fs, Tp, krows, c->gsW, c->gsL, c->debug_starve ? 1 : 0);
            hipEventRecord(c->ev_join, c->side);
            hipStreamWaitEvent(c->stream, c->ev_join, 0);
            return;
        }
        srukf_launch_gmw_persist(c->stream, n, np, c->p.epsilon, Gbuf, gp.pans, c->D, Sout, gp.sync, gp.tiles, gp.ntiles, workers, c->fs, nullptr, nullptr, 0, 0, Tp, krows, gate_limit(c));
        return;
    }
    int pb = 0;
    for (int j0 = -64; j0 + 64 < np && j0 + 64 <= 64 * Tp; j0 += 64, pb ^= 1)
        srukf_launch_gmw_step64(c->stream, n, np, j0, c->p.epsilon, Gbuf, c->pan[pb ^ 1], c->pan[pb], c->D, Sout, c->fs);
}

void exact_path(srukf_ctx* c, const double* Gbuf, double* Sout)
{
    const int np = c->d.np, n = c->d.n;
    for (int j = 0; j < n; j++) srukf_launch_gmw_col(c->stream, n, np, j, c->p.epsilon, Gbuf, c->Wf, c->D, c->theta, c->fs, Sout);
}

void run_gmw(srukf_ctx* c, double* Gbuf, double* Sout, bool slow)
{
    const int np = c->d.np, n = c->d.n;
    if (!slow) {
        launch_gmw_fast(c, Gbuf, Sout, GMW_ALL_PANELS);
        srukf_launch_gmw_check(c->stream, n, np, c->D, Sout, c->fs, c->X, 0, nullptr);
    } else {
        launch_refactor_reset(c->stream, np, c->theta, c->fs, 0);
        exact_path(c, Gbuf, Sout);
    }
}

int refactor_reorder(srukf_ctx* c, int ub, int ue)
{
    const KDims& d = c->d;
    const int np = d.np, n = d.n, r = n - 3 * c->K_new;
    const size_t bytes = sizeof(double) * (size_t)np * np;
    if (!c->Sdis) { if (srukf_dmalloc((void**)&c->Sdis, bytes) != hipSuccess) { c->err = "out of device memory (NEED_REORDER buffer)"; return SRUKF_ERR_NOMEM; } }
    launch_refactor_reset(c->stream, np, c->theta, c->fs, 1);
    srukf_launch_syrk(c->stream, d, c->S, c->Ut, ub, ue, c->G, c->fs, c->syrk_tiles, c->n_syrk_tiles, dx_src(c), c->X, RankArgs{}, take_xr1(c));
    c->dx_pending = false;
    for (int stage = 0; stage < 2; stage++) {
        double* out = stage == 0 ? c->Sdis : c->S;
        if (stage == 1) {
            launch_refactor_reset(c->stream, np, c->theta, c->fs, 1);
            srukf_launch_syrk(c->stream, d, c->Sdis, c->Ut, 0, 0, c->G, c->fs, c->syrk_tiles, c->n_syrk_tiles, nullptr, c->X, RankArgs{}, nullptr);
        }
        for (int slow = 0; slow < 2; slow++) {
            launch_set_frame(c->stream, c->fs, 0, 1);
            launch_sym_permute(c->stream, n, np, c->G, np, c->Gbak, stage == 0 ? c->iperm : c->perm);
            if (stage == 0) HIPCHK(c, hipMemsetAsync(c->Sdis, 0, bytes, c->stream));
            run_gmw(c, c->Gbak, out, slow != 0);
            if (stage == 0 && r < np) hipLaunchKernelGGL(k_zero_rows, dim3(np - r), dim3(256), 0, c->stream, np, r, c->Sdis);
            if (slow) break;
            int rc = read_fs(c); if (rc) return rc;
            if (c->hfs->clamp_rows == 0) break;
        }
    }
    quantize_state(c);
    return SRUKF_OK;
}

static void launch_pxy(srukf_ctx* c, FrameForm ff, const GainFold& gf)
{
    const KDims& d = c->d;
    const double nn = d.n;
    const bool fused_stats = ff.fused_stats(), fused_motion = ff.fused_motion(), table = ff.pxy2(), fmode = ff.fused_tail();
    ProfScope ps(c, table ? KC_PXY2 : KC_PXY, nn * nn * 2.0 * d.N, 8.0 * (nn * nn / 2 + 2.0 * nn * 2 * d.N));
    MeasArgs ms = {};
    const double* xrob = fmode ? c->sigR : fused_motion ? (const double*)((const char*)c->fs + offsetof(FrameScalars, Xr1)) : c->X + (d.n - 4);
    if (fused_stats) ms = MeasArgs{ c->X, xrob, c->sigR, c->Z, c->mpart, c->h, c->Si, c->vis, c->PxyR, c->fs, (d.N + 31) / 32, table ? null_skip(c) : NullSkip{}, fmode ? 1 : 0,
                                    fmode ? 1 : 0, c->Cmat };
    if (fused_stats && c->mirror_next) {
        ms.hmirror = (char*)c->hmeas;
        ms.hflag = (unsigned long long*)((char*)c->hfs + sizeof(FrameScalars) + sizeof(double) * 32);
        ms.hseq = c->meas_seq;
        ms.hstamp = (unsigned long long*)(c->hmeas + c->d.mp + 5 * (size_t)c->d.N);
    }
    if (table) srukf_launch_pxy2(c->stream, d, c->DZ, c->shadowA, c->Utp, c->P1, c->pxy2_tiles, c->n_pxy2_tiles, kept_rows16(c), c->w, ms, gf);
    else srukf_launch_pxy(c->stream, d, c->DZ, c->S, c->Ut, c->pxy_tiles, c->n_pxy_tiles, c->w, ms);
}

void seq_pxy(srukf_ctx* c, FrameForm ff) { launch_pxy(c, ff, GainFold{}); }

void seq_gain_only(srukf_ctx* c, const double* z_dev, const int* m_dev, FrameForm ff)
{
    const KDims& d = c->d;
    const bool fused_motion = ff.fused_motion(), table = ff.pxy2(), fmode = ff.fused_tail();
    ProfScope ps(c, KC_GAIN, 8.0 * d.n * 2 * d.N, 8.0 * 2.0 * d.n * 2 * d.N);
    srukf_launch_gain(c->stream, d, c->w, c->Ut, c->PxyR, c->Si, c->vis, c->h, c->z_seq, z_dev, c->m_seq, m_dev, c->fs, c->dxp, c->X, c->Z, rank_args(c),
                      fused_motion ? c->Cmat : nullptr, c->S, table ? c->P1 : nullptr, c->pxy2_split_b0, c->DZ,
                      (fmode && storage_f32_like(c)) ? (double)(float)sqrt(c->p.epsilon) : sqrt(c->p.epsilon),
                      c->sigR, fmode ? 1 : 0, c->next_pose_pending ? c->next_odo + 3 : nullptr, c->odo_step);
    c->next_pose_pending = false;
    c->dx_pending = true; c->dx_lm = false;
}

void seq_gain(srukf_ctx* c, const double* z_dev, const int* m_dev, FrameForm ff)
{
    const bool fold = c->dbg.gain_fold && ff.fused_tail() && !z_dev && !m_dev && !c->mirror_next && !c->next_pose_pending &&
                      c->fold_sync && c->dxk && c->w.wc0 == c->w.wm0 && c->z_seq && c->m_seq;
    GainFold gf = {};
    if (fold) {
        const KDims& d = c->d;
        gf.sync = c->fold_sync; gf.Utp = c->Utp; gf.dxk = c->dxk; gf.z_seq = c->z_seq; gf.m_seq = c->m_seq;
        gf.DZp = c->DZ; gf.perm = c->red_perm; gf.iperm = c->red_iperm; gf.r = c->red_r; gf.split_b0 = c->pxy2_split_b0;
        gf.sqeps = storage_f32_like(c) ? (double)(float)sqrt(c->p.epsilon) : sqrt(c->p.epsilon);
        gf.sc = c->w.wi * c->w.gamma;
        gf.S = c->S; gf.A = c->shadowA;
        gf.nmt = d.mp / 64; gf.nbt = d.np / 64; gf.bt_r0 = (c->red_r - 4) / 64; gf.bt_r1 = (c->red_r - 1) / 64; gf.robot_tiles = c->fold_robot_tiles;
    }
    launch_pxy(c, ff, gf);
    if (fold) { c->dx_pending = true; c->dx_lm = true; c->fold_seqs++; }
    else seq_gain_only(c, z_dev, m_dev, ff);
}


int update_null_set(srukf_ctx* c)
{
    const int enabled = g_dbg_rank_aware;
    const int n = c->d.n, np = c->d.np, T = np / 64;
    const int was = c->red_r;
    step_invalidate(c);
    c->red_r = 0;
    if (enabled && c->rank_aware && n >= 128) {
        srukf_launch_row_energy(c->stream, n, np, c->S, c->D);
        HIPCHK(c, hipMemcpyAsync(c->hstage, c->D, sizeof(double) * n, hipMemcpyDeviceToHost, c->stream));
        HIPCHK(c, hipMemcpy2DAsync(c->hstage + np, sizeof(double), c->S, sizeof(double) * (np + 1), sizeof(double), n, hipMemcpyDeviceToHost, c->stream));
        HIPCHK(c, hipStreamSynchronize(c->stream));
        std::vector<int> perm, drop;
        for (int k = 0; k < n; k++) ((k < n - 4 && c->hstage[k] < SRUKF_NULL_ENERGY) ? drop : perm).push_back(k);
        {
            const double sq = c->storage != SRUKF_STORAGE_F64 ? (double)(float)sqrt(c->p.epsilon) : sqrt(c->p.epsilon);
            bool canon = true;
            for (int k : drop) canon = canon && c->hstage[np + k] == sq && c->hstage[k] == sq * sq;
            c->null_canonical = canon;
        }
        const int r = (int)perm.size(), Tp = (r + 63) / 64;
        if (!drop.empty() && Tp < T) {
            perm.insert(perm.end(), drop.begin(), drop.end());
            for (int k = n; k < np; k++) perm.push_back(k);
            std::vector<int> iperm(np);
            for (int a = 0; a < np; a++) iperm[perm[a]] = a;
            if (!c->red_perm) {
                HIPCHK(c, srukf_dmalloc(&c->red_perm, sizeof(int) * np)); HIPCHK(c, srukf_dmalloc(&c->red_iperm, sizeof(int) * np));
                HIPCHK(c, srukf_dmalloc(&c->gdiag, sizeof(double) * np));
            }
            HIPCHK(c, hipMemcpy(c->red_perm, perm.data(), sizeof(int) * np, hipMemcpyHostToDevice));
            HIPCHK(c, hipMemcpy(c->red_iperm, iperm.data(), sizeof(int) * np, hipMemcpyHostToDevice));
            if (c->gplan_red.Tp != Tp || !c->gplan_red.pans || c->gplan_red.tenants != plan_tenants(c)) {
                gmw_plan_destroy(c->gplan_red, c->stream);
                const int rc = gmw_plan_create(c->gplan_red, np, c->stream, Tp, plan_tenants(c));
                if (rc) { c->err = "rank-aware refactorisation: allocation failed"; return rc; }
            }
            split_ensure(c, c->gplan_red);
            c->red_r = r; c->red_Tp = Tp;
            {
                const double rp = 64.0 * Tp, nn = n, kr = (r + 15) & ~15;
                c->red_fac_flop = (nn - rp) * rp * rp + rp * rp * rp / 3.0;
                c->red_own_flop = 0.0;
// ... 417 lines not shown
```

Baseline: 5544 frames/s.

## Split pivot panel factorization across two relay blocks in persistent GMW kernel

```diff
diff --git a/cv-monoslam_amd/csrc/srukf_api.hip b/cv-monoslam_amd/csrc/srukf_api.hip
--- a/cv-monoslam_amd/csrc/srukf_api.hip
+++ b/cv-monoslam_amd/csrc/srukf_api.hip
@@ -57,7 +57,7 @@
 
 }
 
-static void gmw_tiles_xcd_order(std::vector<short>& tk, int ntiles_all, int workers, int T, int Tp)
+static void gmw_tiles_xcd_order(std::vector<short>& tk, int ntiles_all, int workers, int T, int Tp, int npiv)
 {
     const int ntiles = ntiles_all - ((Tp > 0 && Tp < T) ? T - Tp : 0);
     if (ntiles > workers || ntiles < 16) return;
@@ -81,13 +81,13 @@
         for (size_t q = 0; q < b.size(); q++) grp[4 * band + std::min<size_t>(3, q * 4 / b.size())].push_back(b[q]);
     }
     int cap[8] = { 0 };
-    for (int w = 0; w < ntiles; w++) cap[(w + 1) % 8]++;
+    for (int w = 0; w < ntiles; w++) cap[(w + npiv) % 8]++;
     std::vector<Tl> spill(rest);
     for (int x = 0; x < 8; x++) while ((int)grp[x].size() > cap[x]) { spill.push_back(grp[x].back()); grp[x].pop_back(); }
     for (int x = 0; x < 8; x++) while ((int)grp[x].size() < cap[x] && !spill.empty()) { grp[x].push_back(spill.back()); spill.pop_back(); }
     size_t pos[8] = { 0 };
     for (int w = 0; w < ntiles; w++) {
-        const int x = (w + 1) % 8;
+        const int x = (w + npiv) % 8;
         const Tl t = grp[x][pos[x]++];
         for (int e = 0; e < 4; e++) tk[4 * w + e] = t.v[e];
     }
@@ -103,13 +103,20 @@
     int cus = 0, dev = 0;
     if (hipGetDevice(&dev) != hipSuccess || hipDeviceGetAttribute(&cus, hipDeviceAttributeMultiprocessorCount, dev) != hipSuccess || cus < 2) cus = 2;
     g.cus = cus;
-    const int cap = cus / (tenants > 1 ? tenants : 1) - 1;
+    g.ntiles = srukf_gmw_build_tiles(g.T, g.Tp, nullptr);
+    g.relay = 0;
+    if (srukf_gmw_get_pivot_relay() && g.Tp >= 2) {
+        const int cap2 = cus / (tenants > 1 ? tenants : 1) - 2;
+        const int w2 = cap2 >= 1 ? srukf_gmw_persist_workers(g.T, g.Tp, cap2) : -1;
+        const int w1 = srukf_gmw_persist_workers(g.T, g.Tp, cap2 + 1), nreal = g.ntiles - (g.Tp < g.T ? g.T - g.Tp : 0);
+        if (w2 > 0 && w1 > 0 && srukf_gmw_register_form(g.T, g.Tp, g.ntiles, w2) && (nreal + w2 - 1) / w2 == (nreal + w1 - 1) / w1) g.relay = 1;
+    }
+    const int cap = cus / (tenants > 1 ? tenants : 1) - (g.relay ? 2 : 1);
     g.workers = cap >= 1 ? srukf_gmw_persist_workers(g.T, g.Tp, cap) : -1;
-    g.ntiles = srukf_gmw_build_tiles(g.T, g.Tp, nullptr);
     g.nreal = g.ntiles - (g.Tp < g.T ? g.T - g.Tp : 0);
     std::vector<short> tk((size_t)4 * (g.ntiles > 0 ? g.ntiles : 1), 0);
     srukf_gmw_build_tiles(g.T, g.Tp, tk.data());
-    gmw_tiles_xcd_order(tk, g.ntiles, g.workers, g.T, g.Tp);
+    gmw_tiles_xcd_order(tk, g.ntiles, g.workers, g.T, g.Tp, g.relay ? 2 : 1);
     const size_t sync_bytes = (size_t)srukf_gmw_sync_bytes(g.T);
     if (srukf_dmalloc_on(&g.pans, (size_t)srukf_gmw_panel_bytes() * g.T, st) != hipSuccess ||
         srukf_dmalloc_on(&g.sync, sync_bytes, st) != hipSuccess ||
diff --git a/cv-monoslam_amd/csrc/srukf_ctx.h b/cv-monoslam_amd/csrc/srukf_ctx.h
--- a/cv-monoslam_amd/csrc/srukf_ctx.h
+++ b/cv-monoslam_amd/csrc/srukf_ctx.h
@@ -38,8 +38,10 @@
 int srukf_gmw_sync_bytes(int T);
 int srukf_gmw_build_tiles(int T, int Tp, short* out);
 int srukf_gmw_persist_workers(int T, int Tp, int max_workers);
-void srukf_launch_gmw_persist(hipStream_t, int, int, double, double*, void*, double*, double*, void*, const void*, int, int, void*, const double*, const double*, int, int, int, int, int);
-void srukf_launch_gmw_persist_head(hipStream_t, int, int, double, double*, void*, double*, double*, void*, const void*, int, int, void*, const double*, const double*, int, int, int, int, int, const HeadArgs*);
+void srukf_launch_gmw_persist(hipStream_t, int, int, double, double*, void*, double*, double*, void*, const void*, int, int, void*, const double*, const double*, int, int, int, int, int, int);
+void srukf_gmw_set_pivot_relay(int);
+int srukf_gmw_get_pivot_relay(void);
+void srukf_launch_gmw_persist_head(hipStream_t, int, int, double, double*, void*, double*, double*, void*, const void*, int, int, void*, const double*, const double*, int, int, int, int, int, const HeadArgs*, int);
 void srukf_launch_gmw_split(hipStream_t, hipStream_t, int, int, double, double*, void*, double*, double*, void*, const void*, int, void*, int, int, double*, double*, int);
 void srukf_launch_gmw_split_fold(hipStream_t, hipStream_t, int, int, double, double*, void*, double*, double*, void*, const void*, int, void*, int, int, double*, double*, const double*, const double*, int);
 int srukf_gmw_build_fold_list(int T, int Tp, short* out);
@@ -114,7 +116,7 @@
               KC_ARCHIVE_PREDICT, KC_ARCHIVE_WARP, KC_ARCHIVE_SEARCH, KC_ASSOC_CHECKED, KC_COUNT };
 struct ProfEvent { hipEvent_t a, b; int kc; };
 
-struct GmwPlan { void* pans = nullptr; void* sync = nullptr; void* tiles = nullptr; int ntiles = 0, nreal = 0, T = 0, Tp = 0, workers = -1, tenants = 1, cus = 0; };
+struct GmwPlan { void* pans = nullptr; void* sync = nullptr; void* tiles = nullptr; int ntiles = 0, nreal = 0, T = 0, Tp = 0, workers = -1, tenants = 1, cus = 0, relay = 0; };
 
 struct DetScratch {
     double *resp = nullptr, *cand_r = nullptr; int *cand_pix = nullptr, *sorted = nullptr, *rank = nullptr, *gxy = nullptr, *blk = nullptr; void* hdr = nullptr;
diff --git a/cv-monoslam_amd/csrc/srukf_debug.hip b/cv-monoslam_amd/csrc/srukf_debug.hip
--- a/cv-monoslam_amd/csrc/srukf_debug.hip
+++ b/cv-monoslam_amd/csrc/srukf_debug.hip
@@ -68,6 +68,7 @@
                                                   };
     if (!strcmp(key, "batch_split")) { g_dbg_batch_split = value ? 1 : 0; batch_drop_all_graphs(); return SRUKF_OK; }
     if (!strcmp(key, "head_fold_free")) { if (value < 1) return SRUKF_ERR_BAD_ARG; g_dbg_head_fold_free = value; if (c) { hipSetDevice(c->device); step_commit_motion(c); step_invalidate(c); hipStreamSynchronize(c->stream); drop_graphs(c); } return SRUKF_OK; }
+    if (!strcmp(key, "pivot_relay")) { srukf_gmw_set_pivot_relay(value); return SRUKF_OK; }
     if (!strcmp(key, "batch_groups")) { if (value < 0 || value > SRUKF_BATCH_GROUPS_MAX) return SRUKF_ERR_BAD_ARG; g_dbg_batch_groups = value; return SRUKF_OK; }
     if (!strcmp(key, "batch_wide")) { g_dbg_batch_wide = value ? 1 : 0; return SRUKF_OK; }
     if (!strcmp(key, "timing")) { g_dbg_timing = value ? 1 : 0; return SRUKF_OK; }
@@ -183,6 +184,7 @@
         else if (!strcmp(k, "workers")) *value = gp.workers;
         else if (!strcmp(k, "persist")) *value = persist ? 1 : 0;
         else if (!strcmp(k, "register_form")) *value = (persist && !split_form(c, gp) && srukf_gmw_register_form(gp.T, gp.Tp, gp.ntiles, gp.workers)) ? 1 : 0;
+        else if (!strcmp(k, "relay")) *value = (persist && !split_form(c, gp) && gp.relay && srukf_gmw_register_form(gp.T, gp.Tp, gp.ntiles, gp.workers)) ? 1 : 0;
         else if (!strcmp(k, "tiles_per_worker")) *value = gp.workers > 0 ? (gp.nreal + gp.workers - 1) / gp.workers : -1;
         else if (!strcmp(k, "fold")) *value = rp.form == RF_OWNERS_FOLD ? 1 : 0;
         else if (!strcmp(k, "head_fold")) *value = rp.head_fold ? 1 : 0;
@@ -259,7 +261,7 @@
     if (!force_slow) {
         if (gmw_persist_mode()) { const int rc = gmw_plan_create(r.gp, np, st); if (rc) return rc; }
         if (gmw_persist_mode() && r.gp.workers >= 0) {
-            srukf_launch_gmw_persist(st, n, np, epsilon, r.dG, r.gp.pans, r.dD, r.dS, r.gp.sync, r.gp.tiles, r.gp.ntiles, r.gp.workers, r.dFs, nullptr, nullptr, 0, 0, 0, 0, 0);
+            srukf_launch_gmw_persist(st, n, np, epsilon, r.dG, r.gp.pans, r.dD, r.dS, r.gp.sync, r.gp.tiles, r.gp.ntiles, r.gp.workers, r.dFs, nullptr, nullptr, 0, 0, 0, 0, 0, r.gp.relay);
         } else {
             GH(srukf_dmalloc(&r.pan[0], srukf_gmw_panel_bytes())); GH(srukf_dmalloc(&r.pan[1], srukf_gmw_panel_bytes()));
             GH(hipMemset(r.pan[0], 0, srukf_gmw_panel_bytes())); GH(hipMemset(r.pan[1], 0, srukf_gmw_panel_bytes()));
diff --git a/cv-monoslam_amd/csrc/srukf_gmw_persist.hip b/cv-monoslam_amd/csrc/srukf_gmw_persist.hip
--- a/cv-monoslam_amd/csrc/srukf_gmw_persist.hip
+++ b/cv-monoslam_amd/csrc/srukf_gmw_persist.hip
@@ -299,6 +299,288 @@
     }
 }
 
+#ifndef GMW_RELAY_ACC_EARLY
+#define GMW_RELAY_ACC_EARLY 1
+#endif
+#define GMW_PIVOT_COPY(q) ((q) * GMW_FLAG_STRIDE + 128)
+__device__ __forceinline__ void gmw_set_panel_flag_relay(unsigned long long* f, unsigned long long v, int lane)
+{
+    const int idx = lane < GMW_FLAG_COPIES ? lane * GMW_FLAG_STRIDE : GMW_PIVOT_COPY((lane - GMW_FLAG_COPIES) & 1);
+    if (lane < GMW_FLAG_COPIES + 2) __hip_atomic_store(&f[idx], v, __ATOMIC_RELAXED, __HIP_MEMORY_SCOPE_AGENT);
+}
+__device__ __forceinline__ void gmw_pivot_relay(int n, int ld, int T, int Tp, double eps, double* __restrict__ G, GmwPanel64* __restrict__ pans,
+                                                double* __restrict__ Dall, double* __restrict__ Sout, GmwSync* sy, unsigned long long ebase,
+                                                double (*Lr)[G64_LS], double (*Wc)[G64_LS], double* facreg, double* xreg,
+                                                int* okp, int* halfcnt, int tid, int klim, const int q)
+{
+    const int lane = tid & 63, wv = tid >> 6, lr = lane & 15, lk = lane >> 4;
+    const int qa = wv >> 1, qb = wv & 1;
+    const GmwColsLds ws = gmw_cols_carve(facreg), ws2 = gmw_cols_carve(facreg + GMW_FAC_DOUBLES);
+    double (*X01)[32] = (double (*)[32])xreg;
+    double (*X11)[32] = (double (*)[32])(xreg + 1024);
+    double* const T1l = xreg + 2048;
+    double* const T2l = xreg;
+    unsigned long long* ver = gmw_sync_ver(sy);
+    const unsigned long long* my_half = &sy->half_ready[GMW_PIVOT_COPY(q)];
+    const unsigned long long* my_full = &sy->panel_ready[GMW_PIVOT_COPY(q)];
+    const int ro = (wv == 1) ? 0 : 32;
+    const int wvu = __builtin_amdgcn_readfirstlane(wv);
+    const bool wv0 = wvu == 0, wv1 = wvu == 1, wv3 = wvu == 3;
+    const unsigned int site = q ? 8u : 1u;
+    if (wv0) *okp = 1;
+    if (q == 0 && wv3) gmw_stage_tile(Wc, G, ld, 0, 0, lane);
+    __syncthreads();
+    for (int p = q; p < Tp; p += 2) {
+        const int j0 = 64 * (p - 1), base = 64 * p;
+        const bool first = (p == 0);
+        const bool half_only = (p == Tp - 1) && (Tp < T) && (klim <= base + 32);
+        GmwPanel64* nxt = pans + p;
+        const GmwPanel64* prv = pans + (first ? 0 : p - 1);
+        if (wv0) GMW_TS(sy, p, 5);
+        if (!first) {
+            const bool tileA = wvu < 2;
+            const int tr = tileA ? p - 1 : p, r0 = (wvu & 1) ? 0 : 32;
+            const bool ready = p == 1 || gmw_wait_ge(&ver[GMW_VIDX(tr, p, T)], ebase + p - 1, &sy->abort);
+            if (!ready) *okp = 0;
+            else {
+                double (*dst)[G64_LS] = tileA ? Lr : Wc;
+                const double* src = G + (size_t)(64 * tr + r0) * ld + base + lane;
+                double v[32];
+#pragma unroll
+                for (int r = 0; r < 32; r++) v[r] = ld_dev(src + (size_t)r * ld);
+#pragma unroll
+                for (int r = 0; r < 32; r++) dst[r0 + r][lane] = v[r];
+            }
+            __syncthreads();
+            if (!*okp) { if (wv0) gmw_abandon(sy, site); return; }
+        }
+        if (wv0) GMW_TS(sy, p, 6);
+        if (wv0) { ws.Dv[lane & 31] = 0.0; ws2.Dv[lane & 31] = 0.0; *halfcnt = 0; }
+        d4 g;
+#pragma unroll
+        for (int t = 0; t < 4; t++) g[t] = Wc[16 * qa + lk + 4 * t][16 * qb + lr];
+        d4 acc[2][2];
+        zero_acc(acc);
+        if (wv & 1) {
+#pragma unroll
+            for (int a = 0; a < 2; a++)
+#pragma unroll
+                for (int b = 0; b < 2; b++)
+#pragma unroll
+                    for (int t = 0; t < 4; t++) acc[a][b][t] = Wc[ro + 16 * a + lk + 4 * t][32 + 16 * b + lr];
+        }
+        d4 X2[2];
+        double fb[8], sqv[8];
+        if (!first) {
+#pragma unroll
+            for (int u = 0; u < 8; u++) fb[u] = Lr[4 * u + lk][16 * wv + lr];
+#pragma unroll
+            for (int a = 0; a < 2; a++)
+#pragma unroll
+                for (int t = 0; t < 4; t++) X2[a][t] = Lr[32 + 16 * a + lk + 4 * t][16 * wv + lr];
+        }
+        __syncthreads();
+        if (!first) {
+            const int cc = 16 * wv + lr;
+            if (!gmw_wait_ge(my_half, ebase + p, &sy->abort)) *okp = 0;
+            if (wv0) GMW_TS(sy, p, 7);
+            {
+                double ta0[4], ta1[8], ea0[8], ea1[8], dr[2][4];
+#pragma unroll
+                for (int u = 0; u < 8; u++) {
+                    const int o = (4 * u + lk) * 32 + lr;
+                    if (u < 4) ta0[u] = ld_dev(&prv->Tt1[o]);
+                    ta1[u] = ld_dev(&prv->Tt1[o + 16]);
+                    ea0[u] = ld_dev(&prv->E[o]); ea1[u] = ld_dev(&prv->E[o + 16]);
+                }
+#pragma unroll
+                for (int a = 0; a < 2; a++)
+#pragma unroll
+                    for (int t = 0; t < 4; t++) dr[a][t] = ld_dev(&prv->rD[16 * a + lk + 4 * t]);
+                d4 W1[2] = { (d4){0, 0, 0, 0}, (d4){0, 0, 0, 0} };
+#pragma unroll
+                for (int u = 0; u < 8; u++) {
+                    if (u < 4) W1[0] = __builtin_amdgcn_mfma_f64_16x16x4f64(ta0[u], fb[u], W1[0], 0, 0, 0);
+                    W1[1] = __builtin_amdgcn_mfma_f64_16x16x4f64(ta1[u], fb[u], W1[1], 0, 0, 0);
+                }
+#pragma unroll
+                for (int u = 0; u < 8; u++) {
+                    X2[0] = __builtin_amdgcn_mfma_f64_16x16x4f64(-ea0[u], W1[u >> 2][u & 3], X2[0], 0, 0, 0);
+                    X2[1] = __builtin_amdgcn_mfma_f64_16x16x4f64(-ea1[u], W1[u >> 2][u & 3], X2[1], 0, 0, 0);
+                }
+#pragma unroll
+                for (int a = 0; a < 2; a++)
+#pragma unroll
+                    for (int t = 0; t < 4; t++) {
+                        const int jj = 16 * a + lk + 4 * t;
+                        Wc[jj][cc] = W1[a][t];       Lr[jj][cc] = W1[a][t] * dr[a][t];
+                    }
+            }
+            __syncthreads();
+#pragma unroll
+            for (int k = 0; k < 32; k += 4)
+                g = __builtin_amdgcn_mfma_f64_16x16x4f64(-Lr[k + lk][16 * qa + lr], Wc[k + lk][16 * qb + lr], g, 0, 0, 0);
+#if GMW_RELAY_ACC_EARLY
+            if (wv & 1) {
+#pragma unroll
+                for (int k = 0; k < 32; k += 4) {
+                    const double a0 = -Lr[k + lk][ro + lr], a1 = -Lr[k + lk][ro + 16 + lr];
+                    const double b0 = Wc[k + lk][32 + lr], b1 = Wc[k + lk][48 + lr];
+                    acc[0][0] = __builtin_amdgcn_mfma_f64_16x16x4f64(a0, b0, acc[0][0], 0, 0, 0);
+                    acc[0][1] = __builtin_amdgcn_mfma_f64_16x16x4f64(a0, b1, acc[0][1], 0, 0, 0);
+                    acc[1][0] = __builtin_amdgcn_mfma_f64_16x16x4f64(a1, b0, acc[1][0], 0, 0, 0);
+                    acc[1][1] = __builtin_amdgcn_mfma_f64_16x16x4f64(a1, b1, acc[1][1], 0, 0, 0);
+                }
+            }
+#endif
+            if (wv0) GMW_TS(sy, p, 0);
+            if (!gmw_wait_ge(my_full, ebase + p, &sy->abort)) *okp = 0;
+            if (wv0) GMW_TS(sy, p, 1);
+            {
+                double tb0[4], tb1[8], dr2[2][4];
+#pragma unroll
+                for (int u = 0; u < 8; u++) {
+                    const int o = (4 * u + lk) * 32 + lr;
+                    if (u < 4) tb0[u] = ld_dev(&prv->Tt2[o]);
+                    tb1[u] = ld_dev(&prv->Tt2[o + 16]);
+                }
+#pragma unroll
+                for (int a = 0; a < 2; a++)
+#pragma unroll
+                    for (int t = 0; t < 4; t++) dr2[a][t] = ld_dev(&prv->rD[32 + 16 * a + lk + 4 * t]);
+                if (wv & 1) {
+#pragma unroll
+                    for (int i = 0; i < 8; i++) sqv[i] = ld_dev(&prv->sq[ro + 4 * i + lk]);
+                }
+                d4 W2[2] = { (d4){0, 0, 0, 0}, (d4){0, 0, 0, 0} };
+#pragma unroll
+                for (int u = 0; u < 8; u++) {
+                    if (u < 4) W2[0] = __builtin_amdgcn_mfma_f64_16x16x4f64(tb0[u], X2[u >> 2][u & 3], W2[0], 0, 0, 0);
+                    W2[1] = __builtin_amdgcn_mfma_f64_16x16x4f64(tb1[u], X2[u >> 2][u & 3], W2[1], 0, 0, 0);
+                }
+#pragma unroll
+                for (int a = 0; a < 2; a++)
+#pragma unroll
+                    for (int t = 0; t < 4; t++) {
+                        const int jj = 32 + 16 * a + lk + 4 * t;
+                        Wc[jj][cc] = W2[a][t];       Lr[jj][cc] = W2[a][t] * dr2[a][t];
+                    }
+            }
+            __syncthreads();
+#pragma unroll
+            for (int k = 32; k < 64; k += 4)
+                g = __builtin_amdgcn_mfma_f64_16x16x4f64(-Lr[k + lk][16 * qa + lr], Wc[k + lk][16 * qb + lr], g, 0, 0, 0);
+        }
+#pragma unroll
+        for (int t = 0; t < 4; t++) ws.Xm[16 * qa + lk + 4 * t][16 * qb + lr] = g[t];
+        __syncthreads();
+        if (wv0) GMW_TS(sy, p, 2);
+        if (!*okp) { if (wv0) gmw_abandon(sy, site); return; }
+        if (wv0) { gmw_cols_pivot_wave(ws, eps, lane); GMW_TS(sy, p + 64, 4); }
+        else if (wvu == 2) { gmw_cols_t_wave<0>(ws, lane, nullptr, T1l); GMW_TS(sy, p + 64, 5); }
+        else {
+            if (!first) {
+#pragma unroll
+                for (int k = GMW_RELAY_ACC_EARLY ? 32 : 0; k < 64; k += 4) {
+                    const double a0 = -Lr[k + lk][ro + lr], a1 = -Lr[k + lk][ro + 16 + lr];
+                    const double b0 = Wc[k + lk][32 + lr], b1 = Wc[k + lk][48 + lr];
+                    acc[0][0] = __builtin_amdgcn_mfma_f64_16x16x4f64(a0, b0, acc[0][0], 0, 0, 0);
+                    acc[0][1] = __builtin_amdgcn_mfma_f64_16x16x4f64(a0, b1, acc[0][1], 0, 0, 0);
+                    acc[1][0] = __builtin_amdgcn_mfma_f64_16x16x4f64(a1, b0, acc[1][0], 0, 0, 0);
+                    acc[1][1] = __builtin_amdgcn_mfma_f64_16x16x4f64(a1, b1, acc[1][1], 0, 0, 0);
+                }
+            }
+            double (*X)[32] = (wv == 1) ? X01 : X11;
+#pragma unroll
+            for (int a = 0; a < 2; a++)
+#pragma unroll
+                for (int b = 0; b < 2; b++)
+#pragma unroll
+                    for (int t = 0; t < 4; t++) X[16 * a + lk + 4 * t][16 * b + lr] = acc[a][b][t];
+            if (!first) {
+                const int c4 = lr * 4;
+#pragma unroll
+                for (int i = 0; i < 8; i++) {
+                    const int row = ro + 4 * i + lk;
+                    const double sq = sqv[i];
+                    d4 w = *(const d4*)&Wc[row][c4];
+                    w[0] *= sq; w[1] *= sq; w[2] *= sq; w[3] *= sq;
+                    *(d4*)&Sout[(size_t)(j0 + row) * ld + base + c4] = w;
+                }
+            }
+            if (wv1) GMW_TS(sy, p + 64, 6); else GMW_TS(sy, p + 64, 7);
+        }
+        __syncthreads();
+        if (wv0) GMW_TS(sy, p, 3);
+        {
+            d4 wq = (d4){0, 0, 0, 0};
+#pragma unroll
+            for (int u = 0; u < 8; u++)
+                wq = __builtin_amdgcn_mfma_f64_16x16x4f64(T1l[(4 * u + lk) * 33 + 16 * qa + lr], X01[4 * u + lk][16 * qb + lr], wq, 0, 0, 0);
+#pragma unroll
+            for (int t = 0; t < 4; t++) {
+                const int k = 16 * qa + lk + 4 * t, cc = 16 * qb + lr;
+                const double e = wq[t] * gmw_pivot_rcp(ws.Dv[k]);
+                Wc[k][cc] = wq[t];
+                Lr[k][cc] = e;
+            }
+        }
+        __syncthreads();
+        if (!half_only) {
+            d4 x;
+#pragma unroll
+            for (int t = 0; t < 4; t++) x[t] = X11[16 * qa + lk + 4 * t][16 * qb + lr];
+#pragma unroll
+            for (int k = 0; k < 32; k += 4)
+                x = __builtin_amdgcn_mfma_f64_16x16x4f64(-Lr[k + lk][16 * qa + lr], Wc[k + lk][16 * qb + lr], x, 0, 0, 0);
+#pragma unroll
+            for (int t = 0; t < 4; t++) ws2.Xm[16 * qa + lk + 4 * t][16 * qb + lr] = x[t];
+        }
+        __syncthreads();
+        if (wv0) GMW_TS(sy, p, 4);
+        if (wv0) { if (!half_only) gmw_cols_pivot_wave(ws2, eps, lane); GMW_TS(sy, p + 64, 0); }
+        else if (wvu == 2) {
+            if (!half_only) { gmw_cols_t_wave<2>(ws2, lane, nxt->Tt2, T2l); GMW_TS(sy, p + 64, 3); }
+        } else {
+            const int c4 = (lane & 7) * 4;
+            if (wv1) {
+#pragma unroll
+                for (int i = 0; i < 4; i++) {
+                    const int row = 8 * i + (lane >> 3);
+                    st_d4<true>(&nxt->E[row * 32 + c4], *(const d4*)&Lr[row][c4]);
+                }
+                if (lane < 32) {
+                    const double D = ws.Dv[lane], rc = gmw_pivot_rcp(D), sq = sqrt(D) * rc;
+                    st_dev(&nxt->D[lane], D); st_dev(&nxt->sq[lane], sq); st_dev(&nxt->rD[lane], rc);
+                }
+            } else gmw_copy_t<true>(T1l, nxt->Tt1, lane);
+            asm volatile("s_waitcnt vmcnt(0)" ::: "memory");
+            {
+                int prev = 0;
+                if (lane == 0) prev = __hip_atomic_fetch_add(halfcnt, 1, __ATOMIC_RELAXED, __HIP_MEMORY_SCOPE_WORKGROUP);
+                if (__builtin_amdgcn_readfirstlane(prev) == 1) gmw_set_panel_flag_relay(sy->half_ready, ebase + p + 1, lane);
+            }
+            if (!wv1) {
+#pragma unroll
+                for (int i = 0; i < 4; i++) {
+                    const int row = 8 * i + (lane >> 3);
+                    const double Dr = ws.Dv[row];
+                    const double sq = (base + row < n) ? sqrt(Dr) * gmw_pivot_rcp(Dr) : 0.0;
+                    d4 w = *(const d4*)&Wc[row][c4];
+                    w[0] *= sq; w[1] *= sq; w[2] *= sq; w[3] *= sq;
+                    *(d4*)&Sout[(size_t)(base + row) * ld + base + 32 + c4] = w;
+                }
+            }
+            gmw_cols_out_wave<true>(ws, wv1 ? 0 : 1, lane, n, ld, base, nxt->D, nxt->sq, nxt->rD, Dall, Sout);
+            if (!half_only) gmw_cols_out_wave<true>(ws2, wv1 ? 0 : 1, lane, n, ld, base + 32, nxt->D + 32, nxt->sq + 32, nxt->rD + 32, Dall, Sout);
+            if (wv1) GMW_TS(sy, p + 64, 1); else GMW_TS(sy, p + 64, 2);
+        }
+        asm volatile("s_waitcnt vmcnt(0)" ::: "memory");
+        __syncthreads();
+        if (wv3 && p + 1 < T) gmw_set_panel_flag_relay(sy->panel_ready, ebase + p + 1, lane);
+    }
+}
+
 #ifndef GMW_MEM_EARLY2
 #define GMW_MEM_EARLY2 0
 #endif
@@ -483,7 +765,7 @@
                                                      GmwSync* __restrict__ sy, const GmwTile* __restrict__ tiles, int ntiles,
                                                      FrameScalars* __restrict__ fs,
                                                      const double* __restrict__ S0, const double* __restrict__ Ut0, int u0, int u1, int krows, int gated,
-                                                     const HeadArgs ha)
+                                                     const HeadArgs ha, const int relay)
 {
     __shared__ double Lr[64][G64_LS];
     __shared__ double Wc[64][G64_LS];
@@ -494,17 +776,18 @@
     const int tid = threadIdx.x;
     const int nhelp = ha.nhelp;
     const int nmain = (int)gridDim.x - nhelp;
+    const int npiv = (!MEM && relay) ? 2 : 1;
     const int role = (int)blockIdx.x < nmain ? (int)blockIdx.x : -1;
     int2 mytile = make_int2(-1, -1);
     unsigned long long t01 = 0, t23 = 0, t45 = 0;
     const int npass = (!MEM && Tp < T) ? T - Tp : 0, nreal = ntiles - npass;
     if (!MEM) {
         if (role < 0) { const int hb = (int)blockIdx.x - nmain; if (hb < ha.ntiles) mytile = ha.tiles[hb]; }
-        else if (role > 0) {
+        else if (role >= npiv) {
             const unsigned long long* tq = (const unsigned long long*)tiles;
-            if (role - 1 < nreal) t01 = tq[role - 1];
-            if (role - 1 + nmain - 1 < nreal) t23 = tq[role - 1 + nmain - 1];
-            if (role - 1 < npass) t45 = tq[nreal + role - 1];
+            if (role - npiv < nreal) t01 = tq[role - npiv];
+            if (role - npiv + nmain - npiv < nreal) t23 = tq[role - npiv + nmain - npiv];
+            if (role - npiv < npass) t45 = tq[nreal + role - npiv];
         }
     }
     int frozen_now = fs->frozen;
@@ -543,7 +826,7 @@
         if (tid == 0) atomicAdd(&sy->pad[2], 1ull);
 #endif
         }
-    } else if (role == 0) {
+    } else if (role < npiv) {
         bool head_ok = true;
         GMW_TS(sy, 128, 0);
         if (ha.ntiles > 0) {
@@ -553,12 +836,13 @@
             __syncthreads();
         }
         GMW_TS(sy, 128, 1);
-        if (head_ok) gmw_pivot_persist(n, ld, T, Tp, eps, G, pans, Dall, Sout, sy, ebase, Lr, Wc, facreg, xreg, keepreg, &ok, &halfcnt, stageok, tid, krows);
-        else if (__builtin_amdgcn_readfirstlane(tid >> 6) == 0) gmw_abandon(sy, 2);
+        if (!head_ok) { if (__builtin_amdgcn_readfirstlane(tid >> 6) == 0) gmw_abandon(sy, 2); }
+        else if (npiv == 2) { if constexpr (!MEM) gmw_pivot_relay(n, ld, T, Tp, eps, G, pans, Dall, Sout, sy, ebase, Lr, Wc, facreg, xreg, &ok, &halfcnt, tid, krows, role); }
+        else gmw_pivot_persist(n, ld, T, Tp, eps, G, pans, Dall, Sout, sy, ebase, Lr, Wc, facreg, xreg, keepreg, &ok, &halfcnt, stageok, tid, krows);
         GMW_TS(sy, 128, 2);
     } else {
         const bool wv0 = __builtin_amdgcn_readfirstlane(tid >> 6) == 0;
-        const int workers = nmain - 1, w = role - 1;
+        const int workers = nmain - npiv, w = role - npiv;
         bool good = true;
         const bool half_last = (Tp < T) && (krows <= 64 * (Tp - 1) + 32);
         if constexpr (MEM) {
@@ -584,14 +868,14 @@
         if (w < npass) { const GmwTile t = entry(t45); tc.I = t.I; tc.J = t.J; tc.nsteps = t.nsteps; tc.kfirst = t.pad; tc.passon = true; tc.computed = true; }
         d4 acca[2][2], accb[2][2];
         zero_acc(acca); zero_acc(accb);
-        if (role == 1) GMW_TS(sy, 129, 0);
+        if (role == npiv) GMW_TS(sy, 129, 0);
         if (role == nmain - 1) GMW_TS(sy, 130, 0);
         if (S0) {
             const KDimsLite dl = { n, ld };
             if (ta.nsteps > 0 && gmw_owner_computes(ta.I, ta.J)) { if (!ta.passon) gmw_owner_syrk(dl, S0, Ut0, u0, u1, ta.I, ta.J, acca, fs, tid, krows); ta.computed = true; }
             if (tb.nsteps > 0 && gmw_owner_computes(tb.I, tb.J)) { if (!tb.passon) gmw_owner_syrk(dl, S0, Ut0, u0, u1, tb.I, tb.J, accb, fs, tid, krows); tb.computed = true; }
         }
-        if (role == 1) GMW_TS(sy, 129, 1);
+        if (role == npiv) GMW_TS(sy, 129, 1);
         if (role == nmain - 1) GMW_TS(sy, 130, 1);
         if (ha.ntiles > 0) {
             if (wv0) ok = (gmw_wait_head(gmw_head_crit(sy), (unsigned)ha.ncrit, &sy->abort) && gmw_wait_head(gmw_head_done(sy), (unsigned)(ha.ntiles - ha.ncrit), &sy->abort)) ? 1 : 0;
@@ -600,7 +884,7 @@
             if (!good && wv0) gmw_abandon(sy, 3);
             __syncthreads();
         }
-        if (role == 1) GMW_TS(sy, 129, 2);
+        if (role == npiv) GMW_TS(sy, 129, 2);
         if (role == nmain - 1) GMW_TS(sy, 130, 2);
         const int kmax = max(ta.nsteps, tb.nsteps);
         for (int k = 0; k < kmax && good; k++) {
@@ -610,7 +894,7 @@
         if (good && tc.nsteps > 0) good = gmw_owner_step(n, ld, T, tc.kfirst, tc, acca, G, pans, Sout, sy, ebase, Lr, Wc, &ok, wv0, tid, false, half_last);
         }
         if (!good && wv0) gmw_abandon(sy, 4);
-        if (role == 1) GMW_TS(sy, 129, 3);
+        if (role == npiv) GMW_TS(sy, 129, 3);
         if (role == nmain - 1) GMW_TS(sy, 130, 3);
     }
     GMW_DBG(sy, 6, 7777);
@@ -951,6 +1235,9 @@
 }
 
 extern "C" {
+#ifndef SRUKF_PIVOT_RELAY_DEFAULT
+#define SRUKF_PIVOT_RELAY_DEFAULT 1
+#endif
 int srukf_gmw_sync_bytes(int T) { return (int)(sizeof(GmwSync) + 3 * sizeof(unsigned long long) * (size_t)T * T * GMW_VER_STRIDE); }
 int srukf_gmw_build_tiles(int T, int Tp, short* out)
 {
@@ -965,6 +1252,9 @@
         }
     return cnt;
 }
+static int g_pivot_relay = SRUKF_PIVOT_RELAY_DEFAULT;
+void srukf_gmw_set_pivot_relay(int v) { g_pivot_relay = v ? 1 : 0; }
+int srukf_gmw_get_pivot_relay(void) { return g_pivot_relay; }
 int srukf_gmw_persist_workers(int T, int Tp, int max_workers)
 {
     const int nt = srukf_gmw_build_tiles(T, Tp, nullptr);
@@ -984,7 +1274,7 @@
 }
 void srukf_launch_gmw_persist_head(hipStream_t st, int n, int ld, double eps, double* G, void* pans, double* D, double* Sout,
                                    void* sync, const void* tiles, int ntiles, int workers, void* fs,
-                                   const double* S0, const double* Ut0, int u0, int u1, int Tp, int krows, int gate_limit, const HeadArgs* hap)
+                                   const double* S0, const double* Ut0, int u0, int u1, int Tp, int krows, int gate_limit, const HeadArgs* hap, int relay)
 {
     if (gate_limit > 0) hipLaunchKernelGGL(k_gmw_gate, dim3(1), dim3(64), 0, st, (FrameScalars*)fs, gate_limit);
     const int T = ld / 64;
@@ -994,16 +1284,16 @@
     if (hap) ha = *hap;
     if (workers > 0 && !gmw_register_form(T, Tp, ntiles, workers))
         hipLaunchKernelGGL((k_gmw_persist<true>), dim3(1 + workers), dim3(256), 0, st, n, ld, T, Tp, G, (GmwPanel64*)pans, Sout, D, eps,
-                           (GmwSync*)sync, (const GmwTile*)tiles, ntiles, (FrameScalars*)fs, S0, Ut0, u0, u1, krows, gate_limit > 0 ? 1 : 0, HeadArgs{});
+                           (GmwSync*)sync, (const GmwTile*)tiles, ntiles, (FrameScalars*)fs, S0, Ut0, u0, u1, krows, gate_limit > 0 ? 1 : 0, HeadArgs{}, 0);
     else
-        hipLaunchKernelGGL((k_gmw_persist<false>), dim3(ha.nhelp + 1 + workers), dim3(256), 0, st, n, ld, T, Tp, G, (GmwPanel64*)pans, Sout, D, eps,
-                           (GmwSync*)sync, (const GmwTile*)tiles, ntiles, (FrameScalars*)fs, S0, Ut0, u0, u1, krows, gate_limit > 0 ? 1 : 0, ha);
+        hipLaunchKernelGGL((k_gmw_persist<false>), dim3(ha.nhelp + (relay ? 2 : 1) + workers), dim3(256), 0, st, n, ld, T, Tp, G, (GmwPanel64*)pans, Sout, D, eps,
+                           (GmwSync*)sync, (const GmwTile*)tiles, ntiles, (FrameScalars*)fs, S0, Ut0, u0, u1, krows, gate_limit > 0 ? 1 : 0, ha, relay ? 1 : 0);
 }
 void srukf_launch_gmw_persist(hipStream_t st, int n, int ld, double eps, double* G, void* pans, double* D, double* Sout,
                               void* sync, const void* tiles, int ntiles, int workers, void* fs,
-                              const double* S0, const double* Ut0, int u0, int u1, int Tp, int krows, int gate_limit)
-{
-    srukf_launch_gmw_persist_head(st, n, ld, eps, G, pans, D, Sout, sync, tiles, ntiles, workers, fs, S0, Ut0, u0, u1, Tp, krows, gate_limit, nullptr);
+                              const double* S0, const double* Ut0, int u0, int u1, int Tp, int krows, int gate_limit, int relay)
+{
+    srukf_launch_gmw_persist_head(st, n, ld, eps, G, pans, D, Sout, sync, tiles, ntiles, workers, fs, S0, Ut0, u0, u1, Tp, krows, gate_limit, nullptr, relay);
 }
 void srukf_launch_syrk_own(hipStream_t st, int n, int ld, const double* S0, const double* Ut0, int u0, int u1, int krows, double* G, void* fs, const void* tiles, int ntiles, int Tp)
 {
diff --git a/cv-monoslam_amd/csrc/srukf_replay.hip b/cv-monoslam_amd/csrc/srukf_replay.hip
--- a/cv-monoslam_amd/csrc/srukf_replay.hip
+++ b/cv-monoslam_amd/csrc/srukf_replay.hip
@@ -274,9 +274,9 @@
 static bool head_fold_ok(const srukf_ctx* c)
 {
     const int need = g_dbg_head_fold_free.load() > 0 ? g_dbg_head_fold_free.load() : SRUKF_HEAD_FOLD_MIN_FREE_CUS;
-    const int free_cus = c->gplan_red.cus - 1 - c->gplan_red.workers;
+    const int free_cus = c->gplan_red.cus - (c->gplan_red.relay ? 2 : 1) - c->gplan_red.workers;
     const int nhelp = head_fold_jobs(c).total();
-    const bool pays = g_dbg_head_fold_free.load() > 0 || 4 * nhelp <= 9 * free_cus;
+    const bool pays = g_dbg_head_fold_free.load() > 0 || 4 * nhelp <= 9 * (c->gplan_red.cus - 1 - c->gplan_red.workers);
     return c->dbg.head_fold && c->gmw_shared == 0 && free_cus >= need && pays;
 }
 
@@ -338,7 +338,7 @@
             c->dx_pending = false;
         }
         srukf_launch_gmw_persist_head(c->stream, n, np, c->p.epsilon, c->Wf, c->gplan_red.pans, c->D, c->G, c->gplan_red.sync, c->gplan_red.tiles, c->gplan_red.ntiles,
-                                      c->gplan_red.workers, c->fs, c->shadowA, c->Utp, 0, d.mp, c->red_Tp, kept_rows16(c), gate_limit(c), plan.head_fold ? &ha : nullptr);
+                                      c->gplan_red.workers, c->fs, c->shadowA, c->Utp, 0, d.mp, c->red_Tp, kept_rows16(c), gate_limit(c), plan.head_fold ? &ha : nullptr, c->gplan_red.relay);
     }
     ProfScope ps(c, KC_RANK_EXPAND, 0, 8.0 * 2.5 * (double)n * n);
     rank_expand(c, rq, ff);
@@ -437,7 +437,7 @@
         for (int j0 = -64; j0 + 64 < np; j0 += 64) { fl += panel_flop(j0); by += panel_byte(j0); }
         ProfScope ps(c, KC_GMW_PERSIST, fl + syrk_flop * (1.0 - head_frac), by + syrk_byte * (1.0 - head_frac));
         if (fused) srukf_launch_gmw_persist(c->stream, n, np, c->p.epsilon, c->G, c->gplan.pans, c->D, c->Wf, c->gplan.sync, c->gplan.tiles, c->gplan.ntiles,
-                                            c->gplan.workers, c->fs, c->S, c->Ut, rq.ub, rq.ue, 0, 0, gate_limit(c));
+                                            c->gplan.workers, c->fs, c->S, c->Ut, rq.ub, rq.ue, 0, 0, gate_limit(c), c->gplan.relay);
         else launch_gmw_fast(c, c->G, c->S, GMW_ALL_PANELS);
     } else {
         int pb = 0;
@@ -502,7 +502,7 @@
             hipStreamWaitEvent(c->stream, c->ev_join, 0);
             return;
         }
-        srukf_launch_gmw_persist(c->stream, n, np, c->p.epsilon, Gbuf, gp.pans, c->D, Sout, gp.sync, gp.tiles, gp.ntiles, workers, c->fs, nullptr, nullptr, 0, 0, Tp, krows, gate_limit(c));
+        srukf_launch_gmw_persist(c->stream, n, np, c->p.epsilon, Gbuf, gp.pans, c->D, Sout, gp.sync, gp.tiles, gp.ntiles, workers, c->fs, nullptr, nullptr, 0, 0, Tp, krows, gate_limit(c), gp.relay);
         return;
     }
     int pb = 0;
```

Result: faster. 5607 frames/s (median of 6 runs) (+1.1%).
